# Toptachamann/Linear_Programming_Solver

Measured on AMD Instinct MI355X. Metric: simplex_pivots_per_sec, higher is better.
Workload: dtype f64

## Files before the change

### linear_programming_solver_amd/csrc/lpx_decisions.inc

```
constexpr int kMaxBlock = 32;

__global__ __launch_bounds__(256) void k_peek_multi(const double* __restrict__ A, int64_t ld,
                                                    const double* __restrict__ b, int m_local, int row0,
                                                    const double* __restrict__ prow_ring,
                                                    const double* __restrict__ col_ring, int64_t mp,
                                                    const LpxCtl* __restrict__ ring, int np,
                                                    double* __restrict__ col_out, double* __restrict__ col0_out,
                                                    RatioRow* __restrict__ partial,
                                                    const LpxCtl* __restrict__ ctl) {
  __shared__ RatioRow sh[4];
  __shared__ double sh_pe[kMaxBlock], sh_p[kMaxBlock], sh_bl[kMaxBlock];
  __shared__ int sh_e[kMaxBlock], sh_l[kMaxBlock];
  if (ctl->status != kRunning) return;
  const int en = ctl->e_next;
  if (en < 0) return;
  if ((int)threadIdx.x < np) {
    const LpxCtl& q = ring[threadIdx.x];
    sh_e[threadIdx.x] = q.e_cur;
    sh_l[threadIdx.x] = q.l - row0;
    sh_p[threadIdx.x] = q.p;
    sh_bl[threadIdx.x] = q.bl;
    sh_pe[threadIdx.x] = prow_ring[(int64_t)threadIdx.x * ld + en];
  }
  __syncthreads();
// ... 77 lines not shown
  }
}

struct ChainPart {
  double ratio, a, bi;
  int32_t row, pad;
  double unused[4];
};
#ifndef LPX_CHAIN_TAGGED
#define LPX_CHAIN_TAGGED 1
#endif
__device__ __forceinline__ unsigned lo32(double x) { return (unsigned)__double2loint(x); }
__device__ __forceinline__ unsigned hi32(double x) { return (unsigned)__double2hiint(x); }
__device__ __forceinline__ double from32(unsigned lo, unsigned hi) { return __hiloint2double((int)hi, (int)lo); }

struct MgMail {
  double ratio, a, bi;
  int32_t row;
  uint32_t tag;
};
static_assert(sizeof(MgMail) == 32, "mailbox record is one 32-byte granule");

__device__ __forceinline__ double ld_sys(const double* p) {
  return __hip_atomic_load(p, __ATOMIC_RELAXED, __HIP_MEMORY_SCOPE_SYSTEM);
}
__device__ __forceinline__ void st_sys(double* p, double x) {
  __hip_atomic_store(p, x, __ATOMIC_RELAXED, __HIP_MEMORY_SCOPE_SYSTEM);
}

__device__ __forceinline__ double ld_agent(const double* p) {
  return __hip_atomic_load(p, __ATOMIC_RELAXED, __HIP_MEMORY_SCOPE_AGENT);
}
__device__ __forceinline__ int ld_agent(const int32_t* p) {
  return __hip_atomic_load(p, __ATOMIC_RELAXED, __HIP_MEMORY_SCOPE_AGENT);
}
__device__ __forceinline__ void st_agent(double* p, double x) {
  __hip_atomic_store(p, x, __ATOMIC_RELAXED, __HIP_MEMORY_SCOPE_AGENT);
}
__device__ __forceinline__ void st_agent(int32_t* p, int32_t x) {
  __hip_atomic_store(p, x, __ATOMIC_RELAXED, __HIP_MEMORY_SCOPE_AGENT);
}

#ifndef LPX_BARRIER_SLEEP
#define LPX_BARRIER_SLEEP __builtin_amdgcn_s_sleep(1)
#endif
__device__ __forceinline__ bool grid_barrier(unsigned* bar, unsigned target, int* sh_fail, int fences, unsigned spin_max) {
  asm volatile("s_waitcnt vmcnt(0)" ::: "memory");
  __syncthreads();
  if (threadIdx.x == 0) {
    if (fences & 1) {
      __builtin_amdgcn_fence(__ATOMIC_RELEASE, "agent");
      asm volatile("s_waitcnt vmcnt(0)" ::: "memory");
    }
    __hip_atomic_fetch_add(bar, 1u, __ATOMIC_RELAXED, __HIP_MEMORY_SCOPE_AGENT);
    unsigned spins = 0;
    while (__hip_atomic_load(bar, __ATOMIC_RELAXED, __HIP_MEMORY_SCOPE_AGENT) < target) {
      LPX_BARRIER_SLEEP;
      if (++spins > spin_max) { *sh_fail = 1; break; }
    }
    if (fences & 2) {
      __builtin_amdgcn_fence(__ATOMIC_ACQUIRE, "agent");
      asm volatile("s_waitcnt vmcnt(0)" ::: "memory");
    }
  }
  __syncthreads();
  return *sh_fail == 0;
}

#define LPX_CHAIN_STEP_A(on, cs_r, pe_r, l_r)                                      \
  {                                                                                \
    const double t_ = submul(a, (cs_r), (pe_r));                     \
    const double nv_ = (ig == (l_r)) ? (pe_r) : t_;                                \
    a = (on) ? nv_ : a;                                                            \
  }
#define LPX_CHAIN_STEP_B(on, cs_r, prv_r, e_r, dv_r)                               \
  {                                                                                \
    const double t_ = submul(x, (cs_r), (prv_r));                    \
    const double nv_ = (j == (e_r)) ? (dv_r) : t_;                                 \
    x = (on) ? nv_ : x;                                                            \
  }
#define LPX_CHAIN_LIVE(r0, first, last) ((r0) < (last) && (r0) + 8 > (first))
#define LPX_CHAIN_CHUNK_A(off, r0, first, last, csv)                                                   \
  if (LPX_CHAIN_LIVE(r0, first, last)) {                                                           \
    double pe8[8];                                                                                     \
    int l8[8];                                                                                         \
    _Pragma("unroll") for (int q = 0; q < 8; ++q) { pe8[q] = sh_pe[(off) + (r0) + q]; l8[q] = sh_l[(off) + (r0) + q]; } \
    __builtin_amdgcn_sched_barrier(0);                                                                 \
    _Pragma("unroll") for (int q = 0; q < 8; ++q)                                                      \
        LPX_CHAIN_STEP_A(((r0) + q >= (first) && (r0) + q < (last)), csv[(r0) + q], pe8[q], l8[q])     \
  }
#define LPX_CHAIN_CHUNK_B(off, r0, first, last, prvv)                                                  \
  if (LPX_CHAIN_LIVE(r0, first, last)) {                                                           \
    double cs8[8], dv8[8];                                                                             \
    int e8[8];                                                                                         \
    _Pragma("unroll") for (int q = 0; q < 8; ++q) {                                                    \
      cs8[q] = sh_cs[(off) + (r0) + q]; dv8[q] = sh_dv[(off) + (r0) + q]; e8[q] = sh_e[(off) + (r0) + q]; \
    }                                                                                                  \
    __builtin_amdgcn_sched_barrier(0);                                                                 \
    _Pragma("unroll") for (int q = 0; q < 8; ++q)                                                      \
        LPX_CHAIN_STEP_B(((r0) + q >= (first) && (r0) + q < (last)), cs8[q], prvv[(r0) + q], e8[q], dv8[q]) \
  }

__device__ __forceinline__ void chain_publish(const LpxCtl* ctl, LpxCtl* host_snap) {
  if (!host_snap) return;
  *host_snap = *ctl;
  __threadfence_system();
}

__device__ __forceinline__ unsigned xcc_id() {
  unsigned x;
  asm volatile("s_getreg_b32 %0, hwreg(HW_REG_XCC_ID)" : "=s"(x));
  return x & 15u;
}

struct ChainArgs {
  const double* A;
  const double* b;
  int64_t ld, mp;
  int n, m;
  double* c;
  int32_t* perm;
  LpxCtl* ctl;
  double *prow, *col, *col0, *row0, *own_col, *own_prow, *own_dvc;
  LpxCtl* up;
  const double *prow_o, *col_o, *own_col_o, *own_prow_o, *own_dvc_o;
  const LpxCtl* up_o;
  int n_old;
  double* own_b;
  int32_t *own_rs_a, *own_rs_b;
  int b_from_tableau;
  int nb;
  ChainPart* partA;
  RatioRow* partB;
  unsigned long long* hand;
  unsigned hand_base;
  unsigned* bar;
  unsigned* bar_next;
  int dantzig, fences;
  LpxCtl* host_snap;
  long long* dbg;
  unsigned* census;
  int shard_row0;
  int m_global;
  int n_dev, dev;
  int mail_slot0;
  MgMail* mail_peer[kMaxDevices];
  double* prow_peer[kMaxDevices];
  unsigned long long* arrive_peer[kMaxDevices];
  int onehop;
  double* candrow_peer[kMaxDevices];
  unsigned long long* arrive2_peer[kMaxDevices];
  unsigned spin_max;
  int diag;
};

template <int KB>
__device__ __forceinline__ int chain_restart(const unsigned long long* sh_mask) {
  if constexpr (KB > 32) {
    const unsigned long long hi = sh_mask[1], lo = sh_mask[0];
    return hi ? 127 - __clzll((long long)hi) : (lo ? 63 - __clzll((long long)lo) : -1);
  } else {
    const unsigned long long lo = sh_mask[0];
    return lo ? 63 - __clzll((long long)lo) : -1;
  }
}

template <bool MG, int KB>
__global__ __launch_bounds__(256) void k_block_chain_t(const ChainArgs P) {
  static_assert(KB == 32 || KB == 64, "ring half of 32 or 64 slots");
  __shared__ RatioRow sh_rr[4];
  __shared__ unsigned long long sh_mask[2];
#if LPX_CHAIN_TAGGED
  __shared__ unsigned sh_gran[8], sh_part[kChainMaxWgs * 8];
#endif
  __shared__ double sh_pe[2 * KB], sh_cs[2 * KB], sh_dv[2 * KB], sh_p[2 * KB], sh_bl[2 * KB], sh_win[2];
  __shared__ int sh_e[2 * KB], sh_l[2 * KB];
  __shared__ int sh_fail, sh_restart;
  const int row0 = MG ? P.shard_row0 : 0;
  const double* __restrict__ A = P.A;
  const double* __restrict__ b = P.b;
  const int64_t ld = P.ld, mp = P.mp;
  const int n = P.n, m = P.m, nb = P.nb, n_old = P.n_old;
  LpxCtl* const ctl = P.ctl;
  const int G = gridDim.x, T = G * 256, tid = threadIdx.x, gid = blockIdx.x * 256 + tid;
  const bool lead = gid == 0;
  if (tid == 0) {
    sh_fail = 0;
    if (P.census) P.census[blockIdx.x] = xcc_id() + 1u;
  }
  if (lead) st_agent(reinterpret_cast<int32_t*>(P.bar_next), 0);
  int e = ctl->e_next;
  if (ctl->status != kRunning || e < 0 || nb < 1) {
    if (lead && nb >= 1) P.up[0].do_update = 0;
    if (lead) chain_publish(ctl, P.host_snap);
    return;
  }
  if (tid < n_old) {
    const LpxCtl& q = P.up_o[tid];
    sh_e[tid] = q.e_cur; sh_l[tid] = q.l; sh_p[tid] = q.p; sh_bl[tid] = q.bl;
  }
  int64_t pivots = ctl->pivots;
  const int64_t max_pivots = ctl->max_pivots;
  double v = ctl->v;
  int track = ctl->track, parity = ctl->parity;
  unsigned target = 0;

  for (int s = 0; s < nb; ++s) {
    if (P.dbg && lead) P.dbg[s * 5 + 0] = wall_clock64();
    const double pc = ld_agent(&P.c[e]);
    if (tid < 2 * KB) {
      const int r = tid & (KB - 1);
      const bool old = tid < KB;
      const bool valid = old ? r < n_old : r < s;
      bool same = false;
      if (valid) {
        const double* pe_src = (old ? P.prow_o : P.prow) + (int64_t)r * ld + e;
        sh_pe[tid] = MG ? ld_sys(pe_src) : ld_agent(pe_src);
        same = sh_e[tid] == e;
      }
      const unsigned long long mask = __ballot(same);
      if ((tid & 63) == 0) sh_mask[tid >> 6] = mask;
    }
    __syncthreads();
    const int ra = chain_restart<KB>(sh_mask);
    const int fo_a = ra < 0 ? 0 : (ra < KB ? ra + 1 : n_old);
    const int fn_a = ra >= KB ? ra - KB + 1 : 0;
    const bool use_b = P.b_from_tableau && s == 0;
    RatioRow best = rr_none();
    double best_a = 0.0, best_b = 0.0;
    for (int i = gid; i < m; i += T) {
      const double* src_a = ra < 0 ? &A[(int64_t)i * ld + e]
                                   : (ra < KB ? &P.own_dvc_o[(int64_t)ra * mp + i] : &P.own_dvc[(int64_t)(ra - KB) * mp + i]);
      const double* src_b = use_b ? &b[i] : &P.own_b[i];
      double a = *src_a;
      const double bi = *src_b;
      const int ig = row0 + i;
      double cs[KB], cso[KB];
#pragma unroll
      for (int r0 = 0; r0 < KB; r0 += 8)
        if (LPX_CHAIN_LIVE(r0, fo_a, n_old)) {
#pragma unroll
          for (int q = 0; q < 8; ++q) cso[r0 + q] = P.own_col_o[(int64_t)(r0 + q) * mp + i];
        }
#pragma unroll
      for (int r0 = 0; r0 < KB; r0 += 8)
        if (LPX_CHAIN_LIVE(r0, fn_a, s)) {
#pragma unroll
          for (int q = 0; q < 8; ++q) cs[r0 + q] = P.own_col[(int64_t)(r0 + q) * mp + i];
        }
#pragma unroll
      for (int r0 = 0; r0 < KB; r0 += 8) LPX_CHAIN_CHUNK_A(0, r0, fo_a, n_old, cso)
      st_agent(&P.col0[(int64_t)s * mp + i], a);
#pragma unroll
      for (int r0 = 0; r0 < KB; r0 += 8) LPX_CHAIN_CHUNK_A(KB, r0, fn_a, s, cs)
      st_agent(&P.col[(int64_t)s * mp + i], a);
      P.own_col[(int64_t)s * mp + i] = a;
      const double rt = ratio_of(a, bi);
      if (rt < best.ratio) {
        best = RatioRow{rt, ig, 0};
        best_a = a;
        best_b = bi;
      }
    }
    {
      const RatioRow w = rr_block_min(best, sh_rr);
      if (w.row != INT_MAX && best.row == w.row) { sh_win[0] = best_a; sh_win[1] = best_b; }
      __syncthreads();
#if !LPX_CHAIN_TAGGED
      if (tid == 0) {
        ChainPart* rec = &P.partA[(s & 1) * kChainMaxWgs + blockIdx.x];
        st_agent(&rec->ratio, w.ratio);
        st_agent(&rec->row, w.row);
        st_agent(&rec->a, (w.row != INT_MAX) ? sh_win[0] : 0.0);
        st_agent(&rec->bi, (w.row != INT_MAX) ? sh_win[1] : 0.0);
      }
    }
    const unsigned xtag = P.hand_base + (unsigned)s;
    if (P.dbg && lead) P.dbg[s * 5 + 1] = wall_clock64();
    target += (unsigned)G;
    if (!grid_barrier(P.bar, target, &sh_fail, P.fences, P.spin_max)) {
      if (lead) { ctl->status = 7 ; chain_publish(ctl, P.host_snap); }
      return;
    }
    if (P.dbg && lead) P.dbg[s * 5 + 2] = wall_clock64();

    RatioRow mine = rr_none();
    double mine_a = 0.0, mine_b = 0.0;
    if (tid < G) {
      const ChainPart* rec = &P.partA[(s & 1) * kChainMaxWgs + tid];
      mine.ratio = ld_agent(&rec->ratio);
      mine.row = ld_agent(&rec->row);
      mine_a = ld_agent(&rec->a);
      mine_b = ld_agent(&rec->bi);
    }
#else
      sh_gran[0] = lo32(w.ratio); sh_gran[1] = hi32(w.ratio);
      const double wa = (w.row != INT_MAX) ? sh_win[0] : 0.0, wb = (w.row != INT_MAX) ? sh_win[1] : 0.0;
      sh_gran[2] = lo32(wa); sh_gran[3] = hi32(wa); sh_gran[4] = lo32(wb); sh_gran[5] = hi32(wb);
      sh_gran[6] = (unsigned)w.row;
    }
    const unsigned xtag = P.hand_base + (unsigned)s;
#ifndef LPX_CHAIN_DBG2
    if (P.dbg && lead) P.dbg[s * 5 + 1] = wall_clock64();
#endif
    {
      unsigned long long* const gran = reinterpret_cast<unsigned long long*>(P.partA) + (size_t)(s & 1) * kChainMaxWgs * 8;
      asm volatile("s_waitcnt vmcnt(0)" ::: "memory");
// ... 328 lines not shown
      __syncthreads();
    }
    if (e_next < 0) {
      target += (unsigned)G;
      if (!grid_barrier(P.bar, target, &sh_fail, P.fences, P.spin_max)) {
        if (lead) { ctl->status = 7; chain_publish(ctl, P.host_snap); }
        return;
      }
      RatioRow m2 = rr_none();
      if (tid < G) { m2.ratio = ld_agent(&P.partB[tid].ratio); m2.row = ld_agent(&P.partB[tid].row); }
      const RatioRow w3 = rr_block_min(m2, sh_rr);
      e_next = (w3.row == INT_MAX) ? -1 : w3.row;
    }
    if (P.dbg && lead) P.dbg[s * 5 + 4] = wall_clock64();
    pivots += 1;
    parity ^= 1;
    if (lead) {
      ctl->v = v; ctl->p = p; ctl->bl = bl; ctl->pc = pc; ctl->ratio = w.ratio;
      ctl->e_cur = e; ctl->l = l; ctl->e_next = e_next; ctl->parity = parity; ctl->pivots = pivots;
      ctl->track = track; ctl->do_update = 1;
      if (e_next < 0) {
        ctl->status = 0 ;
        if (s + 1 < nb) P.up[s + 1].do_update = 0;
      }
    }
    if (e_next < 0 || s + 1 == nb) {
      if (lead) chain_publish(ctl, P.host_snap);
      return;
    }
    e = e_next;
  }
}

template <int CTRL>
__device__ __forceinline__ int dpp_i32(int v) { return __builtin_amdgcn_update_dpp(v, v, CTRL, 0xf, 0xf, false); }
template <int CTRL>
__device__ __forceinline__ double dpp_f64(double x) {
  return __hiloint2double(dpp_i32<CTRL>(__double2hiint(x)), dpp_i32<CTRL>(__double2loint(x)));
}
__device__ __forceinline__ double lane_f64(double x, int lane) {
  return __hiloint2double(__builtin_amdgcn_readlane(__double2hiint(x), lane), __builtin_amdgcn_readlane(__double2loint(x), lane));
}
__device__ __forceinline__ RatioRow rr_wave_min_all(RatioRow x) {
  double r = x.ratio;
  { const double o = dpp_f64<0xB1>(r); r = o < r ? o : r; }
  { const double o = dpp_f64<0x4E>(r); r = o < r ? o : r; }
  { const double o = dpp_f64<0x141>(r); r = o < r ? o : r; }
  { const double o = dpp_f64<0x140>(r); r = o < r ? o : r; }
  const double r0 = lane_f64(r, 0), r1 = lane_f64(r, 16), r2 = lane_f64(r, 32), r3 = lane_f64(r, 48);
  const double ra = r1 < r0 ? r1 : r0, rb = r3 < r2 ? r3 : r2;
  const double rmin = rb < ra ? rb : ra;
  int row = (x.ratio == rmin) ? x.row : INT_MAX;
  row = min(row, dpp_i32<0xB1>(row));
  row = min(row, dpp_i32<0x4E>(row));
  row = min(row, dpp_i32<0x141>(row));
  row = min(row, dpp_i32<0x140>(row));
  const int q = min(min(__builtin_amdgcn_readlane(row, 0), __builtin_amdgcn_readlane(row, 16)),
                    min(__builtin_amdgcn_readlane(row, 32), __builtin_amdgcn_readlane(row, 48)));
  return RatioRow{rmin, q, 0};
}
__device__ __forceinline__ void lds_barrier() { asm volatile("s_waitcnt lgkmcnt(0)\n\ts_barrier" ::: "memory"); }
__device__ __forceinline__ RatioRow rr_block_min2(RatioRow x, RatioRow* sh) {
  const int lane = threadIdx.x & 63, wave = threadIdx.x >> 6, nw = (blockDim.x + 63) >> 6;
  x = rr_wave_min_all(x);
  lds_barrier();
  if (lane == 0) sh[wave] = x;
  lds_barrier();
  RatioRow r = sh[0];
  for (int w = 1; w < nw; ++w) r = rr_min(r, sh[w]);
  return r;
}

#if LPX_FUSED
#define LPX_C2_T_OUT
#define LPX_C2_STEP(q) "v_fma_f64 %[x], -%[c" #q "], %[r" #q "], %[x]\n\t"
#else
#define LPX_C2_T_OUT , [t] "=&v"(t)
#define LPX_C2_STEP(q) "v_mul_f64 %[t], %[c" #q "], %[r" #q "]\n\tv_add_f64 %[x], %[x], -%[t]\n\t"
#endif
#define LPX_C2_INS                                                                                                           \
  [c0] "v"(c[0]), [c1] "v"(c[1]), [c2] "v"(c[2]), [c3] "v"(c[3]), [c4] "v"(c[4]), [c5] "v"(c[5]), [c6] "v"(c[6]), [c7] "v"(c[7]), \
  [r0] "v"(r[0]), [r1] "v"(r[1]), [r2] "v"(r[2]), [r3] "v"(r[3]), [r4] "v"(r[4]), [r5] "v"(r[5]), [r6] "v"(r[6]), [r7] "v"(r[7])
__device__ __forceinline__ void chain8(double& x, const double* c, const double* r) {
#if !LPX_FUSED
  double t;
#endif
  asm volatile(LPX_C2_STEP(0) LPX_C2_STEP(1) LPX_C2_STEP(2) LPX_C2_STEP(3) LPX_C2_STEP(4) LPX_C2_STEP(5) LPX_C2_STEP(6) LPX_C2_STEP(7)
               : [x] "+v"(x) LPX_C2_T_OUT : LPX_C2_INS);
}
__device__ __forceinline__ void chain8_from(double& x, const double* c, const double* r, int stc) {
#if !LPX_FUSED
  double t;
#endif
  unsigned long long sv, m0, m1, m2, m3, m4, m5, m6, m7;
  asm volatile("s_mov_b64 %[sv], exec\n\t"
               "v_cmp_ge_i32 %[m0], 0, %[stc]\n\tv_cmp_ge_i32 %[m1], 1, %[stc]\n\tv_cmp_ge_i32 %[m2], 2, %[stc]\n\t"
               "v_cmp_ge_i32 %[m3], 3, %[stc]\n\tv_cmp_ge_i32 %[m4], 4, %[stc]\n\tv_cmp_ge_i32 %[m5], 5, %[stc]\n\t"
               "v_cmp_ge_i32 %[m6], 6, %[stc]\n\tv_cmp_ge_i32 %[m7], 7, %[stc]\n\t"
               "s_mov_b64 exec, %[m0]\n\t" LPX_C2_STEP(0) "s_mov_b64 exec, %[m1]\n\t" LPX_C2_STEP(1)
               "s_mov_b64 exec, %[m2]\n\t" LPX_C2_STEP(2) "s_mov_b64 exec, %[m3]\n\t" LPX_C2_STEP(3)
               "s_mov_b64 exec, %[m4]\n\t" LPX_C2_STEP(4) "s_mov_b64 exec, %[m5]\n\t" LPX_C2_STEP(5)
               "s_mov_b64 exec, %[m6]\n\t" LPX_C2_STEP(6) "s_mov_b64 exec, %[m7]\n\t" LPX_C2_STEP(7)
               "s_mov_b64 exec, %[sv]"
               : [x] "+v"(x) LPX_C2_T_OUT, [sv] "=&s"(sv), [m0] "=&s"(m0), [m1] "=&s"(m1), [m2] "=&s"(m2), [m3] "=&s"(m3),
                 [m4] "=&s"(m4), [m5] "=&s"(m5), [m6] "=&s"(m6), [m7] "=&s"(m7)
               : LPX_C2_INS, [stc] "v"(stc));
}
#undef LPX_C2_INS
#undef LPX_C2_STEP
#undef LPX_C2_T_OUT
__device__ __forceinline__ int top_bit(unsigned long long lo, unsigned long long hi) {
  return hi ? 127 - __clzll((long long)hi) : (lo ? 63 - __clzll((long long)lo) : -1);
}
template <int H>
__device__ __forceinline__ int top_bit_of(const unsigned long long (&w)[H]) {
  static_assert(H == 1 || H == 2 || H == 4, "ballots of 64, 128 or 256 slots");
  if constexpr (H == 4) {
    const int hi = top_bit(w[2], w[3]);
    return hi >= 0 ? 128 + hi : top_bit(w[0], w[1]);
  } else if constexpr (H == 2) {
    return top_bit(w[0], w[1]);
  } else {
    return top_bit(w[0], 0);
  }
}

struct MinRec {
  double ratio, a, b;
  int row, pad;
};
template <int NW>
__device__ __forceinline__ RatioRow rr_block_min_rec(RatioRow x, double& a, double& b, MinRec (*sh)[NW], int slot) {
  const int wave = threadIdx.x >> 6, lane = threadIdx.x & 63;
  const RatioRow w = rr_wave_min_all(x);
  if (w.row == INT_MAX ? lane == 0 : x.row == w.row) sh[slot][wave] = MinRec{w.ratio, a, b, w.row, 0};
  lds_barrier();
  MinRec r = sh[slot][0];
#pragma unroll
  for (int k = 1; k < NW; ++k) {
    const MinRec o = sh[slot][k];
    if (o.ratio < r.ratio || (o.ratio == r.ratio && o.row < r.row)) r = o;
  }
  a = r.a;
  b = r.b;
  return RatioRow{r.ratio, r.row, 0};
}

constexpr int kChain2Threads = 256;
#ifdef LPX_CHAIN2_OWN_WT
#define LPX_OWN_STORE(p_, x_) st_agent((p_), (x_))
#else
#define LPX_OWN_STORE(p_, x_) (*(p_) = (x_))
#endif
template <int KB, int NT, bool MG>
__device__ __forceinline__ void block_chain2_body(const ChainArgs& P) {
  static_assert(KB == 32 || KB == 64 || KB == 128, "ring half of 32, 64 or 128 slots");
  static_assert(NT % 64 == 0 && NT >= 256 && NT >= 2 * KB + (KB == 128 ? 0 : 64), "lanes for the pending pivots and the loader lane");
  static_assert(KB <= 64 || !MG, "the shards decide at most kShardBlockMax pivots per block");
  constexpr int NC = 2 * KB / 8;
  constexpr int NH = (2 * KB + 63) / 64;
  constexpr int kWin = 8;
  __shared__ RatioRow sh_rr[NT / 64];
  __shared__ MinRec sh_rec[2][NT / 64];
  __shared__ unsigned sh_part[kChainMaxWgs * 8], sh_hand[8];
  __shared__ __attribute__((aligned(16))) double sh_pe[2 * KB], sh_cs[2 * KB], sh_dv[2 * KB], sh_p[2 * KB], sh_bl[2 * KB];
  __shared__ __attribute__((aligned(16))) int sh_e[2 * KB], sh_l[2 * KB];
  __shared__ int sh_fail;
#ifdef LPX_CHAIN2_FINE
#define LPX_C2_STAMP(k) if (P.dbg && lead) P.dbg[s * 16 + (k)] = wall_clock64();
#define LPX_C2_STRIDE 16
#else
#define LPX_C2_STAMP(k)
#define LPX_C2_STRIDE 8
#endif
  const int row0 = MG ? P.shard_row0 : 0;
  const double* __restrict__ A = P.A;
  const double* __restrict__ b = P.b;
  const int64_t ld = P.ld, mp = P.mp;
  const int n = P.n, m = P.m, nb = P.nb, n_old = P.n_old;
  LpxCtl* const ctl = P.ctl;
#ifdef LPX_CHAIN2_ONE_XCD
  if (blockIdx.x & 7u) return;
  const unsigned bid = blockIdx.x >> 3;
  const int G = gridDim.x >> 3;
#else
  const unsigned bid = blockIdx.x;
  const int G = gridDim.x;
#endif
  const int T = G * NT, tid = threadIdx.x, gid = bid * NT + tid;
  const bool lead = gid == 0;
  const bool book = bid == (unsigned)(G - 1) && tid == 0;
  if (tid == 0) {
    sh_fail = 0;
    if (P.census) P.census[bid] = xcc_id() + 1u;
  }
#ifdef LPX_CHAIN2_LAUNCH_STAMPS
  long long* const lst = P.dbg ? P.dbg + 8 * kBlockMax + 8 * ((P.hand_base / (unsigned)kBlockMax) & 1u) : nullptr;
  if (lst && lead) { lst[0] = wall_clock64(); lst[3] = P.hand_base / (unsigned)kBlockMax; }
#endif
  if (lead) st_agent(reinterpret_cast<int32_t*>(P.bar_next), 0);
  int e = ctl->e_next;
  if (ctl->status != kRunning || e < 0 || nb < 1) {
    if (book && nb >= 1) P.up[0].do_update = 0;
    if (book) chain_publish(ctl, P.host_snap);
    return;
  }
  if (tid < 2 * KB) {
    sh_pe[tid] = 0.0; sh_cs[tid] = 0.0; sh_dv[tid] = 0.0; sh_p[tid] = 1.0; sh_bl[tid] = 0.0;
    sh_e[tid] = -1; sh_l[tid] = -1;
  }
  lds_barrier();
  if (tid < n_old) {
    const LpxCtl& q = P.up_o[tid];
    sh_e[tid] = q.e_cur; sh_l[tid] = q.l; sh_p[tid] = q.p; sh_bl[tid] = q.bl;
  }
  int64_t pivots = ctl->pivots;
  const int64_t max_pivots = ctl->max_pivots;
  double v = ctl->v;
  int track = ctl->track, parity = ctl->parity;
  unsigned target = 0;
  const bool window = !P.dantzig && ld >= 256 && G > 1;
  const int jfirst = !window ? gid : (bid == 0 ? (tid < 256 ? tid : (int)ld) : 256 + (int)(bid - 1) * NT + tid);
  const int jstep = !window ? T : (bid == 0 ? (int)ld : T - NT);
  const char* const oc_o = reinterpret_cast<const char*>(P.own_col_o);
  const char* const oc_n = reinterpret_cast<const char*>(P.own_col);
  const char* const op_o = reinterpret_cast<const char*>(P.own_prow_o);
  const char* const op_n = reinterpret_cast<const char*>(P.own_prow);
  const uint32_t mp8_0 = (uint32_t)mp * 8u, ld8_0 = (uint32_t)ld * 8u;
  bool have_rec = false;
  unsigned long long* const hand = P.hand;
  for (int i = gid; i < m; i += T) {
#pragma unroll 8
    for (int u = 0; u < KB; ++u) LPX_OWN_STORE(&P.own_col[(int64_t)u * mp + i], 0.0);
  }
  for (int j = jfirst; j < (int)ld; j += jstep) {
#pragma unroll 8
    for (int u = 0; u < KB; ++u) LPX_OWN_STORE(&P.own_prow[(int64_t)u * ld + j], 0.0);
  }
  lds_barrier();
  for (int i = gid; i < m; i += T) {
    int r = -1;
    for (int u = 0; u < n_old; ++u) r = sh_l[u] == row0 + i ? u : r;
    P.own_rs_a[i] = r;
  }
  for (int j = jfirst; j < (int)ld; j += jstep) {
    int r = -1;
    for (int u = 0; u < n_old; ++u) r = sh_e[u] == j ? u : r;
    P.own_rs_b[j] = r;
  }

#ifdef LPX_CHAIN2_LAUNCH_STAMPS
  if (lst && lead) lst[1] = wall_clock64();
#endif
  for (int s = 0; s < nb; ++s) {
    if (P.dbg && lead) P.dbg[s * LPX_C2_STRIDE + 0] = wall_clock64();
#ifdef LPX_CHAIN2_LAUNCH_STAMPS
    if (lst && lead) lst[2] = wall_clock64();
#endif
    uint32_t mp8 = mp8_0, ld8 = ld8_0;
    asm volatile("" : "+s"(mp8), "+s"(ld8));
    const int r_mine = tid & (KB - 1);
    const bool old_mine = tid < KB;
    const bool valid_mine = tid < 2 * KB && (old_mine ? r_mine < n_old : r_mine < s);
    int ra;
    {
      unsigned long long hit[NH];
#pragma unroll
      for (int h = 0; h < NH; ++h) hit[h] = __ballot(sh_e[h * 64 + (tid & 63)] == e);
      ra = top_bit_of(hit);
    }
    const int fo_a = ra < 0 ? 0 : (ra < KB ? ra + 1 : n_old);
    const int fn_a = ra >= KB ? ra - KB + 1 : 0;
    const bool use_b = P.b_from_tableau && s == 0;
    const int co0_a = fo_a >> 3, co1_a = fo_a < n_old ? (n_old + 7) >> 3 : co0_a;
    const int cn0_a = fn_a >> 3, cn1_a = fn_a < s ? (s + 7) >> 3 : cn0_a;
    const int Lo_a = co1_a - co0_a, L_a = Lo_a + (cn1_a - cn0_a);
    auto chunk_a = [&](int k) { return (k < Lo_a ? co0_a + k : KB / 8 + cn0_a + (k - Lo_a)) & (NC - 1); };
    double pe_mine = 0.0, pc_mine = 0.0;
    const bool pe_from_rec = have_rec && tid == KB + s - 1;
    if (valid_mine && !pe_from_rec) {
      const double* const pe_src = (old_mine ? P.prow_o : P.prow) + (int64_t)r_mine * ld + e;
      pe_mine = MG ? ld_sys(pe_src) : ld_agent(pe_src);
    }
    if (tid == NT - 1 && !have_rec) pc_mine = ld_agent(&P.c[e]);
    RatioRow best = rr_none();
    double best_a = 0.0, best_b = 0.0;
    double a = 0.0, bi = 0.0, a_first = 0.0, b_first = 0.0;
    int rs = -1;
    double cv[kWin * 8];
    auto load_window_a = [&](int i, int w0) {
#pragma unroll
      for (int k = 0; k < kWin; ++k) {
        if (w0 + k < L_a) {
          const int c = chunk_a(w0 + k);
          const char* const base = (c < KB / 8 ? oc_o : oc_n) + (uint32_t)((c * 8) & (KB - 1)) * mp8;
#pragma unroll
          for (int q = 0; q < 8; ++q) cv[k * 8 + q] = *reinterpret_cast<const double*>(base + ((uint32_t)q * mp8 + (uint32_t)i * 8u));
        }
      }
    };
    auto load_row = [&](int i) {
      const uint32_t i8 = (uint32_t)i * 8u;
#ifdef LPX_DIAG_BUILD
      a = ra < 0 ? ((P.diag & 1) ? A[(int64_t)(e & 7) * ld + i] : A[(int64_t)i * ld + e])
#else
      a = ra < 0 ? A[(int64_t)i * ld + e]
#endif
                 : *reinterpret_cast<const double*>((ra < KB ? oc_o : oc_n) + ((uint32_t)(ra & (KB - 1)) * mp8 + i8));
      bi = use_b ? b[i] : P.own_b[i];
      rs = P.own_rs_a[i];
      load_window_a(i, 0);
    };
    int i = gid;
    if (i < m) load_row(i);
    int reach_a[2];
    {
      const int row_w = row0 + (int)(bid * NT) + (tid & ~63);
      unsigned long long h0[NH], h1[NH];
#pragma unroll
      for (int h = 0; h < NH; ++h) {
        const int lu = sh_l[h * 64 + (tid & 63)];
        h0[h] = __ballot((unsigned)(lu - row_w) < 64u);
        h1[h] = __ballot((unsigned)(lu - row_w - T) < 64u);
      }
      reach_a[0] = max(ra, top_bit_of(h0)) + 1;
      reach_a[1] = max(ra, top_bit_of(h1)) + 1;
    }
    asm volatile("s_waitcnt vmcnt(0)" ::: "memory");
    if (P.dbg && lead) P.dbg[s * LPX_C2_STRIDE + 1] = wall_clock64();
    if (valid_mine) sh_pe[tid] = pe_from_rec ? from32(sh_hand[3], sh_hand[4]) : pe_mine;
    if (tid == NT - 1 && !have_rec) { sh_hand[1] = lo32(pc_mine); sh_hand[2] = hi32(pc_mine); }
    lds_barrier();
    LPX_C2_STAMP(8)
    int pass_a = 0;
    while (i < m) {
      const int ig = row0 + i;
      const int reach = pass_a == 0 ? reach_a[0] : pass_a == 1 ? reach_a[1] : 2 * KB;
      ++pass_a;
      const int st = max(ra, rs) + 1;
      if (rs >= ra && rs >= 0) a = sh_pe[rs];
      else if (ra >= 0) a = -__ddiv_rn(a, sh_p[ra]);
      double pe8[2][8];
      double a_mid = a;
      auto ladder_a = [&](const int w0) {
        auto params = [&](int k) {
          if (k < kWin) {
            const double* const src = &sh_pe[chunk_a(w0 + k) * 8];
#pragma unroll
            for (int q = 0; q < 8; ++q) pe8[k & 1][q] = src[q];
          }
        };
        params(0);
#pragma unroll
        for (int k = 0; k < kWin; ++k) {
          if (w0 + k >= L_a) break;
          params(k + 1);
          __builtin_amdgcn_sched_barrier(0);
          if (w0 + k == Lo_a) a_mid = a;
          const int c8 = chunk_a(w0 + k) * 8;
          if (__builtin_expect(c8 >= reach, 1)) chain8(a, &cv[k * 8], pe8[k & 1]);
          else chain8_from(a, &cv[k * 8], pe8[k & 1], st - c8);
          __builtin_amdgcn_sched_barrier(0);
        }
      };
      ladder_a(0);
      if constexpr (NC > kWin) {
        if (L_a > kWin) {
          load_window_a(i, kWin);
          ladder_a(kWin);
        }
      }
      if constexpr (NC > 2 * kWin) {
        if (L_a > 2 * kWin) {
          load_window_a(i, 2 * kWin);
          ladder_a(2 * kWin);
        }
        if (L_a > 3 * kWin) {
          load_window_a(i, 3 * kWin);
          ladder_a(3 * kWin);
        }
      }
      if (Lo_a >= L_a) a_mid = a;
      P.col0[(int64_t)s * mp + i] = a_mid;
      LPX_C2_STAMP(9)
      st_agent(&P.col[(int64_t)s * mp + i], a);
      LPX_OWN_STORE(&P.own_col[(int64_t)s * mp + i], a);
      if (i == gid) { a_first = a; b_first = bi; }
      const double rt = ratio_of(a, bi);
      if (rt < best.ratio) {
        best = RatioRow{rt, ig, 0};
        best_a = a;
        best_b = bi;
      }
      i += T;
      __builtin_amdgcn_sched_barrier(0);
      if (i < m) load_row(i);
    }
    LPX_C2_STAMP(10)
    const double pc = from32(sh_hand[1], sh_hand[2]);
    const unsigned xtag = P.hand_base + (unsigned)s;
    {
      double wa = best_a, wb = best_b;
      const RatioRow w = rr_block_min_rec<NT / 64>(best, wa, wb, sh_rec, s & 1);
      LPX_C2_STAMP(11)
      if (w.row == INT_MAX) { wa = 0.0; wb = 0.0; }
      if (P.dbg && lead) P.dbg[s * LPX_C2_STRIDE + 2] = wall_clock64();
      unsigned long long* const gran = reinterpret_cast<unsigned long long*>(P.partA) + (size_t)(s & 1) * kChainMaxWgs * 8;
      if (tid < 7) {
        const unsigned d = tid == 0 ? lo32(w.ratio) : tid == 1 ? hi32(w.ratio) : tid == 2 ? lo32(wa) : tid == 3 ? hi32(wa)
                         : tid == 4 ? lo32(wb) : tid == 5 ? hi32(wb) : (unsigned)w.row;
        __hip_atomic_store(&gran[bid * 8 + tid], ((unsigned long long)xtag << 32) | d, __ATOMIC_RELAXED,
                           __HIP_MEMORY_SCOPE_AGENT);
      }
      for (int idx = tid; idx < G * 8; idx += NT) {
        if ((idx & 7) == 7) continue;
        unsigned long long g;
        unsigned spins = 0;
        while ((unsigned)((g = __hip_atomic_load(&gran[idx], __ATOMIC_RELAXED, __HIP_MEMORY_SCOPE_AGENT)) >> 32) != xtag) {
          LPX_BARRIER_SLEEP;
          if (++spins > P.spin_max) { sh_fail = 1; break; }
        }
        sh_part[idx] = (unsigned)g;
      }
      if (P.fences & 2) __builtin_amdgcn_fence(__ATOMIC_ACQUIRE, "agent");
      lds_barrier();
      if (sh_fail) {
        if (book) { ctl->status = 7 ; ctl->reserved = sh_fail + 1000 * s; chain_publish(ctl, P.host_snap); }
        return;
      }
    }
    if (P.dbg && lead) P.dbg[s * LPX_C2_STRIDE + 3] = wall_clock64();

    RatioRow mine = rr_none();
    double mine_a = 0.0, mine_b = 0.0;
    for (int t = tid & 63; t < G; t += 64) {
      const unsigned* q = &sh_part[t * 8];
      const RatioRow o{from32(q[0], q[1]), (int)q[6], 0};
      if (o.ratio < mine.ratio || (o.ratio == mine.ratio && o.row < mine.row)) {
        mine = o;
        mine_a = from32(q[2], q[3]);
        mine_b = from32(q[4], q[5]);
      }
    }
    RatioRow w = rr_wave_min_all(mine);
    double win_p = 0.0, win_b = 0.0;
    if (w.row != INT_MAX) {
      const int wl = __ffsll((long long)__ballot(mine.row == w.row)) - 1;
      win_p = lane_f64(mine_a, wl);
      win_b = lane_f64(mine_b, wl);
    }
    if constexpr (MG) {
      const int mslot = (P.mail_slot0 + s) & 1;
      if (lead) {
        for (int d = 0; d < P.n_dev; ++d) {
          MgMail* rec = &P.mail_peer[d][mslot * kMaxDevices + P.dev];
          st_sys(&rec->ratio, w.ratio);
          st_sys(&rec->a, win_p);
          st_sys(&rec->bi, win_b);
          __hip_atomic_store(&rec->row, w.row, __ATOMIC_RELAXED, __HIP_MEMORY_SCOPE_SYSTEM);
        }
        asm volatile("s_waitcnt vmcnt(0)" ::: "memory");
        if (P.fences & 1) {
          __builtin_amdgcn_fence(__ATOMIC_RELEASE, "");
          asm volatile("s_waitcnt vmcnt(0)" ::: "memory");
        }
        for (int d = 0; d < P.n_dev; ++d)
          __hip_atomic_store(&P.mail_peer[d][mslot * kMaxDevices + P.dev].tag, xtag, __ATOMIC_RELAXED, __HIP_MEMORY_SCOPE_SYSTEM);
      }
      RatioRow theirs = rr_none();
      double theirs_a = 0.0, theirs_b = 0.0;
      if ((tid & 63) < P.n_dev) {
        const MgMail* rec = &P.mail_peer[P.dev][mslot * kMaxDevices + (tid & 63)];
        unsigned spins = 0;
        while (__hip_atomic_load(&rec->tag, __ATOMIC_RELAXED, __HIP_MEMORY_SCOPE_SYSTEM) != xtag) {
          LPX_BARRIER_SLEEP;
          if (++spins > P.spin_max) { sh_fail = 2 + 16 * (tid & 63); break; }
        }
        if (P.fences & 2) __builtin_amdgcn_fence(__ATOMIC_ACQUIRE, "");
        theirs.ratio = ld_sys(&rec->ratio);
        theirs.row = __hip_atomic_load(&rec->row, __ATOMIC_RELAXED, __HIP_MEMORY_SCOPE_SYSTEM);
        theirs_a = ld_sys(&rec->a);
        theirs_b = ld_sys(&rec->bi);
      }
      w = rr_wave_min_all(theirs);
      win_p = 0.0; win_b = 0.0;
      if (w.row != INT_MAX) {
        const int wl = __ffsll((long long)__ballot(theirs.row == w.row)) - 1;
        win_p = lane_f64(theirs_a, wl);
        win_b = lane_f64(theirs_b, wl);
      }
      lds_barrier();
      if (sh_fail) { if (book) { ctl->status = 7; ctl->reserved = sh_fail + 1000 * s; chain_publish(ctl, P.host_snap); } return; }
    }
    if (w.row == INT_MAX || !(w.ratio < kInf)) {
      if (book) {
        ctl->status = 1; ctl->do_update = 0; ctl->l = -1; ctl->ratio = w.ratio; P.up[s].do_update = 0;
        chain_publish(ctl, P.host_snap);
      }
      return;
    }
    if (max_pivots >= 0 && pivots >= max_pivots) {
      if (book) {
        ctl->status = 9 ; ctl->do_update = 0; P.up[s].do_update = 0;
        chain_publish(ctl, P.host_snap);
      }
      return;
    }
    LPX_C2_STAMP(12)
    const int l = w.row;
    const double p = win_p, raw_b = win_b;
    if (p == 0.0) {
      if (book) { ctl->status = 8; ctl->do_update = 0; P.up[s].do_update = 0; chain_publish(ctl, P.host_snap); }
      return;
    }
    int rb;
    {
      unsigned long long hit[NH];
#pragma unroll
      for (int h = 0; h < NH; ++h) hit[h] = __ballot(sh_l[h * 64 + (tid & 63)] == l);
      rb = top_bit_of(hit);
    }
    const bool owner = !MG || (l >= row0 && l < row0 + m);
    const int ll = l - row0;
    const int fo_b = rb < 0 ? 0 : (rb < KB ? rb + 1 : n_old);
    const int fn_b = rb >= KB ? rb - KB + 1 : 0;
    const int co0_b = fo_b >> 3, co1_b = fo_b < n_old ? (n_old + 7) >> 3 : co0_b;
    const int cn0_b = fn_b >> 3, cn1_b = fn_b < s ? (s + 7) >> 3 : cn0_b;
    const int Lo_b = owner ? co1_b - co0_b : 0, L_b = owner ? Lo_b + (cn1_b - cn0_b) : 0;
    auto chunk_b = [&](int k) { return (k < Lo_b ? co0_b + k : KB / 8 + cn0_b + (k - Lo_b)) & (NC - 1); };
    double cs_mine = 0.0;
    if (valid_mine && owner) cs_mine = ld_agent((old_mine ? P.col_o : P.col) + (int64_t)r_mine * mp + ll);
    int32_t perm_e = 0, perm_l = 0;
    if (book) { perm_e = P.perm[e]; perm_l = P.perm[n + l]; }
    const double bl = __ddiv_rn(raw_b, p);
    const double inv_p = __ddiv_rn(1.0, p);
    RatioRow cand = rr_none();
    double rec_c = 0.0, rec_pr = 0.0;
    const double* rowl = A + (int64_t)(owner ? ll : 0) * ld;
    if constexpr (MG) {
      if (!owner) {
        if (tid < G) {
          const unsigned long long* aw = &P.arrive_peer[P.dev][tid];
          unsigned spins = 0;
          while (__hip_atomic_load(aw, __ATOMIC_RELAXED, __HIP_MEMORY_SCOPE_SYSTEM) != (unsigned long long)xtag) {
            LPX_BARRIER_SLEEP;
            if (++spins > P.spin_max) { sh_fail = 3 + 16 * tid; break; }
          }
          if (P.fences & 2) __builtin_amdgcn_fence(__ATOMIC_ACQUIRE, "");
        }
        lds_barrier();
        if (sh_fail) { if (book) { ctl->status = 7; ctl->reserved = sh_fail + 1000 * s; chain_publish(ctl, P.host_snap); } return; }
      }
    }
    double x = 0.0, cj = 0.0;
    int rsb = -1;
    auto load_window_b = [&](int j, int w0) {
#pragma unroll
      for (int k = 0; k < kWin; ++k) {
        if (w0 + k < L_b) {
          const int c = chunk_b(w0 + k);
          const char* const base = (c < KB / 8 ? op_o : op_n) + (uint32_t)((c * 8) & (KB - 1)) * ld8;
#pragma unroll
          for (int q = 0; q < 8; ++q) cv[k * 8 + q] = *reinterpret_cast<const double*>(base + ((uint32_t)q * ld8 + (uint32_t)j * 8u));
        }
      }
    };
    auto load_col = [&](int j) {
      cj = ld_agent(&P.c[j]);
      x = 0.0;
      rsb = P.own_rs_b[j];
      if (!owner) {
        x = (j < n && j != e) ? ld_sys(&P.prow[(int64_t)s * ld + j]) : 0.0;
      } else if (j < n) {
        const uint32_t j8 = (uint32_t)j * 8u;
        x = rb < 0 ? rowl[j]
                   : *reinterpret_cast<const double*>((rb < KB ? op_o : op_n) + ((uint32_t)(rb & (KB - 1)) * ld8 + j8));
        load_window_b(j, 0);
      }
    };
    int j = jfirst;
    if (j < (int)ld) load_col(j);
    int reach_b[2];
    {
      const int col_w = __builtin_amdgcn_readfirstlane(jfirst);
      unsigned long long h0[NH], h1[NH];
#pragma unroll
      for (int h = 0; h < NH; ++h) {
        const int eu = sh_e[h * 64 + (tid & 63)];
        h0[h] = __ballot((unsigned)(eu - col_w) < 64u);
        h1[h] = __ballot((unsigned)(eu - col_w - jstep) < 64u);
      }
      reach_b[0] = max(rb, top_bit_of(h0)) + 1;
      reach_b[1] = max(rb, top_bit_of(h1)) + 1;
    }
    asm volatile("s_waitcnt vmcnt(0)" ::: "memory");
    if (P.dbg && lead) P.dbg[s * LPX_C2_STRIDE + 4] = wall_clock64();
    if (valid_mine) {
      sh_cs[tid] = cs_mine;
      sh_dv[tid] = -__ddiv_rn(cs_mine, sh_p[tid]);
    }
    lds_barrier();
    LPX_C2_STAMP(13)
    int pass_b = 0;
    while (j < (int)ld) {
      const int reach = pass_b == 0 ? reach_b[0] : pass_b == 1 ? reach_b[1] : 2 * KB;
      ++pass_b;
      if (j < n && owner) {
        const int st = max(rb, rsb) + 1;
        if (rsb > rb) x = sh_dv[rsb];
        double cs8[2][8];
        double x_mid = x;
        auto ladder_b = [&](const int w0) {
          auto params = [&](int k) {
            if (k < kWin) {
              const double* const src = &sh_cs[chunk_b(w0 + k) * 8];
#pragma unroll
              for (int q = 0; q < 8; ++q) cs8[k & 1][q] = src[q];
            }
          };
          params(0);
#pragma unroll
          for (int k = 0; k < kWin; ++k) {
            if (w0 + k >= L_b) break;
            params(k + 1);
            __builtin_amdgcn_sched_barrier(0);
            if (w0 + k == Lo_b) x_mid = x;
            const int c8 = chunk_b(w0 + k) * 8;
            if (__builtin_expect(c8 >= reach, 1)) chain8(x, cs8[k & 1], &cv[k * 8]);
            else chain8_from(x, cs8[k & 1], &cv[k * 8], st - c8);
            __builtin_amdgcn_sched_barrier(0);
          }
        };
        ladder_b(0);
        if constexpr (NC > kWin) {
          if (L_b > kWin) {
            load_window_b(j, kWin);
            ladder_b(kWin);
          }
        }
        if constexpr (NC > 2 * kWin) {
          if (L_b > 2 * kWin) {
            load_window_b(j, 2 * kWin);
            ladder_b(2 * kWin);
          }
          if (L_b > 3 * kWin) {
            load_window_b(j, 3 * kWin);
            ladder_b(3 * kWin);
          }
        }
        if (Lo_b >= L_b) x_mid = x;
        P.row0[(int64_t)s * ld + j] = x_mid;
      }
      LPX_C2_STAMP(14)
      double cn, pr;
      if (j == e) {
        pr = inv_p;
        cn = -__ddiv_rn(pc, p);
      } else {
        pr = owner ? __ddiv_rn(x, p) : x;
        cn = submul(cj, pc, pr);
      }
      if constexpr (MG) {
        if (owner) {
          for (int d = 0; d < P.n_dev; ++d)
            if (d != P.dev) st_sys(&P.prow_peer[d][(int64_t)s * ld + j], pr);
        }
      }
      st_agent(&P.prow[(int64_t)s * ld + j], pr);
      LPX_OWN_STORE(&P.own_prow[(int64_t)s * ld + j], pr);
      if (j == e) P.own_rs_b[j] = KB + s;
      st_agent(&P.c[j], cn);
      if (j < n && cn > kEps) {
        const RatioRow k2{P.dantzig ? -cn : 0.0, j, 0};
        cand = rr_min(cand, k2);
      }
      rec_c = cn;
      rec_pr = pr;
      j += jstep;
      __builtin_amdgcn_sched_barrier(0);
      if (j < (int)ld) load_col(j);
    }
    LPX_C2_STAMP(15)
    if (window && bid == 0) {
      MinRec* const ho = sh_rec[s & 1];
      const unsigned long long cm = __ballot(cand.row != INT_MAX);
      if ((tid & 63) == (cm ? __ffsll((long long)cm) - 1 : 0)) ho[tid >> 6] = MinRec{rec_c, rec_pr, 0.0, cm ? cand.row : -1, 0};
      lds_barrier();
      if (tid < 5) {
        int slot = -1;
        double hc = 0.0, hp = 0.0;
#pragma unroll
        for (int k = NT / 64 - 1; k >= 0; --k) {
          const MinRec o = ho[k];
          if (o.row >= 0) { slot = o.row; hc = o.ratio; hp = o.a; }
        }
        const unsigned d = tid == 0 ? (unsigned)((slot < 0 ? -2 : slot) + 2) : slot < 0 ? 0u : tid == 1 ? lo32(hc) : tid == 2 ? hi32(hc) : tid == 3 ? lo32(hp) : hi32(hp);
        __hip_atomic_store(&hand[tid], ((unsigned long long)xtag << 32) | d, __ATOMIC_RELAXED, __HIP_MEMORY_SCOPE_AGENT);
      }
    }
    if constexpr (MG) {
      if (owner && P.n_dev > 1) {
        asm volatile("s_waitcnt vmcnt(0)" ::: "memory");
        lds_barrier();
        if (tid == 0) {
          if (P.fences & 1) {
            __builtin_amdgcn_fence(__ATOMIC_RELEASE, "");
            asm volatile("s_waitcnt vmcnt(0)" ::: "memory");
          }
          for (int d = 0; d < P.n_dev; ++d)
            if (d != P.dev)
              __hip_atomic_store(&P.arrive_peer[d][bid], (unsigned long long)xtag, __ATOMIC_RELAXED, __HIP_MEMORY_SCOPE_SYSTEM);
        }
      }
    }
    if (P.dbg && lead) P.dbg[s * LPX_C2_STRIDE + 5] = wall_clock64();
    if (gid < m) P.own_b[gid] = (row0 + gid == l) ? bl : submul(b_first, a_first, bl);
    if (gid < m && row0 + gid == l) P.own_rs_a[gid] = KB + s;
    for (int i2 = gid + T; i2 < m; i2 += T) {
      const double colv = P.own_col[(int64_t)s * mp + i2];
      const double bcur = use_b ? b[i2] : P.own_b[i2];
      P.own_b[i2] = (row0 + i2 == l) ? bl : submul(bcur, colv, bl);
      if (row0 + i2 == l) P.own_rs_a[i2] = KB + s;
    }
    if (tid == 0) { sh_e[KB + s] = e; sh_l[KB + s] = l; sh_p[KB + s] = p; sh_bl[KB + s] = bl; }
    if (book) {
      v = addmul(v, bl, pc);
      P.perm[e] = perm_l;
      P.perm[n + l] = perm_e;
      if (track >= 0) {
        if (e == track) track = l + n;
        else if (l + n == track) track = e;
      }
      LpxCtl& up = P.up[s];
      up.p = p; up.bl = bl; up.e_cur = e; up.l = l; up.e_next = -1; up.parity = 0; up.do_update = 1;
    }
    if (P.dbg && lead) P.dbg[s * LPX_C2_STRIDE + 6] = wall_clock64();
    int e_next = -2;
    have_rec = false;
    if (window) {
      if (tid < 5) {
        unsigned long long rec = 0;
        unsigned spins = 0;
        for (;;) {
          rec = __hip_atomic_load(&hand[tid], __ATOMIC_RELAXED, __HIP_MEMORY_SCOPE_AGENT);
          if ((unsigned)(rec >> 32) == xtag) break;
          LPX_BARRIER_SLEEP;
          if (++spins > P.spin_max) { sh_fail = 4; break; }
        }
        sh_hand[tid] = (unsigned)rec;
      }
      lds_barrier();
      if (sh_fail) { if (book) { ctl->status = 7; ctl->reserved = sh_fail + 1000 * s; chain_publish(ctl, P.host_snap); } return; }
      e_next = (int)sh_hand[0] - 2;
      have_rec = e_next >= 0;
    }
    if (e_next < 0) {
      const RatioRow w2 = rr_block_min2(cand, sh_rr);
      if (tid == 0) {
        st_agent(&P.partB[bid].ratio, w2.ratio);
        st_agent(&P.partB[bid].row, w2.row);
      }
      target += (unsigned)G;
      if (!grid_barrier(P.bar, target, &sh_fail, P.fences, P.spin_max)) {
        if (book) { ctl->status = 7; chain_publish(ctl, P.host_snap); }
        return;
      }
      RatioRow m2 = rr_none();
      if (tid < G) { m2.ratio = ld_agent(&P.partB[tid].ratio); m2.row = ld_agent(&P.partB[tid].row); }
      const RatioRow w3 = rr_block_min2(m2, sh_rr);
      e_next = (w3.row == INT_MAX) ? -1 : w3.row;
    }
    if (P.dbg && lead) P.dbg[s * LPX_C2_STRIDE + 7] = wall_clock64();
    pivots += 1;
    parity ^= 1;
    if (book) {
      ctl->v = v; ctl->p = p; ctl->bl = bl; ctl->pc = pc; ctl->ratio = w.ratio;
      ctl->e_cur = e; ctl->l = l; ctl->e_next = e_next; ctl->parity = parity; ctl->pivots = pivots;
      ctl->track = track; ctl->do_update = 1;
      if (e_next < 0) {
        ctl->status = 0 ;
        if (s + 1 < nb) P.up[s + 1].do_update = 0;
      }
    }
    if (e_next < 0 || s + 1 == nb) {
      if (book) chain_publish(ctl, P.host_snap);
      return;
    }
    e = e_next;
    lds_barrier();
  }
}
template <int KB, int NT, bool MG>
__global__ __launch_bounds__(NT) void k_block_chain2_t(const ChainArgs P) {
  static_assert(KB == 32 || KB == 64, "ring half of 32 or 64 slots");
  block_chain2_body<KB, NT, MG>(P);
}
template <int NT>
__global__ __launch_bounds__(NT) void k_block_decide128(const ChainArgs P) {
  block_chain2_body<128, NT, false>(P);
}
#undef LPX_C2_STAMP
#undef LPX_C2_STRIDE
#undef LPX_CHAIN_STEP_A
#undef LPX_CHAIN_STEP_B
#undef LPX_CHAIN_CHUNK_A
#undef LPX_CHAIN_CHUNK_B
#undef LPX_CHAIN_LIVE
```

### linear_programming_solver_amd/csrc/lpx_dispatch.cpp

```cpp
#include "lpx_kernels.h"

#include <algorithm>

namespace lpxk {

#define LPX_PICK(B, f) ((B).fused ? fused::f : plain::f)

void launch_entering(const Buffers& B, int n, hipStream_t s, const LoopStart& start) { LPX_PICK(B, launch_entering)(B, n, s, start); }
void launch_entering_dantzig(const Buffers& B, int n, bool seed, hipStream_t s, const LoopStart& start) {
  LPX_PICK(B, launch_entering_dantzig)(B, n, seed, s, start);
}
void launch_ratio_gather(const Buffers& B, int m_local, int row0, const Geometry& g, int forced_e, hipStream_t s) {
  LPX_PICK(B, launch_ratio_gather)(B, m_local, row0, g, forced_e, s);
}
void launch_reduce_partials(const Buffers& B, const Geometry& g, hipStream_t s) {
  LPX_PICK(B, launch_reduce_partials)(B, g, s);
}
void launch_select_pivot(const Buffers& B, int n, int m_global, const Geometry& g, int forced_e, int forced_l,
                         hipStream_t s) {
  LPX_PICK(B, launch_select_pivot)(B, n, m_global, g, forced_e, forced_l, s);
}
void launch_update(const Buffers& B, int m_local, int n, int row0, const Geometry& g, bool nontemporal,
                   const double* prow, const LpxCtl* up, double* A_out, double* b_out, hipStream_t s) {
  LPX_PICK(B, launch_update)(B, m_local, n, row0, g, nontemporal, prow, up, A_out, b_out, s);
}
void launch_propose(const Buffers& B, int n, int row0, int m_local, const Geometry& g, double* d_candidate,
                    hipStream_t s) {
  LPX_PICK(B, launch_propose)(B, n, row0, m_local, g, d_candidate, s);
}
void launch_commit(const Buffers& B, int n, int m_global, const double* d_gathered, int nranks, double* prow,
                   LpxCtl* up, int up_parity, hipStream_t s) {
  LPX_PICK(B, launch_commit)(B, n, m_global, d_gathered, nranks, prow, up, up_parity, s);
}
void launch_peek(const Buffers& B, int n, int m_local, int row0, const double* prow_t, const double* col_t,
                 double* col_next, const LpxCtl* pend, double* d_candidate, hipStream_t s) {
  LPX_PICK(B, launch_peek)(B, n, m_local, row0, prow_t, col_t, col_next, pend, d_candidate, s);
}
void launch_block_peek(const Buffers& B, const BlockRing& R, int n, int m_local, int row0, int np, double* d_candidate,
                       hipStream_t s) {
  LPX_PICK(B, launch_block_peek)(B, R, n, m_local, row0, np, d_candidate, s);
}
void launch_block_decide(const Buffers& B, const BlockRing& R, int n, int m_global, const double* d_gathered, int nranks,
                         int slot, hipStream_t s) {
  LPX_PICK(B, launch_block_decide)(B, R, n, m_global, d_gathered, nranks, slot, s);
}
int launch_block_chain(const Buffers& B, const BlockRing& R, int n, int m, int nb, int half, int old_half, int n_old,
                       int b_from_tableau, int seq, int dantzig, int wgs, int fences, bool trace, LpxCtl* host_snap,
                       hipStream_t s, const MgPeers* mg, hipEvent_t stop) {
  return LPX_PICK(B, launch_block_chain)(B, R, n, m, nb, half, old_half, n_old, b_from_tableau, seq, dantzig, wgs, fences, trace,
                                  host_snap, s, mg, stop);
}
void preload_block_kernels(const Buffers& B, const BlockRing& R, hipStream_t s) {
  plain::preload_block_kernels(B, R, s);
  fused::preload_block_kernels(B, R, s);
}
unsigned* sweep_fail_word(const BlockRing& R, int64_t ld) { return plain::sweep_fail_word(R, ld); }
int64_t sweep_ticket_slots(int64_t ld) { return plain::sweep_ticket_slots(ld); }
int chain_blocks_per_cu() { return std::min(plain::chain_blocks_per_cu(), fused::chain_blocks_per_cu()); }
const char* sweep_kernel_name(int code) { return plain::sweep_kernel_name(code); }
int launch_block_sweep(const Buffers& B, const BlockRing& R, int n, int m_local, int row0, int K, int rows_per_wg,
                       bool nt, hipStream_t s, const double* A_src, const double* b_src, hipEvent_t after_sweep, int cus,
                       int form, int* kernel_used, const FixSide* side, hipEvent_t stop, hipEvent_t before_sweep) {
  return LPX_PICK(B, launch_block_sweep)(B, R, n, m_local, row0, K, rows_per_wg, nt, s, A_src, b_src, after_sweep, cus,
                                         form, kernel_used, side, stop, before_sweep);
}
void launch_fill_column(double* A, int64_t ld, int m, int col, double value, hipStream_t s) {
  plain::launch_fill_column(A, ld, m, col, value, s);
}
void launch_drop_column(double* A, int64_t ld, int m, int n_old, int col, hipStream_t s) {
  plain::launch_drop_column(A, ld, m, n_old, col, s);
}
void launch_restore_objective(const Buffers& B, int n, const RestoreEntry* d_entries, int n_entries, hipStream_t s) {
  LPX_PICK(B, launch_restore_objective)(B, n, d_entries, n_entries, s);
}
void launch_checksum(const Buffers& B, int m_local, int n, int row0, unsigned long long* d_out3, hipStream_t s) {
  plain::launch_checksum(B, m_local, n, row0, d_out3, s);
}
hipError_t launch_batch_simplex(const BatchArgs& a, hipStream_t s) {
  return a.fused ? fused::launch_batch_simplex(a, s) : plain::launch_batch_simplex(a, s);
}
int batch_blocks_per_cu(int threads, int lds_bytes) {
  return std::min(plain::batch_blocks_per_cu(threads, lds_bytes), fused::batch_blocks_per_cu(threads, lds_bytes));
}
hipError_t launch_batch_solve(const BatchSolveArgs& a, hipStream_t s) {
  return a.fused ? fused::launch_batch_solve(a, s) : plain::launch_batch_solve(a, s);
}
int batch_solve_blocks_per_cu(int threads, int lds_bytes) {
  return std::min(plain::batch_solve_blocks_per_cu(threads, lds_bytes), fused::batch_solve_blocks_per_cu(threads, lds_bytes));
}
hipError_t launch_batch_scenarios(const BatchScenarioArgs& a, hipStream_t s) {
  return a.fused ? fused::launch_batch_scenarios(a, s) : plain::launch_batch_scenarios(a, s);
}
int batch_scenarios_blocks_per_cu(int threads, int lds_bytes) {
  return std::min(plain::batch_scenarios_blocks_per_cu(threads, lds_bytes), fused::batch_scenarios_blocks_per_cu(threads, lds_bytes));
}
hipError_t launch_scenarios_crash(const ScenarioCrashArgs& a, hipStream_t s) {
  return a.fused ? fused::launch_scenarios_crash(a, s) : plain::launch_scenarios_crash(a, s);
}
hipError_t launch_batch_resolve(const BatchResolveArgs& a, hipStream_t s) {
  return a.fused ? fused::launch_batch_resolve(a, s) : plain::launch_batch_resolve(a, s);
}
int batch_resolve_blocks_per_cu(int threads, int lds_bytes) {
  return std::min(plain::batch_resolve_blocks_per_cu(threads, lds_bytes), fused::batch_resolve_blocks_per_cu(threads, lds_bytes));
}
void launch_transpose(const double* dA, int64_t lda, double* dAt, int64_t ldat, int m, int n, hipStream_t s) {
  plain::launch_transpose(dA, lda, dAt, ldat, m, n, s);
}

}
```

### linear_programming_solver_amd/csrc/lpx_engine.cpp

```cpp
#include <hip/hip_runtime.h>

#include <algorithm>
#include <chrono>
#include <cmath>
#include <cstdio>
#include <cstdlib>
#include <cstring>
#include <string>
#include <vector>

#include "../../include/lpx.h"
#include "lpx_kernels.h"
#include "lpx_internal.h"

using lpxk::Buffers;
using lpxk::Geometry;
using lpxk::LpxCtl;
using lpxk::RatioRow;

thread_local std::string g_last_error;

int fail(int status, const std::string& msg) {
  g_last_error = msg;
  return status;
// ... 457 lines not shown
extern "C" int lpx_pivot(lpx_state* s, int32_t entering, int32_t leaving) {
  if (int rc = require_single(s, "lpx_pivot")) return rc;
  if (!(entering >= 0 && entering < s->n) || !(leaving >= 0 && leaving < s->m))
    return fail(LPX_BAD_ARGUMENT, "lpx_pivot: index out of range");
  HIP_TRY(hipSetDevice(s->device));
  if (int rc = set_running(s, -1, -1)) return rc;
  lpxk::launch_ratio_gather(s->B, s->m, s->row0, s->g, entering, s->stream);
  lpxk::launch_select_pivot(s->B, s->n, s->m_global, s->g, entering, leaving, s->stream);
  if (int rc = launch_update_profiled(s)) return rc;
  HIP_TRY(hipGetLastError());
  if (int rc = sync_ctl_to_host(s)) return rc;
  if (s->h_ctl->status == LPX_DIVIDE_BY_ZERO) return fail(LPX_DIVIDE_BY_ZERO, "lpx_pivot: pivot element is zero");
  return 0;
}

hipError_t peer_visible_malloc(const lpx_state* s, void** ptr, size_t bytes) {
  if (s->peer_written) return hipExtMallocWithFlags(ptr, bytes, hipDeviceMallocFinegrained);
  return hipMalloc(ptr, bytes);
}

int32_t state_n(const lpx_state* s) { return s->n; }

static int build_block_ring(lpx_state* s);
int ensure_block_ring(lpx_state* s) {
  if (s->R.prow) return 0;
  const int rc = build_block_ring(s);
  if (rc) {
    const std::string why = g_last_error;
    free_block_ring(s);
    if (s->peer_written) return fail(rc, (why + " (ring of a multi-GPU shard: peer-written buffers need fine-grained device memory)").c_str());
    g_last_error = why;
  }
  return rc;
}
static int build_block_ring(lpx_state* s) {
  const int64_t mp = std::max<int64_t>(2, round_up(s->m, 2)) + 2;
  s->R.mp = mp;
  const size_t K = 2 * lpxk::kBlockMax;
  HIP_TRY(peer_visible_malloc(s, (void**)&s->R.prow, K * (size_t)s->B.ld * sizeof(double)));
  HIP_TRY(peer_visible_malloc(s, &s->R.mg_mail, 2 * lpxk::kMaxDevices * 32));
  HIP_TRY(peer_visible_malloc(s, (void**)&s->R.mg_arrive, lpxk::kChainMaxWgs * sizeof(unsigned long long)));
  HIP_TRY(hipMemsetAsync(s->R.mg_mail, 0, 2 * lpxk::kMaxDevices * 32, s->stream));
  HIP_TRY(hipMemsetAsync(s->R.mg_arrive, 0, lpxk::kChainMaxWgs * sizeof(unsigned long long), s->stream));
  if (s->m != s->m_global || s->peer_written || s->multi_shard) {
    const size_t rows_bytes = 2 * (size_t)lpxk::kMaxDevices * (size_t)s->B.ld * sizeof(double);
    const size_t words_bytes = 2 * (size_t)lpxk::kMaxDevices * lpxk::kChainMaxWgs * sizeof(unsigned long long);
    HIP_TRY(peer_visible_malloc(s, (void**)&s->R.mg_candrow, rows_bytes));
    HIP_TRY(peer_visible_malloc(s, (void**)&s->R.mg_arrive2, words_bytes));
    HIP_TRY(hipMemsetAsync(s->R.mg_candrow, 0, rows_bytes, s->stream));
    HIP_TRY(hipMemsetAsync(s->R.mg_arrive2, 0, words_bytes, s->stream));
  }
  HIP_TRY(hipMalloc((void**)&s->R.col, K * (size_t)mp * sizeof(double)));
  HIP_TRY(hipMalloc((void**)&s->R.col0, K * (size_t)mp * sizeof(double)));
  HIP_TRY(hipMalloc((void**)&s->R.row0, K * (size_t)s->B.ld * sizeof(double)));
  HIP_TRY(hipMemsetAsync(s->R.col0, 0, K * (size_t)mp * sizeof(double), s->stream));
  HIP_TRY(hipMemsetAsync(s->R.row0, 0, K * (size_t)s->B.ld * sizeof(double), s->stream));
  HIP_TRY(hipMalloc((void**)&s->R.up, K * sizeof(LpxCtl)));
  HIP_TRY(hipMalloc(&s->R.chain_part_a, 2 * lpxk::kChainMaxWgs * 64));
  HIP_TRY(hipMemsetAsync(s->R.chain_part_a, 0, 2 * lpxk::kChainMaxWgs * 64, s->stream));
  HIP_TRY(hipMalloc(&s->R.chain_part_b, lpxk::kChainMaxWgs * 16));
  HIP_TRY(hipMalloc((void**)&s->R.chain_bar, 512));
  HIP_TRY(hipMemsetAsync(s->R.chain_bar, 0, 512, s->stream));
  HIP_TRY(hipMalloc((void**)&s->R.chain_own_col, K * (size_t)mp * sizeof(double)));
  HIP_TRY(hipMalloc((void**)&s->R.chain_own_prow, K * (size_t)s->B.ld * sizeof(double)));
  HIP_TRY(hipMalloc((void**)&s->R.chain_own_dvc, K * (size_t)mp * sizeof(double)));
  HIP_TRY(hipMalloc((void**)&s->R.chain_own_b, (size_t)mp * sizeof(double)));
  HIP_TRY(hipMalloc((void**)&s->R.chain_own_rs, (size_t)(mp + s->B.ld) * sizeof(int32_t)));
  HIP_TRY(hipMemsetAsync(s->R.chain_own_rs, 0xff, (size_t)(mp + s->B.ld) * sizeof(int32_t), s->stream));
  HIP_TRY(hipMemsetAsync(s->R.chain_own_col, 0, K * (size_t)mp * sizeof(double), s->stream));
  HIP_TRY(hipMemsetAsync(s->R.chain_own_prow, 0, K * (size_t)s->B.ld * sizeof(double), s->stream));
  HIP_TRY(hipMalloc((void**)&s->R.chain_dbg, 16 * lpxk::kBlockMax * sizeof(long long)));
  HIP_TRY(hipMemsetAsync(s->R.chain_dbg, 0, 16 * lpxk::kBlockMax * sizeof(long long), s->stream));
  HIP_TRY(hipMalloc((void**)&s->R.census, (lpxk::kChainMaxWgs + 2 + 1200) * sizeof(unsigned)));
  HIP_TRY(hipMemsetAsync(s->R.census, 0, (lpxk::kChainMaxWgs + 2 + 1200) * sizeof(unsigned), s->stream));
  HIP_TRY(hipMalloc((void**)&s->R.zeros, 256));
  HIP_TRY(hipMemsetAsync(const_cast<double*>(s->R.zeros), 0, 256, s->stream));
  HIP_TRY(hipMalloc((void**)&s->R.tickets, 2 * (size_t)lpxk::sweep_ticket_slots(s->B.ld) * 128));
  HIP_TRY(hipMemsetAsync(s->R.tickets, 0, 2 * (size_t)lpxk::sweep_ticket_slots(s->B.ld) * 128, s->stream));
  HIP_TRY(hipMalloc((void**)&s->R.sweep_fail, 128));
  HIP_TRY(hipMemsetAsync(s->R.sweep_fail, 0, 128, s->stream));
  HIP_TRY(hipMalloc((void**)&s->R.clk, 256));
  HIP_TRY(hipMemsetAsync(s->R.clk, 0, 256, s->stream));
  HIP_TRY(hipMalloc((void**)&s->R.col_packed, 2 * (size_t)(mp / 4 + 1) * 4 * lpxk::kColPackedRowBytes));
  HIP_TRY(hipMemsetAsync(s->R.col_packed, 0, 2 * (size_t)(mp / 4 + 1) * 4 * lpxk::kColPackedRowBytes, s->stream));
  HIP_TRY(hipMalloc((void**)&s->d_cand, (size_t)(LPX_CAND_HEADER + s->B.ld) * sizeof(double)));
  HIP_TRY(hipMemsetAsync(s->R.prow, 0, K * (size_t)s->B.ld * sizeof(double), s->stream));
  HIP_TRY(hipMemsetAsync(s->R.col, 0, K * (size_t)mp * sizeof(double), s->stream));
  HIP_TRY(hipMemsetAsync(s->R.up, 0, K * sizeof(LpxCtl), s->stream));
  HIP_TRY(hipMemsetAsync(s->d_cand, 0, (size_t)(LPX_CAND_HEADER + s->B.ld) * sizeof(double), s->stream));
  lpxk::preload_block_kernels(s->B, s->R, s->stream);
  return 0;
}

int ensure_spare_tableau(lpx_state* s) {
  if (s->A2) return 0;
  const int64_t mp = std::max<int64_t>(2, round_up(s->m, 2)) + 2;
  const int64_t off = s->opt[LPX_OPT_A2_OFFSET];
  HIP_TRY(hipMalloc((void**)&s->A_base[1], (size_t)(mp * s->B.ld + off) * sizeof(double)));
  s->A2 = s->A_base[1] + off;
  HIP_TRY(hipMalloc((void**)&s->b_base[1], (size_t)mp * sizeof(double)));
  s->b2 = s->b_base[1];
  HIP_TRY(hipMemset(s->A2, 0, (size_t)(mp * s->B.ld) * sizeof(double)));
  HIP_TRY(hipMemset(s->b2, 0, (size_t)mp * sizeof(double)));
  HIP_TRY(hipDeviceSynchronize());
  return 0;
}

constexpr double kBlock128MinSweepUs = 1400.0;
constexpr int64_t kBlock128MinBudget = 256;
int choose_block(const lpx_state* s, int64_t max_pivots) {
  int K = (int)s->opt[LPX_OPT_BLOCK];
  if (K == 0) {
    const double sweep_us = 16.0 * (double)s->m * (double)s->B.ld / 6.0e6;
    if (sweep_us < 6.3) K = s->R.prow ? 16 : 1;
    else if (sweep_us < 10.0) K = 16;
    else K = 32;
    if (sweep_us >= 2500.0 && s->m % 4 == 0 && s->B.ld >= 512) K = 64;
    if (s->B.fused && sweep_us >= 300.0 && s->m % 16 == 0 && s->B.ld >= 512 && s->m_global == s->m) K = 64;
    if (K == 64 && s->B.fused && sweep_us >= kBlock128MinSweepUs && s->B.ld % 512 == 0 && s->m_global == s->m && !s->multi_shard &&
        s->opt[LPX_OPT_CHAIN] != 0 && s->opt[LPX_OPT_OVERLAP] != 0 && (max_pivots < 0 || max_pivots >= kBlock128MinBudget))
      K = 128;
  }
#ifdef LPX_WITH_VARIANTS
  if (s->B.chain_form != 1) K = std::min(K, 64);
#endif
  if (!s->opt[LPX_OPT_CHAIN] || s->m_global != s->m) K = std::min(K, (int)lpxk::kShardBlockMax);
  return std::max(1, std::min(K, (int)lpxk::kBlockMax));
}

int block_len(int K, int64_t max_pivots, int64_t decided) {
  if (max_pivots < 0) return K;
  const int64_t room = max_pivots + 1 - decided;
  return (int)std::max<int64_t>(0, std::min<int64_t>(K, room));
}

int clamp_chain_wgs(lpx_state* s, int want, int cus) {
  const int per_cu = lpxk::chain_blocks_per_cu();
  const int cap = std::max(1, per_cu * std::max(1, cus));
  s->info.chain_blocks_per_cu = per_cu;
  s->info.chain_resident_max = cap;
  s->info.chain_wgs_requested = want;
  const int G = std::max(1, std::min(std::min(want, cap), (int)lpxk::kChainMaxWgs));
  s->info.chain_wgs = G;
  return G;
}

int device_cus(const lpx_state* s) {
  int ncu = 0;
  if (hipDeviceGetAttribute(&ncu, hipDeviceAttributeMultiprocessorCount, s->device) != hipSuccess) ncu = 0;
  return ncu;
}

int launch_sweep_profiled(lpx_state* s, int K, hipStream_t stream, const Buffers& B, const lpxk::BlockRing& R,
                                 const double* A_src, const double* b_src, const lpxk::FixSide* side, hipEvent_t stop) {
  const bool sample = s->prof > 0 && (s->prof_seq++ % s->prof) == 0;
  if (sample) {
    if (s->ev_used + 2 > s->ev.size()) {
      for (int k = 0; k < 512; k++) {
        hipEvent_t e;
        HIP_TRY(hipEventCreate(&e));
        s->ev.push_back(e);
      }
    }
  }
  const int cus = (stream == s->ov_sweep && s->ov_masked) ? s->ov_sweep_cus : device_cus(s);
  int kernel_used = 0;
  s->info.sweep_cus = cus;
  s->info.sweep_rows = lpxk::launch_block_sweep(B, R, s->n, s->m, s->row0, K, (int)s->opt[LPX_OPT_SWEEP_ROWS],
                                                s->nontemporal, stream, A_src, b_src,
                                                sample ? s->ev[s->ev_used + 1] : nullptr, cus,
                                                (int)s->opt[LPX_OPT_SWEEP_FORM], &kernel_used, side, stop,
                                                sample ? s->ev[s->ev_used] : nullptr);
  s->info.sweep_kernel = kernel_used;
  if (sample) s->ev_used += 2;
  HIP_TRY(hipGetLastError());
  return 0;
}
static int launch_sweep_profiled(lpx_state* s, int K) {
  return launch_sweep_profiled(s, K, s->stream, s->B, s->R, nullptr, nullptr, nullptr, nullptr);
}

lpxk::BlockRing ring_half(const lpx_state* s, int h) {
  lpxk::BlockRing R = s->R;
  const int64_t o = (int64_t)h * lpxk::kBlockMax;
  R.prow += o * s->B.ld;
  R.row0 += o * s->B.ld;
  R.col += o * R.mp;
  R.col0 += o * R.mp;
  if (R.fix_col) R.fix_col += o * R.mp;
  if (R.fix_row) R.fix_row += o * s->B.ld;
  if (R.col_packed) R.col_packed += (int64_t)h * (R.mp / 4 + 1) * (4 * lpxk::kColPackedRowBytes / sizeof(double));
  if (R.tickets) R.tickets += (int64_t)h * lpxk::sweep_ticket_slots(s->B.ld) * 32;
  R.up += o;
  return R;
}

#ifndef LPX_CHAIN_CUS_PER_XCD
#define LPX_CHAIN_CUS_PER_XCD 4
#endif
static int chain_cus_per_xcd(const lpx_state* s, int per_xcd) {
  int k = LPX_CHAIN_CUS_PER_XCD;
  const int64_t work = std::max<int64_t>(s->m, s->B.ld);
  const double bytes = 8.0 * (double)s->m * (double)s->B.ld;
  if (!s->multi_shard && work > 8192 && bytes <= 1.5 * 1073741824.0) k = 8;
  if (!s->multi_shard && work > 8192 && s->B.fused) k = 8;
  if (s->opt[LPX_OPT_CHAIN_CUS] > 0) k = std::max(4, (int)s->opt[LPX_OPT_CHAIN_CUS] / 4 * 4);
  return std::max(1, std::min(k, (per_xcd - 1) / 4 * 4));
}
int ensure_overlap_streams(lpx_state* s) {
  if (s->ov_chain) return 0;
  hipDeviceProp_t prop;
  HIP_TRY(hipGetDeviceProperties(&prop, s->device));
  const int ncu = prop.multiProcessorCount;
  const int per_xcd = ncu / 8;
  std::vector<uint32_t> m_sweep((ncu + 31) / 32, 0u), m_chain((ncu + 31) / 32, 0u);
  const int kChainCusPerXcd = chain_cus_per_xcd(s, per_xcd);
  int sweep_per_xcd = per_xcd - kChainCusPerXcd;
  if (s->opt[LPX_OPT_SWEEP_CUS] > 0) sweep_per_xcd = std::max(1, std::min(sweep_per_xcd, (int)s->opt[LPX_OPT_SWEEP_CUS] / 8));
  for (int cu = 0; cu < ncu; cu++) {
    if (cu / 8 >= per_xcd - kChainCusPerXcd) m_chain[cu / 32] |= 1u << (cu % 32);
    else if (cu / 8 < sweep_per_xcd) m_sweep[cu / 32] |= 1u << (cu % 32);
  }
  bool masked = false;
  if (s->opt[LPX_OPT_OVERLAP_MASK] != 0 && ncu >= 64) {
    masked = hipExtStreamCreateWithCUMask(&s->ov_chain, (uint32_t)m_chain.size(), m_chain.data()) == hipSuccess &&
             hipExtStreamCreateWithCUMask(&s->ov_sweep, (uint32_t)m_sweep.size(), m_sweep.data()) == hipSuccess;
    if (!masked) {
      (void)hipGetLastError();
      if (s->ov_chain) { (void)hipStreamDestroy(s->ov_chain); s->ov_chain = nullptr; }
      if (s->ov_sweep) { (void)hipStreamDestroy(s->ov_sweep); s->ov_sweep = nullptr; }
    }
  }
  if (!masked) {
    int lo = 0, hi = 0;
    HIP_TRY(hipDeviceGetStreamPriorityRange(&lo, &hi));
    HIP_TRY(hipStreamCreateWithPriority(&s->ov_chain, hipStreamNonBlocking, hi));
    HIP_TRY(hipStreamCreateWithFlags(&s->ov_sweep, hipStreamNonBlocking));
  }
  s->ov_masked = masked;
  s->ov_chain_cus = masked ? 8 * kChainCusPerXcd : ncu;
  s->ov_sweep_cus = masked ? 8 * sweep_per_xcd : ncu;
  for (int k = 0; k < 2; k++) {
    HIP_TRY(hipEventCreateWithFlags(&s->ev_ov_chain[k], hipEventDisableTiming));
    HIP_TRY(hipEventCreateWithFlags(&s->ev_ov_sweep[k], hipEventDisableTiming));
  }
  for (int k = 0; k < 3; k++) HIP_TRY(hipEventCreateWithFlags(&s->ev_ov_join[k], hipEventDisableTiming));
  return 0;
}

int ensure_fix_side(lpx_state* s, int mode) {
  if (mode < 1 || mode > 3) return fail(LPX_BAD_ARGUMENT, "ensure_fix_side: mode");
  const size_t K = 2 * lpxk::kBlockMax;
  if (!s->R.fix_col) {
    HIP_TRY(hipMalloc((void**)&s->R.fix_col, K * (size_t)s->R.mp * sizeof(double)));
    HIP_TRY(hipMemsetAsync(s->R.fix_col, 0, K * (size_t)s->R.mp * sizeof(double), s->stream));
  }
  if (!s->R.fix_row) {
    HIP_TRY(hipMalloc((void**)&s->R.fix_row, K * (size_t)s->B.ld * sizeof(double)));
    HIP_TRY(hipMemsetAsync(s->R.fix_row, 0, K * (size_t)s->B.ld * sizeof(double), s->stream));
  }
  for (int k = 0; k < 2; k++) {
    if (!s->ev_ov_fix[k]) HIP_TRY(hipEventCreateWithFlags(&s->ev_ov_fix[k], hipEventDisableTiming));
    if (!s->ev_ov_pack[k]) HIP_TRY(hipEventCreateWithFlags(&s->ev_ov_pack[k], hipEventDisableTiming));
  }
  if (s->ov_fix[mode]) return 0;
  bool made = false;
  if (s->ov_masked && mode != 3) {
    hipDeviceProp_t prop;
    HIP_TRY(hipGetDeviceProperties(&prop, s->device));
    const int ncu = prop.multiProcessorCount, per_xcd = ncu / 8;
    const int chain_per_xcd = s->ov_chain_cus / 8, sweep_per_xcd = s->ov_sweep_cus / 8;
    std::vector<uint32_t> mask((ncu + 31) / 32, 0u);
    for (int cu = 0; cu < ncu; cu++) {
      const bool chain_cu = cu / 8 >= per_xcd - chain_per_xcd, sweep_cu = !chain_cu && cu / 8 < sweep_per_xcd;
      if (mode == 1 ? sweep_cu : chain_cu) mask[cu / 32] |= 1u << (cu % 32);
    }
    made = hipExtStreamCreateWithCUMask(&s->ov_fix[mode], (uint32_t)mask.size(), mask.data()) == hipSuccess;
    if (!made) { (void)hipGetLastError(); s->ov_fix[mode] = nullptr; }
  }
  if (!made) HIP_TRY(hipStreamCreateWithFlags(&s->ov_fix[mode], hipStreamNonBlocking));
  return 0;
}

static int blocked_loop_overlapped(lpx_state* s, int K, int64_t max_pivots, const lpxk::LoopStart& start) {
  if (int rc = ensure_block_ring(s)) return rc;
  if (int rc = ensure_spare_tableau(s)) return rc;
  if (int rc = ensure_overlap_streams(s)) return rc;
  launch_seed_entering(s, start);
  HIP_TRY(hipEventRecord(s->ev_ov_join[0], s->stream));
  HIP_TRY(hipStreamWaitEvent(s->ov_chain, s->ev_ov_join[0], 0));
  HIP_TRY(hipStreamWaitEvent(s->ov_sweep, s->ev_ov_join[0], 0));
  LpxCtl* h2 = s->h_snap;
  LpxCtl* d_snap = nullptr;
  HIP_TRY(hipHostGetDevicePointer((void**)&d_snap, s->h_snap, 0));
  const int64_t work = std::max<int64_t>(s->m, s->B.ld);
  const int chain_cap = s->ov_masked ? std::max(32, s->ov_chain_cus) : 32;
  int auto_wgs = (int)std::min<int64_t>(chain_cap, std::max<int64_t>(1, (work + 255) / 256));
  if (s->pricing == 0 && auto_wgs >= 8) auto_wgs += 1;
  const int chain_wgs = clamp_chain_wgs(s, s->opt[LPX_OPT_CHAIN_WGS] > 0 ? (int)s->opt[LPX_OPT_CHAIN_WGS] : auto_wgs,
                                        s->ov_chain_cus);
  const int fences = (int)s->opt[LPX_OPT_CHAIN_FENCES];
  const bool trace = s->opt[LPX_OPT_CHAIN_TRACE] != 0;
  s->info.chain_stream_masked = s->ov_masked ? 1 : 0;
  s->info.overlapped = 1;
  double* Abuf[2] = {s->B.A, s->A2};
  double* bbuf[2] = {s->B.b, s->b2};
  int64_t decided = 0;
  int nb_prev = 0, nblk = 0;
  const bool serial = s->opt[LPX_OPT_OVERLAP_SERIAL] != 0;
  int fix_mode = serial ? 0 : (int)s->opt[LPX_OPT_FIXUP_SIDE];
  if (fix_mode == 4) fix_mode = 8.0 * (double)s->m * (double)s->B.ld >= 2.0 * 1073741824.0 ? 2 : 0;
  if (fix_mode > 0 && ensure_fix_side(s, fix_mode) != 0) {
    (void)hipGetLastError();
    fix_mode = 0;
  }
  auto issue_block = [&](int k) -> int {
    const int nb = block_len(K, max_pivots, decided);
    if (nb <= 0) return 1;
    const int h = k & 1;
    Buffers Brd = s->B;
    if (serial) {
      if (k >= 1) HIP_TRY(hipStreamWaitEvent(s->ov_chain, s->ev_ov_sweep[h ^ 1], 0));
      Brd.A = Abuf[h];
      Brd.b = bbuf[h];
      s->info.chain_wgs = lpxk::launch_block_chain(Brd, s->R, s->n, s->m, nb, h, h ^ 1, 0, 1, s->chain_seq++, s->pricing == 1,
                                                   chain_wgs, fences, trace, d_snap + h, s->ov_chain, nullptr, s->ev_ov_chain[h]);
    } else {
      if (k >= 2) HIP_TRY(hipStreamWaitEvent(s->ov_chain, s->ev_ov_sweep[h], 0));
      Brd.A = Abuf[k == 0 ? 0 : (k - 1) & 1];
      Brd.b = bbuf[k == 0 ? 0 : (k - 1) & 1];
      s->info.chain_wgs = lpxk::launch_block_chain(Brd, s->R, s->n, s->m, nb, h, h ^ 1, k > 0 ? nb_prev : 0, k == 0,
                                                   s->chain_seq++, s->pricing == 1, chain_wgs, fences, trace, d_snap + h,
                                                   s->ov_chain, nullptr, s->ev_ov_chain[h]);
    }
    s->chain_nb_last = nb;
    if (max_pivots >= 0 && decided == max_pivots) {
      decided += nb;
      return 0;
    }
    HIP_TRY(hipStreamWaitEvent(s->ov_sweep, s->ev_ov_chain[h], 0));
    Buffers Bdst = s->B;
    Bdst.A = Abuf[h ^ 1];
    Bdst.b = bbuf[h ^ 1];
    const lpxk::FixSide side{fix_mode > 0 ? s->ov_fix[fix_mode] : nullptr, s->ev_ov_chain[h], s->ev_ov_fix[h], s->ev_ov_pack[h]};
    if (int rc = launch_sweep_profiled(s, nb, s->ov_sweep, Bdst, ring_half(s, h), Abuf[h], bbuf[h], fix_mode > 0 ? &side : nullptr,
                                       s->ev_ov_sweep[h])) return rc;
    decided += nb;
    nb_prev = nb;
    nblk = k + 1;
    return 0;
  };
  int rc = issue_block(0);
  if (rc == 1) rc = 0;
  for (int k = 1; rc == 0; k++) {
    const int r = issue_block(k);
    if (r != 0 && r != 1) { rc = r; break; }
    hipError_t e = hipEventSynchronize(s->ev_ov_chain[(k - 1) & 1]);
    if (e != hipSuccess) { rc = fail(LPX_DEVICE_ERROR, hipGetErrorString(e)); break; }
    if (h2[(k - 1) & 1].status != lpxk::kRunning || r == 1) break;
  }
  (void)hipEventRecord(s->ev_ov_join[1], s->ov_chain);
  (void)hipEventRecord(s->ev_ov_join[2], s->ov_sweep);
  (void)hipStreamWaitEvent(s->stream, s->ev_ov_join[1], 0);
  (void)hipStreamWaitEvent(s->stream, s->ev_ov_join[2], 0);
  if (nblk & 1) {
    std::swap(s->B.A, s->A2);
    std::swap(s->B.b, s->b2);
  }
  if (rc == 0) rc = enqueue_ctl_fetch(s);
  hipError_t e2 = hipStreamSynchronize(s->stream);
  if (rc == 0 && e2 != hipSuccess) rc = fail(LPX_DEVICE_ERROR, hipGetErrorString(e2));
  return rc;
}

static int blocked_loop(lpx_state* s, int K, int64_t max_pivots, const lpxk::LoopStart& start) {
  const bool one_block = max_pivots >= 0 && max_pivots + 1 <= K;
  if (s->opt[LPX_OPT_CHAIN] != 0 && s->opt[LPX_OPT_OVERLAP] != 0 && s->row0 == 0 && s->m == s->m_global && !one_block) {
    if (s->A2 || ensure_spare_tableau(s) == 0) return blocked_loop_overlapped(s, K, max_pivots, start);
    (void)hipGetLastError();
    if (s->A_base[1]) { (void)hipFree(s->A_base[1]); s->A_base[1] = nullptr; }
    if (s->b_base[1]) { (void)hipFree(s->b_base[1]); s->b_base[1] = nullptr; }
    s->A2 = nullptr;
    s->b2 = nullptr;
  }
  if (int rc = ensure_block_ring(s)) return rc;
  launch_seed_entering(s, start);
  hipEvent_t* evs = s->ev_batch;
  LpxCtl* h2 = s->h_snap;
  int64_t decided = 0;
  const bool fused = s->opt[LPX_OPT_CHAIN] != 0 && s->row0 == 0 && s->m == s->m_global;
  const int64_t work = std::max<int64_t>(s->m, s->B.ld);
  const int auto_wgs = (int)std::min<int64_t>(64, std::max<int64_t>(1, (work + 255) / 256));
  const int chain_wgs = fused ? clamp_chain_wgs(s, s->opt[LPX_OPT_CHAIN_WGS] > 0 ? (int)s->opt[LPX_OPT_CHAIN_WGS] : auto_wgs,
                                                device_cus(s))
                              : 0;
  const int fences = (int)s->opt[LPX_OPT_CHAIN_FENCES];
  const bool trace = s->opt[LPX_OPT_CHAIN_TRACE] != 0;
  s->info.chain_stream_masked = 0;
  s->info.overlapped = 0;
  LpxCtl* d_snap = nullptr;
  if (fused) HIP_TRY(hipHostGetDevicePointer((void**)&d_snap, s->h_snap, 0));
  auto issue_block = [&](int slot) -> int {
    const int nb = block_len(K, max_pivots, decided);
    if (fused && nb > 0) {
      s->info.chain_wgs = lpxk::launch_block_chain(s->B, s->R, s->n, s->m, nb, 0, 0, 0, 1, s->chain_seq++, s->pricing == 1,
                                                   chain_wgs, fences, trace, d_snap + slot, s->stream);
      s->chain_nb_last = nb;
    } else {
      for (int k = 0; k < nb; k++) {
        lpxk::launch_block_peek(s->B, s->R, s->n, s->m, s->row0, k, s->d_cand, s->stream);
        lpxk::launch_block_decide(s->B, s->R, s->n, s->m_global, s->d_cand, 1, k, s->stream);
        if (s->pricing == 1) lpxk::launch_entering_dantzig(s->B, s->n, false, s->stream);
      }
    }
    const bool probe_only = max_pivots >= 0 && decided == max_pivots;
    decided += nb;
    if (nb > 0 && !probe_only) {
      if (int rc = launch_sweep_profiled(s, nb)) return rc;
    }
    if (!fused)
      HIP_TRY(hipMemcpyAsync(&h2[slot], s->B.ctl, sizeof(LpxCtl), hipMemcpyDeviceToHost, s->stream));
    HIP_TRY(hipEventRecord(evs[slot], s->stream));
    return 0;
  };
  int rc = issue_block(0);
  int cur = 0;
  while (rc == 0) {
    rc = issue_block(cur ^ 1);
    if (rc) break;
    hipError_t e = hipEventSynchronize(evs[cur]);
    if (e != hipSuccess) { rc = fail(LPX_DEVICE_ERROR, hipGetErrorString(e)); break; }
    if (h2[cur].status != lpxk::kRunning) break;
    cur ^= 1;
  }
  if (rc == 0) rc = enqueue_ctl_fetch(s);
  hipError_t e2 = hipStreamSynchronize(s->stream);
  if (rc == 0 && e2 != hipSuccess) rc = fail(LPX_DEVICE_ERROR, hipGetErrorString(e2));
  return rc;
}

extern "C" int lpx_state_get_block(const lpx_state* s) { return s ? choose_block(s, -1) : -1; }

extern "C" int lpx_shard_block_peek(lpx_state* s, double* d_candidate, int32_t slot) {
  if (!s || !d_candidate || slot < 0 || slot >= lpxk::kShardBlockMax)
    return fail(LPX_BAD_ARGUMENT, "lpx_shard_block_peek: bad argument");
  HIP_TRY(hipSetDevice(s->device));
  if (int rc = ensure_block_ring(s)) return rc;
  lpxk::launch_block_peek(s->B, s->R, s->n, s->m, s->row0, slot, d_candidate, s->stream);
  HIP_TRY(hipGetLastError());
  return 0;
}

extern "C" int lpx_shard_block_decide(lpx_state* s, const double* d_gathered, int32_t nranks, int32_t slot) {
  if (!s || !d_gathered || nranks < 1 || slot < 0 || slot >= lpxk::kShardBlockMax)
    return fail(LPX_BAD_ARGUMENT, "lpx_shard_block_decide: bad argument");
  HIP_TRY(hipSetDevice(s->device));
  if (int rc = ensure_block_ring(s)) return rc;
  lpxk::launch_block_decide(s->B, s->R, s->n, s->m_global, d_gathered, nranks, slot, s->stream);
  if (s->pricing == 1) lpxk::launch_entering_dantzig(s->B, s->n, false, s->stream);
  HIP_TRY(hipGetLastError());
  return 0;
}

extern "C" int lpx_shard_block_sweep(lpx_state* s, int32_t nslots) {
  if (!s || nslots < 0 || nslots > lpxk::kShardBlockMax) return fail(LPX_BAD_ARGUMENT, "lpx_shard_block_sweep: bad argument");
  HIP_TRY(hipSetDevice(s->device));
  if (nslots == 0) return 0;
  if (int rc = ensure_block_ring(s)) return rc;
  return launch_sweep_profiled(s, nslots);
}

extern "C" int lpx_state_set_block(lpx_state* s, int32_t pivots_per_sweep) {
  if (!s || pivots_per_sweep < 0 || pivots_per_sweep > lpxk::kBlockMax)
    return fail(LPX_BAD_ARGUMENT, "lpx_state_set_block: 0 (auto), 1 (off) .. 128");
  s->opt[LPX_OPT_BLOCK] = pivots_per_sweep;
  s->loop_block = 0;
  return 0;
}

extern "C" int lpx_state_set_option(lpx_state* s, int32_t key, int64_t value) {
  if (!s || key < 0 || key >= LPX_OPT_COUNT) return fail(LPX_BAD_ARGUMENT, "lpx_state_set_option: unknown option");
  const OptionSpec& sp = kOptionSpec[key];
  if (value < sp.lo || value > sp.hi) return fail(LPX_BAD_ARGUMENT, std::string("lpx_state_set_option: value out of range for ") + sp.env);
  if (key == LPX_OPT_UPDATE_U && value == 3) return fail(LPX_BAD_ARGUMENT, "lpx_state_set_option: UPDATE_U is 1, 2 or 4");
  if (key == LPX_OPT_A2_OFFSET && s->A2) return fail(LPX_BAD_ARGUMENT, "lpx_state_set_option: the second tableau exists already");
  if ((key == LPX_OPT_CHAIN_CUS || key == LPX_OPT_SWEEP_CUS) && s->ov_chain && value != s->opt[key])
    return fail(LPX_BAD_ARGUMENT, "lpx_state_set_option: the CU-masked stream pair of this handle exists already (set CHAIN_CUS / SWEEP_CUS before the first blocked loop)");
  s->opt[key] = value;
  s->loop_block = 0;
  if (key == LPX_OPT_CHAIN_FORM) s->B.chain_form = (int)value;
  if (key == LPX_OPT_FUSED) resolve_arithmetic(s);
  if (key == LPX_OPT_UPDATE_U || key == LPX_OPT_UPDATE_ROWS || key == LPX_OPT_NT) apply_layout_options(s);
  return 0;
}

extern "C" int lpx_state_get_option(const lpx_state* s, int32_t key, int64_t* value) {
  if (!s || !value || key < 0 || key >= LPX_OPT_COUNT) return fail(LPX_BAD_ARGUMENT, "lpx_state_get_option: bad argument");
  *value = s->opt[key];
  return 0;
}

extern "C" int lpx_state_get_info(lpx_state* s, lpx_state_info* out) {
  if (!s || !out) return fail(LPX_BAD_ARGUMENT, "lpx_state_get_info: NULL argument");
  HIP_TRY(hipSetDevice(s->device));
  s->info.block = s->loop_block > 0 ? s->loop_block : choose_block(s, -1);
  s->info.arith_fused = s->B.fused ? 1 : 0;
  s->info.chain_xcd_mask = 0;
  s->info.sweep_xcd_mask = 0;
  if (s->R.census) {
    HIP_TRY(hipStreamSynchronize(s->stream));
    std::vector<unsigned> h(lpxk::kChainMaxWgs + 2);
    HIP_TRY(hipMemcpy(h.data(), s->R.census, h.size() * sizeof(unsigned), hipMemcpyDeviceToHost));
    for (int w = 0; w < s->info.chain_wgs && w < (int)lpxk::kChainMaxWgs; w++)
      if (h[w]) s->info.chain_xcd_mask |= 1 << ((h[w] - 1) & 15);
    s->info.sweep_xcd_mask = (int32_t)h[lpxk::kChainMaxWgs];
  }
  s->info.sweep_clock_mhz = 0;
  if (s->R.clk) {
    long long c32[32] = {};
    HIP_TRY(hipStreamSynchronize(s->stream));
    HIP_TRY(hipMemcpy(c32, s->R.clk, sizeof c32, hipMemcpyDeviceToHost));
    std::vector<double> mhz;
    for (int x = 0; x < 8; x++) {
      const long long* c4 = c32 + 4 * x;
      if (c4[3] > c4[1] && c4[2] > c4[0] && c4[3] - c4[1] > 1000) {
        const double f = 100.0 * (double)(c4[2] - c4[0]) / (double)(c4[3] - c4[1]);
        if (f > 300.0 && f < 3500.0) mhz.push_back(f);
      }
    }
    if (!mhz.empty()) {
      std::sort(mhz.begin(), mhz.end());
      s->info.sweep_clock_mhz = (int32_t)(mhz[mhz.size() / 2] + 0.5);
    }
  }
  *out = s->info;
  return 0;
}

extern "C" const char* lpx_sweep_kernel_name(int32_t code) { return lpxk::sweep_kernel_name(code); }

extern "C" int lpx_debug_read_census(lpx_state* s, uint32_t* out, int32_t count) {
  if (!s || !out || !s->R.census || count < 0 || count > (int)lpxk::kChainMaxWgs + 2 + 1200) return LPX_BAD_ARGUMENT;
  if (hipSetDevice(s->device) != hipSuccess || hipDeviceSynchronize() != hipSuccess) return LPX_DEVICE_ERROR;
  return hipMemcpy(out, s->R.census, (size_t)count * sizeof(uint32_t), hipMemcpyDeviceToHost) == hipSuccess ? 0 : LPX_DEVICE_ERROR;
}

extern "C" int lpx_debug_read_chain_dbg(lpx_state* s, int64_t* out, int32_t count) {
  if (!s || !out || !s->R.chain_dbg || count < 0 || count > 16 * (int)lpxk::kBlockMax) return LPX_BAD_ARGUMENT;
  if (hipSetDevice(s->device) != hipSuccess || hipDeviceSynchronize() != hipSuccess) return LPX_DEVICE_ERROR;
  return hipMemcpy(out, s->R.chain_dbg, (size_t)count * sizeof(int64_t), hipMemcpyDeviceToHost) == hipSuccess ? 0 : LPX_DEVICE_ERROR;
}

#ifdef LPX_CHAIN2_FINE
static int chain_trace_stride(const lpx_state* s) { return (s->B.chain_form == 1 && !(s->multi_shard && s->opt[LPX_OPT_MULTI_ONEHOP] != 0)) ? 16 : 5; }
#else
static int chain_trace_stride(const lpx_state* s) { return (s->B.chain_form == 1 && !(s->multi_shard && s->opt[LPX_OPT_MULTI_ONEHOP] != 0)) ? 8 : 5; }
#endif

extern "C" int lpx_state_read_chain_trace(lpx_state* s, int64_t* ticks, int32_t cap, int32_t* ndecisions) {
  if (!s || !ticks || cap < 0 || !ndecisions) return fail(LPX_BAD_ARGUMENT, "lpx_state_read_chain_trace: bad argument");
  *ndecisions = 0;
  if (!s->R.chain_dbg || s->opt[LPX_OPT_CHAIN_TRACE] == 0) return 0;
  HIP_TRY(hipSetDevice(s->device));
  HIP_TRY(hipStreamSynchronize(s->stream));
  long long h[16 * lpxk::kBlockMax];
  HIP_TRY(hipMemcpy(h, s->R.chain_dbg, sizeof h, hipMemcpyDeviceToHost));
  const int nd = std::min<int>(std::min<int>(cap, s->chain_nb_last), lpxk::kBlockMax);
  static const int pick8[5] = {0, 2, 3, 6, 7};
  const int st = chain_trace_stride(s);
  for (int d = 0; d < nd; d++)
    for (int k = 0; k < 5; k++) ticks[5 * d + k] = h[st * d + (st >= 8 ? pick8[k] : k)];
// ... 327 lines not shown
```

### linear_programming_solver_amd/csrc/lpx_internal.h

```cpp
#pragma once
#include <hip/hip_runtime.h>

#include <string>
#include <vector>

#include "../../include/lpx.h"
#include "lpx_kernels.h"

using lpxk::Buffers;
using lpxk::Geometry;
using lpxk::LpxCtl;
using lpxk::RatioRow;

int fail(int status, const std::string& msg);

#define HIP_TRY(expr)                                                                         \
  do {                                                                                        \
    hipError_t _e = (expr);                                                                   \
    if (_e != hipSuccess)                                                                     \
      return fail(LPX_DEVICE_ERROR, std::string(#expr) + ": " + hipGetErrorString(_e));       \
  } while (0)

struct DeviceRestore {
  int d = -1;
  DeviceRestore() { if (hipGetDevice(&d) != hipSuccess) { d = -1; (void)hipGetLastError(); } }
  ~DeviceRestore() { if (d >= 0) (void)hipSetDevice(d); }
};

struct lpx_state {
  int device = 0;
  hipStream_t own_stream = nullptr;
  hipStream_t stream = nullptr;
  int32_t m = 0;
  int32_t n = 0;
  int32_t row0 = 0, m_global = 0;
  int32_t n_cap = 0;
  Buffers B{};
  Geometry g{};
  bool nontemporal = false;
  int pricing = 0;
  int64_t opt[LPX_OPT_COUNT] = {};
  lpx_state_info info{};
  int loop_block = 0;
  int chain_nb_last = 0;
  bool peer_written = false;
  bool multi_shard = false;
  lpxk::BlockRing R{};
  int chain_seq = 0;
  hipStream_t ov_chain = nullptr, ov_sweep = nullptr;
  bool ov_masked = false;
  int ov_chain_cus = 0;
  int ov_sweep_cus = 0;
  hipEvent_t ev_ov_chain[2] = {nullptr, nullptr}, ev_ov_sweep[2] = {nullptr, nullptr}, ev_ov_join[3] = {nullptr, nullptr, nullptr};
  hipStream_t ov_fix[4] = {nullptr, nullptr, nullptr, nullptr};
  hipEvent_t ev_ov_fix[2] = {nullptr, nullptr};
  hipEvent_t ev_ov_pack[2] = {nullptr, nullptr};
  double* d_cand = nullptr;
  LpxCtl* h_ctl = nullptr;
  LpxCtl* h_snap = nullptr;
  hipEvent_t ev_batch[2] = {nullptr, nullptr};
  LpxCtl* ring = nullptr;
  double* prow2 = nullptr;
  hipStream_t comm_stream = nullptr;
  hipEvent_t ev_peek = nullptr, ev_decide = nullptr, ev_upd = nullptr;
  int pipeline = 1;
  double* A2 = nullptr;
  double* A_base[2] = {nullptr, nullptr};
  double* b_base[2] = {nullptr, nullptr};
  double* b2 = nullptr;
  bool upd_recorded = false;
  bool settled = true;
  unsigned long long* d_sum = nullptr;
  int prof = 0;
  int64_t prof_seq = 0;
  std::vector<hipEvent_t> ev;
  size_t ev_used = 0;
  int64_t prof_launches = 0;
  double prof_ms = 0.0;
};


int sync_ctl_to_host(lpx_state* s);
int push_ctl(lpx_state* s);
void free_state(lpx_state* s);
int alloc_state(int32_t m_local, int32_t n, int32_t n_cap, int32_t row0, int32_t m_global, int device, lpx_state** out);
int upload_common(lpx_state* s, const double* A, int64_t lda, const double* b, const double* c, double v,
                  const int32_t* perm, hipMemcpyKind kind);
void init_ctl(lpx_state* s, double v);
int set_running(lpx_state* s, int64_t max_pivots, int32_t track);
void resolve_arithmetic(lpx_state* s);
int ensure_block_ring(lpx_state* s);
int ensure_spare_tableau(lpx_state* s);
int ensure_overlap_streams(lpx_state* s);
hipError_t peer_visible_malloc(const lpx_state* s, void** ptr, size_t bytes);
int32_t state_n(const lpx_state* s);
int choose_block(const lpx_state* s, int64_t max_pivots = -1);
int block_len(int K, int64_t max_pivots, int64_t decided);
int clamp_chain_wgs(lpx_state* s, int want, int cus);
int device_cus(const lpx_state* s);
int launch_sweep_profiled(lpx_state* s, int K, hipStream_t stream, const Buffers& B, const lpxk::BlockRing& R,
                          const double* A_src, const double* b_src, const lpxk::FixSide* side = nullptr,
                          hipEvent_t stop = nullptr);
int ensure_fix_side(lpx_state* s, int mode);
lpxk::BlockRing ring_half(const lpx_state* s, int h);
void launch_seed_entering(lpx_state* s, const lpxk::LoopStart& start = lpxk::LoopStart{});
int launch_update_profiled(lpx_state* s, const double* prow = nullptr, const LpxCtl* up = nullptr,
                           const Buffers* Bin = nullptr, double* A_out = nullptr, double* b_out = nullptr);

int multi_create(int32_t m, int32_t n, int32_t n_cap, const double* A, int64_t lda, const double* b, const double* c,
                 double v, const int32_t* perm, const int32_t* devices, int32_t n_dev, lpx_multi** out);
namespace lpx_internal {
int multi_shards(lpx_multi* M);
lpx_state* multi_shard(lpx_multi* M, int r);
int multi_device(lpx_multi* M, int r);
int32_t multi_row_start(lpx_multi* M, int r);
int multi_owner(lpx_multi* M, int32_t row);
void multi_set_n(lpx_multi* M, int32_t n);
}
```

### linear_programming_solver_amd/csrc/lpx_kernels.hip

```cpp
#include "lpx_kernels.h"

#include <hip/hip_ext.h>

#include <atomic>

#include <limits.h>
#include <stdint.h>
#include <stdlib.h>

#include <algorithm>
#include <type_traits>

#ifndef LPX_FUSED
#define LPX_FUSED 0
#endif

namespace lpxk {
#if LPX_FUSED
namespace fused {
#else
namespace plain {
#endif

typedef double d2 __attribute__((ext_vector_type(2)));
// ... 637 lines not shown
  const int64_t total = (int64_t)m_local * n;
  for (int64_t idx = (int64_t)blockIdx.x * blockDim.x + threadIdx.x; idx < total;
       idx += (int64_t)gridDim.x * blockDim.x) {
    const int64_t i = idx / n, j = idx - i * n;
    const unsigned long long bits = (unsigned long long)__double_as_longlong(A[i * ld + j]);
    sa += mix64(bits, (unsigned long long)((row0 + i) * (int64_t)n + j));
  }
  if (blockIdx.x == 0) {
    for (int i = threadIdx.x; i < m_local; i += blockDim.x)
      sb += mix64((unsigned long long)__double_as_longlong(b[i]), (unsigned long long)(row0 + i));
    for (int j = threadIdx.x; j < n; j += blockDim.x)
      sc += mix64((unsigned long long)__double_as_longlong(c[j]), (unsigned long long)j);
  }
#pragma unroll
  for (int off = 32; off >= 1; off >>= 1) {
    sa += __shfl_down(sa, off, 64);
    sb += __shfl_down(sb, off, 64);
    sc += __shfl_down(sc, off, 64);
  }
  if ((threadIdx.x & 63) == 0) {
    atomicAdd(&out[0], sa);
    if (blockIdx.x == 0) { atomicAdd(&out[1], sb); atomicAdd(&out[2], sc); }
  }
}

__global__ __launch_bounds__(256) void k_transpose(const double* __restrict__ A, int64_t lda,
                                                   double* __restrict__ At, int64_t ldat, int m, int n) {
  __shared__ double tile[64][65];
  const int bx = blockIdx.x * 64, by = blockIdx.y * 64;
  const int tx = threadIdx.x & 63, ty = threadIdx.x >> 6;
  for (int r = ty; r < 64; r += 4) {
    const int i = by + r, j = bx + tx;
    if (i < m && j < n) tile[r][tx] = A[(int64_t)i * lda + j];
  }
  __syncthreads();
  for (int r = ty; r < 64; r += 4) {
    const int j = bx + r, i = by + tx;
    if (j < n && i < m) At[(int64_t)j * ldat + i] = tile[tx][r];
  }
}

#define LPX_LAUNCH_STOP(kernel_, grid_, block_, stream_, stop_, ...)                                        \
  do {                                                                                                      \
    hipEvent_t lpx_stop_ = (stop_);                                                                          \
    if (lpx_stop_) hipExtLaunchKernelGGL(kernel_, grid_, block_, 0, stream_, nullptr, lpx_stop_, 0, __VA_ARGS__); \
    else hipLaunchKernelGGL(kernel_, grid_, block_, 0, stream_, __VA_ARGS__);                               \
  } while (0)
#define LPX_LAUNCH_TIMED(kernel_, grid_, block_, stream_, t0_, t1_, ...)                                    \
  do {                                                                                                      \
    hipEvent_t lpx_t0_ = (t0_), lpx_t1_ = (t1_);                                                             \
    if (lpx_t0_ && lpx_t1_) hipExtLaunchKernelGGL(kernel_, grid_, block_, 0, stream_, lpx_t0_, lpx_t1_, 0, __VA_ARGS__); \
    else hipLaunchKernelGGL(kernel_, grid_, block_, 0, stream_, __VA_ARGS__);                               \
  } while (0)
void launch_entering(const Buffers& B, int n, hipStream_t s, const LoopStart& start) {
  hipLaunchKernelGGL(k_entering, dim3(1), dim3(1024), 0, s, B.c, n, B.ctl, start);
}

void launch_entering_dantzig(const Buffers& B, int n, bool seed, hipStream_t s, const LoopStart& start) {
  hipLaunchKernelGGL(k_entering_dantzig, dim3(1), dim3(256), 0, s, B.c, n, B.ctl, seed ? 1 : 0, start);
}

void launch_ratio_gather(const Buffers& B, int m_local, int row0, const Geometry& g, int forced_e, hipStream_t s) {
  if (g.ntiles <= 0) return;
  const int nblk = (m_local + 255) / 256;
  hipLaunchKernelGGL(k_ratio_gather, dim3(nblk), dim3(256), 0, s, B.A, B.ld, B.b, m_local, row0, B.col[0],
                     B.col[1], B.partial, B.ctl, g.ntiles, forced_e);
}

void launch_reduce_partials(const Buffers& B, const Geometry& g, hipStream_t s) {
  hipLaunchKernelGGL(k_reduce_partials, dim3(1), dim3(256), 0, s, B.partial, g.ntiles, B.ctl);
}

static int finish_blocks(int64_t ld) {
  if (ld <= 4096) return 1;
  return (int)std::min<int64_t>(16, (ld + 1023) / 1024);
}

void launch_select_pivot(const Buffers& B, int n, int m_global, const Geometry& g, int forced_e, int forced_l,
                         hipStream_t s) {
  hipLaunchKernelGGL(k_select_pivot, dim3(finish_blocks(B.ld)), dim3(1024), 0, s, B.A, B.ld, n, m_global, B.b, B.c, B.prow,
                     B.partial, g.ntiles, B.perm, B.ctl, forced_e, forced_l);
}

template <int U, bool NT, bool OOP>
static void launch_update_t(const Buffers& B, int m_local, int row0, const Geometry& g, const double* prow,
                            const LpxCtl* up, double* A_out, double* b_out, hipStream_t s) {
  hipLaunchKernelGGL((k_update<U, NT, OOP>), dim3(g.nstrips * g.ntiles), dim3(256), 0, s, OOP ? A_out : B.A, B.A, B.ld,
                     m_local, row0, OOP ? b_out : B.b, B.b, prow, B.col[0], B.col[1], B.partial, up, g.rows_per_tile,
                     g.nstrips);
}

template <int U>
static void launch_update_u(const Buffers& B, int m_local, int row0, const Geometry& g, bool nt, const double* prow,
                            const LpxCtl* up, double* A_out, double* b_out, hipStream_t s) {
  const bool oop = A_out != nullptr;
  if (oop) {
    if (nt) launch_update_t<U, true, true>(B, m_local, row0, g, prow, up, A_out, b_out, s);
    else launch_update_t<U, false, true>(B, m_local, row0, g, prow, up, A_out, b_out, s);
  } else {
    if (nt) launch_update_t<U, true, false>(B, m_local, row0, g, prow, up, A_out, b_out, s);
    else launch_update_t<U, false, false>(B, m_local, row0, g, prow, up, A_out, b_out, s);
  }
}

void launch_update(const Buffers& B, int m_local, int n, int row0, const Geometry& g, bool nt, const double* prow,
                   const LpxCtl* up, double* A_out, double* b_out, hipStream_t s) {
  (void)n;
  if (g.ntiles <= 0 || g.nstrips <= 0) return;
  switch (g.U) {
    case 1: launch_update_u<1>(B, m_local, row0, g, nt, prow, up, A_out, b_out, s); break;
    case 2: launch_update_u<2>(B, m_local, row0, g, nt, prow, up, A_out, b_out, s); break;
    default: launch_update_u<4>(B, m_local, row0, g, nt, prow, up, A_out, b_out, s); break;
  }
}

void launch_propose(const Buffers& B, int n, int row0, int m_local, const Geometry& g, double* d_candidate,
                    hipStream_t s) {
  hipLaunchKernelGGL(k_propose, dim3(finish_blocks(B.ld)), dim3(1024), 0, s, B.A, B.ld, n, row0, m_local, B.b, B.partial,
                     g.ntiles, B.ctl, d_candidate);
}

static int small_blocks(int64_t ld) { return (int)std::max<int64_t>(1, std::min<int64_t>(64, (ld + 255) / 256)); }

void launch_commit(const Buffers& B, int n, int m_global, const double* d_gathered, int nranks, double* prow,
                   LpxCtl* up, int up_parity, hipStream_t s) {
  hipLaunchKernelGGL(k_commit, dim3(small_blocks(B.ld)), dim3(256), 0, s, d_gathered, nranks, n, B.ld, m_global, B.c,
                     prow, B.perm, B.ctl, up, up_parity);
}

void launch_peek(const Buffers& B, int n, int m_local, int row0, const double* prow_t, const double* col_t,
                 double* col_next, const LpxCtl* pend, double* d_candidate, hipStream_t s) {
  const int nblk = std::max(1, (m_local + 255) / 256);
  hipLaunchKernelGGL(k_peek, dim3(nblk), dim3(256), 0, s, B.A, B.ld, B.b, m_local, row0, prow_t, col_t, col_next,
                     B.partial, B.ctl, pend);
  hipLaunchKernelGGL(k_peek_pack, dim3(small_blocks(B.ld)), dim3(256), 0, s, B.A, B.ld, n, row0, B.b, prow_t, col_t,
                     B.partial, nblk, B.ctl, pend, d_candidate);
}

void launch_block_peek(const Buffers& B, const BlockRing& R, int n, int m_local, int row0, int np, double* d_candidate,
                       hipStream_t s) {
  const int nblk = std::max(1, (m_local + 255) / 256);
  hipLaunchKernelGGL(k_peek_multi, dim3(nblk), dim3(256), 0, s, B.A, B.ld, B.b, m_local, row0, R.prow, R.col, R.mp, R.up,
                     np, R.col + (int64_t)np * R.mp, R.col0 + (int64_t)np * R.mp, B.partial, B.ctl);
  hipLaunchKernelGGL(k_pack_multi, dim3(small_blocks(B.ld)), dim3(256), 0, s, B.A, B.ld, n, row0, B.b, R.prow, R.col,
                     R.mp, R.up, np, B.partial, nblk, B.ctl, d_candidate, R.row0 + (int64_t)np * B.ld);
}

void launch_block_decide(const Buffers& B, const BlockRing& R, int n, int m_global, const double* d_gathered, int nranks,
                         int slot, hipStream_t s) {
  hipLaunchKernelGGL(k_commit, dim3(small_blocks(B.ld)), dim3(256), 0, s, d_gathered, nranks, n, B.ld, m_global, B.c,
                     R.prow + (int64_t)slot * B.ld, B.perm, B.ctl, R.up + slot, 0);
}

int launch_block_chain(const Buffers& B, const BlockRing& R, int n, int m, int nb, int half, int old_half, int n_old,
                        int b_from_tableau, int seq, int dantzig, int wgs, int fences, bool trace, LpxCtl* host_snap,
                        hipStream_t s, const MgPeers* mg, hipEvent_t stop) {
  const int64_t work = std::max<int64_t>(m, B.ld);
  int G = wgs > 0 ? wgs : (int)std::min<int64_t>(64, std::max<int64_t>(1, (work + 511) / 512));
  G = std::max(1, std::min(G, kChainMaxWgs));
#ifdef LPX_WITH_VARIANTS
  const bool form2 = B.chain_form == 1 && (mg == nullptr || !mg->onehop);
#else
  const bool form2 = mg == nullptr || (B.chain_form == 1 && !mg->onehop);
#endif
  if (form2 && mg == nullptr) {
    const int64_t rows_wgs = (m + kChain2Threads - 1) / kChain2Threads;
    const int64_t cols_wgs = (std::max<int64_t>(B.ld - 256, 0) + kChain2Threads - 1) / kChain2Threads + 1;
    G = (int)std::max<int64_t>(1, std::min<int64_t>(G, std::max(rows_wgs, cols_wgs)));
  }
  const int64_t K = kBlockMax;
  const bool wide = nb > 32 || n_old > 32;
  const bool wide128 = nb > 64 || n_old > 64;
  ChainArgs P{};
  P.A = B.A; P.b = B.b; P.ld = B.ld; P.mp = R.mp; P.n = n; P.m = m;
  P.c = B.c; P.perm = B.perm; P.ctl = B.ctl;
  const int64_t ho = half * K, oo = old_half * K;
  P.prow = R.prow + ho * B.ld; P.col = R.col + ho * R.mp; P.col0 = R.col0 + ho * R.mp; P.row0 = R.row0 + ho * B.ld;
  P.own_col = R.chain_own_col + ho * R.mp; P.own_prow = R.chain_own_prow + ho * B.ld;
  P.own_dvc = R.chain_own_dvc + ho * R.mp; P.up = R.up + ho;
  P.prow_o = R.prow + oo * B.ld; P.col_o = R.col + oo * R.mp;
  P.own_col_o = R.chain_own_col + oo * R.mp; P.own_prow_o = R.chain_own_prow + oo * B.ld;
  P.own_dvc_o = R.chain_own_dvc + oo * R.mp; P.up_o = R.up + oo;
  P.n_old = n_old; P.own_b = R.chain_own_b; P.b_from_tableau = b_from_tableau; P.nb = nb;
  P.own_rs_a = R.chain_own_rs; P.own_rs_b = R.chain_own_rs + R.mp;
  P.partA = reinterpret_cast<ChainPart*>(R.chain_part_a); P.partB = reinterpret_cast<RatioRow*>(R.chain_part_b);
  P.bar = R.chain_bar + 32 * (seq & 1); P.bar_next = R.chain_bar + 32 * ((seq + 1) & 1);
  P.hand = reinterpret_cast<unsigned long long*>(R.chain_bar + 64);
  P.hand_base = (unsigned)(seq + 1) * (unsigned)kBlockMax;
  P.dantzig = dantzig; P.fences = fences; P.host_snap = host_snap; P.dbg = trace ? R.chain_dbg : nullptr;
  P.spin_max = (mg && mg->spin_max) ? mg->spin_max : (1u << 22);
#ifdef LPX_DIAG_BUILD
  static const int chain_diag = getenv("LPX_CHAIN_DIAG") ? atoi(getenv("LPX_CHAIN_DIAG")) : 0;
  P.diag = chain_diag;
#endif
  P.census = R.census;
  if (mg) {
    P.shard_row0 = mg->row0; P.m_global = mg->m_global; P.n_dev = mg->n_dev; P.dev = mg->dev;
    P.mail_slot0 = mg->mail_slot0;
    P.onehop = mg->onehop;
    for (int d = 0; d < mg->n_dev && d < kMaxDevices; ++d) {
      P.mail_peer[d] = reinterpret_cast<MgMail*>(mg->mail[d]);
      P.prow_peer[d] = mg->prow[d] + ho * B.ld;
      P.arrive_peer[d] = mg->arrive[d];
      P.candrow_peer[d] = mg->candrow[d];
      P.arrive2_peer[d] = mg->arrive2[d];
    }
    if (form2) {
      if (wide) LPX_LAUNCH_STOP((k_block_chain2_t<64, kChain2Threads, true>), dim3(G), dim3(kChain2Threads), s, stop, P);
      else LPX_LAUNCH_STOP((k_block_chain2_t<32, kChain2Threads, true>), dim3(G), dim3(kChain2Threads), s, stop, P);
    } else LPX_LAUNCH_STOP((k_block_chain_t<true, 32>), dim3(G), dim3(256), s, stop, P);
  } else if (form2) {
    P.m_global = m; P.n_dev = 1;
#ifdef LPX_CHAIN2_ONE_XCD
    G = std::min(G, 32);
    if (wide128) hipLaunchKernelGGL((k_block_decide128<kChain2Threads>), dim3(8 * G), dim3(kChain2Threads), 0, s, P);
    else if (wide) hipLaunchKernelGGL((k_block_chain2_t<64, kChain2Threads, false>), dim3(8 * G), dim3(kChain2Threads), 0, s, P);
    else hipLaunchKernelGGL((k_block_chain2_t<32, kChain2Threads, false>), dim3(8 * G), dim3(kChain2Threads), 0, s, P);
    if (stop) (void)hipEventRecord(stop, s);
#else
    if (wide128) LPX_LAUNCH_STOP((k_block_decide128<kChain2Threads>), dim3(G), dim3(kChain2Threads), s, stop, P);
    else if (wide) LPX_LAUNCH_STOP((k_block_chain2_t<64, kChain2Threads, false>), dim3(G), dim3(kChain2Threads), s, stop, P);
    else LPX_LAUNCH_STOP((k_block_chain2_t<32, kChain2Threads, false>), dim3(G), dim3(kChain2Threads), s, stop, P);
#endif
  } else {
#ifdef LPX_WITH_VARIANTS
    P.m_global = m; P.n_dev = 1;
    if (wide) LPX_LAUNCH_STOP((k_block_chain_t<false, 64>), dim3(G), dim3(256), s, stop, P);
    else LPX_LAUNCH_STOP((k_block_chain_t<false, 32>), dim3(G), dim3(256), s, stop, P);
#else
    if (stop) (void)hipEventRecord(stop, s);
#endif
  }
  return G;
}

int64_t sweep_ticket_slots(int64_t ld) { return kSweep128Ranges * std::max<int64_t>(ld / 64, 4) + 4; }
unsigned* sweep_fail_word(const BlockRing& R, int64_t ld) {
#ifdef LPX_WITH_VARIANTS
  (void)ld;
  return R.sweep_fail;
#else
  (void)R; (void)ld;
  return nullptr;
#endif
}

void preload_block_kernels(const Buffers& B, const BlockRing& R, hipStream_t s) {
  static std::atomic<unsigned> done{0};
  int dev = 0;
  if (hipGetDevice(&dev) != hipSuccess || dev < 0 || dev >= 32) return;
  if (done.fetch_or(1u << dev) & (1u << dev)) return;
  double* const A = B.A;
  const int64_t ld = B.ld;
  unsigned* const no_census = nullptr;
#define LPX_EACH_NT_OOP(X) X(true, true) X(true, false) X(false, true) X(false, false)
#define LPX_PRE_TILES(K_, NT_, OOP_) \
  hipLaunchKernelGGL((k_update_tiles<K_, NT_, OOP_>), dim3(1), dim3(256), 0, s, A, A, ld, 0, R.prow, R.col, R.mp, R.up, 0, 16, 1, no_census);
#define LPX_PRE_T2(NT_, OOP_) LPX_PRE_TILES(2, NT_, OOP_)
#define LPX_PRE_T4(NT_, OOP_) LPX_PRE_TILES(4, NT_, OOP_)
#define LPX_PRE_T8(NT_, OOP_) LPX_PRE_TILES(8, NT_, OOP_)
#define LPX_PRE_T16(NT_, OOP_) LPX_PRE_TILES(16, NT_, OOP_)
#define LPX_PRE_T32(NT_, OOP_) LPX_PRE_TILES(32, NT_, OOP_)
#define LPX_PRE_MULTI(NT_, OOP_) \
  hipLaunchKernelGGL((k_update_multi<32, NT_, OOP_>), dim3(1), dim3(256), 0, s, A, A, ld, 0, R.prow, R.col, R.mp, R.up, 0, 64, 1, no_census, 0, 0);
#define LPX_PRE_STEADY(NT_, OOP_) \
  hipLaunchKernelGGL((k_sweep32_steady<NT_, OOP_>), dim3(1), dim3(256), 0, s, A, A, ld, 0, R.prow, R.col, R.mp, R.up, 0, 48, 1);
#define LPX_PRE_PIPE(NT_, OOP_) \
  hipLaunchKernelGGL((k_sweep64_pipe<NT_, OOP_>), dim3(1), dim3(512), 0, s, A, A, ld, 0, R.prow, R.col, R.mp, R.up, 0, 48, 1);
#define LPX_PRE_DMA(NT_, OOP_) \
  hipLaunchKernelGGL((k_sweep32_dma<NT_, OOP_>), dim3(1), dim3(256), 0, s, A, A, ld, 0, R.prow, R.col, R.mp, R.up, 0, 2, 1, 1, R.zeros, 0);
  LPX_EACH_NT_OOP(LPX_PRE_T2) LPX_EACH_NT_OOP(LPX_PRE_T4) LPX_EACH_NT_OOP(LPX_PRE_T8) LPX_EACH_NT_OOP(LPX_PRE_T16)
  LPX_EACH_NT_OOP(LPX_PRE_T32) LPX_EACH_NT_OOP(LPX_PRE_MULTI)
#ifdef LPX_WITH_VARIANTS
  LPX_EACH_NT_OOP(LPX_PRE_STEADY) LPX_EACH_NT_OOP(LPX_PRE_PIPE) LPX_EACH_NT_OOP(LPX_PRE_DMA)
#endif
#define LPX_PRE_PULL(NT_, OOP_) \
  hipLaunchKernelGGL((k_sweep32_pull<NT_, OOP_>), dim3(1), dim3(256), 0, s, A, A, ld, 0, R.prow, R.col, R.mp, R.up, 0, 1, R.col_packed, R.tickets, (long long*)nullptr);
  if (R.tickets && R.col_packed) {
    LPX_EACH_NT_OOP(LPX_PRE_PULL)
    hipLaunchKernelGGL(k_pack_multipliers<32>, dim3(1), dim3(256), 0, s, R.col, R.mp, R.up, 0, 0, R.col_packed, R.tickets, 0, (long long*)nullptr);
    hipLaunchKernelGGL(k_pack_multipliers<64>, dim3(1), dim3(256), 0, s, R.col, R.mp, R.up, 0, 0, R.col_packed, R.tickets, 0, (long long*)nullptr);
#ifdef LPX_WITH_VARIANTS
#define LPX_PRE_PULL64(NT_, OOP_) \
    hipLaunchKernelGGL((k_sweep64_pull<NT_, OOP_>), dim3(1), dim3(256), 0, s, A, A, ld, 0, R.prow, R.up, 0, 1, R.col_packed, R.tickets, (sweep_fail_word)(R, ld));
    LPX_EACH_NT_OOP(LPX_PRE_PULL64)
#undef LPX_PRE_PULL64
#endif
#define LPX_PRE_ONE64(NT_, OOP_) \
    hipLaunchKernelGGL((k_sweep64_one<NT_, OOP_>), dim3(1), dim3(256), 0, s, A, A, ld, 0, R.prow, R.up, 0, 1, R.col_packed, R.tickets, (long long*)nullptr);
    LPX_EACH_NT_OOP(LPX_PRE_ONE64)
#undef LPX_PRE_ONE64
#if LPX_FUSED
    hipLaunchKernelGGL(k_pack_multipliers_mfma, dim3(1), dim3(256), 0, s, R.col, R.mp, R.up, 0, 0, R.col_packed, R.tickets, 0, (long long*)nullptr, 0);
#ifdef LPX_WITH_VARIANTS
#define LPX_PRE_MFMA64(NT_, OOP_) \
    hipLaunchKernelGGL((k_sweep64_mfma<NT_, OOP_>), dim3(1), dim3(256), 0, s, A, A, ld, 0, R.prow, R.up, 0, 1, R.col_packed, R.tickets);
    LPX_EACH_NT_OOP(LPX_PRE_MFMA64)
#undef LPX_PRE_MFMA64
#endif
#define LPX_PRE_MFMA642(NT_, OOP_) \
    hipLaunchKernelGGL((k_sweep64_mfma2<NT_, OOP_>), dim3(1), dim3(256), 0, s, A, A, ld, 0, R.prow, R.up, 0, 1, R.col_packed, R.tickets, 33, (long long*)nullptr);
    LPX_EACH_NT_OOP(LPX_PRE_MFMA642)
#undef LPX_PRE_MFMA642
    hipLaunchKernelGGL(k_pack_multipliers_mfma128, dim3(1), dim3(256), 0, s, R.col, R.mp, R.up, 0, 0, R.col_packed, R.tickets, 0, (long long*)nullptr);
#define LPX_PRE_MFMA128(NT_, OOP_) \
    hipLaunchKernelGGL((k_sweep128_mfma<NT_, OOP_>), dim3(1), dim3(256), 0, s, A, A, ld, 0, R.prow, R.up, 0, 0, R.col_packed, R.tickets, 1);
    LPX_EACH_NT_OOP(LPX_PRE_MFMA128)
#undef LPX_PRE_MFMA128
#endif
  }
#undef LPX_PRE_PULL
#undef LPX_PRE_DMA
#undef LPX_PRE_PIPE
#undef LPX_PRE_STEADY
#undef LPX_PRE_MULTI
#undef LPX_PRE_T32
#undef LPX_PRE_T16
#undef LPX_PRE_T8
#undef LPX_PRE_T4
#undef LPX_PRE_T2
#undef LPX_PRE_TILES
#undef LPX_EACH_NT_OOP
  hipLaunchKernelGGL(k_block_fixup, dim3(1, 1, 3), dim3(256), 0, s, A, ld, 0, 0, 0, B.b, R.prow, R.col, R.col0, R.row0,
                     R.mp, R.up, 0, B.b, (long long*)nullptr, (double*)nullptr, (double*)nullptr);
  hipLaunchKernelGGL(k_block_fixup_scatter, dim3(1, 1, 2), dim3(256), 0, s, A, ld, 0, 0, (const double*)nullptr, (const double*)nullptr,
                     R.mp, R.up, 0, (long long*)nullptr);
  ChainArgs P{};
  P.ctl = B.ctl; P.up = R.up; P.nb = 0;
  P.bar = R.chain_bar; P.bar_next = R.chain_bar + 32;
  P.spin_max = 1u << 22;
#ifdef LPX_WITH_VARIANTS
  hipLaunchKernelGGL((k_block_chain_t<false, 32>), dim3(1), dim3(256), 0, s, P);
  hipLaunchKernelGGL((k_block_chain_t<false, 64>), dim3(1), dim3(256), 0, s, P);
#endif
  hipLaunchKernelGGL((k_block_chain_t<true, 32>), dim3(1), dim3(256), 0, s, P);
  hipLaunchKernelGGL((k_block_chain2_t<32, kChain2Threads, false>), dim3(1), dim3(kChain2Threads), 0, s, P);
  hipLaunchKernelGGL((k_block_chain2_t<64, kChain2Threads, false>), dim3(1), dim3(kChain2Threads), 0, s, P);
  hipLaunchKernelGGL((k_block_chain2_t<32, kChain2Threads, true>), dim3(1), dim3(kChain2Threads), 0, s, P);
  hipLaunchKernelGGL((k_block_decide128<kChain2Threads>), dim3(1), dim3(kChain2Threads), 0, s, P);
  (void)hipGetLastError();
}

int chain_blocks_per_cu() {
  int nb = 0;
  int nw = 0;
  int n2 = 0, n3 = 0;
  if (hipOccupancyMaxActiveBlocksPerMultiprocessor(&nb, (k_block_chain_t<true, 32>), 256, 0) != hipSuccess ||
      hipOccupancyMaxActiveBlocksPerMultiprocessor(&nw, (k_block_chain2_t<32, kChain2Threads, false>), kChain2Threads, 0) != hipSuccess ||
      hipOccupancyMaxActiveBlocksPerMultiprocessor(&n2, (k_block_chain2_t<64, kChain2Threads, true>), kChain2Threads, 0) != hipSuccess ||
      hipOccupancyMaxActiveBlocksPerMultiprocessor(&n3, (k_block_decide128<kChain2Threads>), kChain2Threads, 0) != hipSuccess) {
    (void)hipGetLastError();
    nb = nw = n2 = n3 = 1;
  }
  return std::max(1, std::min(std::min(nb, nw), std::min(n2, n3)));
}

template <int K>
static void launch_sweep_tiles(const Buffers& B, const BlockRing& R, int m_local, int kmax, int rows_per_tile, bool nt,
                               const double* A_src, hipStream_t s) {
  const int nstrips = (int)((B.ld + 511) / 512);
  const int ntiles = (m_local + rows_per_tile - 1) / rows_per_tile;
  const dim3 grid(nstrips * ntiles), block(256);
#define LPX_LAUNCH_SWEEP(NT_, OOP_)                                                                              \
  hipLaunchKernelGGL((k_update_tiles<K, NT_, OOP_>), grid, block, 0, s, B.A, A_src, B.ld, m_local, R.prow, R.col, \
                     R.mp, R.up, kmax, rows_per_tile, nstrips, R.census ? R.census + kChainMaxWgs : nullptr)
  if (A_src) { if (nt) LPX_LAUNCH_SWEEP(true, true); else LPX_LAUNCH_SWEEP(false, true); }
  else { if (nt) LPX_LAUNCH_SWEEP(true, false); else LPX_LAUNCH_SWEEP(false, false); }
#undef LPX_LAUNCH_SWEEP
}

template <int K>
static void launch_sweep_k(const Buffers& B, const BlockRing& R, int m_local, int kmax, int rows_per_wg, bool nt,
                           const double* A_src, hipStream_t s, int complement = 0, int slot0 = 0) {
  const int nstrips = (int)((B.ld + 511) / 512);
  const int ngroups = (m_local + rows_per_wg - 1) / rows_per_wg;
  const dim3 grid(nstrips * ngroups), block(256);
#define LPX_LAUNCH_SWEEP(NT_, OOP_)                                                                              \
  hipLaunchKernelGGL((k_update_multi<K, NT_, OOP_>), grid, block, 0, s, B.A, A_src, B.ld, m_local, R.prow, R.col, \
                     R.mp, R.up, kmax, rows_per_wg, nstrips, R.census ? R.census + kChainMaxWgs : nullptr, complement, \
                     slot0)
  if (A_src) { if (nt) LPX_LAUNCH_SWEEP(true, true); else LPX_LAUNCH_SWEEP(false, true); }
  else { if (nt) LPX_LAUNCH_SWEEP(true, false); else LPX_LAUNCH_SWEEP(false, false); }
#undef LPX_LAUNCH_SWEEP
}

static hipStream_t pack_stream(const FixSide* side, hipStream_t s) { return (side && side->stream && side->packed) ? side->stream : s; }
static hipEvent_t pack_stop(const FixSide* side) { return (side && side->stream && side->packed) ? side->packed : nullptr; }
static void pack_done(const FixSide* side, hipStream_t s) {
  if (pack_stop(side)) (void)hipStreamWaitEvent(s, side->packed, 0);
}

static void launch_sweep_pull(const Buffers& B, const BlockRing& R, int m_local, int kmax, bool nt, const double* A_src,
                              hipStream_t s, int slots = 512, const FixSide* side = nullptr, hipEvent_t t0 = nullptr,
                              hipEvent_t t1 = nullptr) {
  const int nstrips_full = (int)(B.ld / 512);
  const int nbt = m_local / 4;
  const int G = std::max(1, std::min(nbt, slots / std::max(1, nstrips_full)));
  LPX_LAUNCH_STOP(k_pack_multipliers<32>, dim3((nbt + 7) / 8), dim3(256), pack_stream(side, s), pack_stop(side), R.col, R.mp, R.up, kmax, nbt, R.col_packed,
                     R.tickets, nstrips_full * 4, (long long*)nullptr);
  pack_done(side, s);
  const dim3 grid(nstrips_full * G), block(256);
#define LPX_LAUNCH_PULL(NT_, OOP_)                                                                                \
  LPX_LAUNCH_TIMED((k_sweep32_pull<NT_, OOP_>), grid, block, s, t0, t1, B.A, A_src, B.ld, m_local, R.prow, R.col, R.mp, \
                   R.up, kmax, nstrips_full, R.col_packed, R.tickets, R.clk)
  if (A_src) { if (nt) LPX_LAUNCH_PULL(true, true); else LPX_LAUNCH_PULL(false, true); }
  else { if (nt) LPX_LAUNCH_PULL(true, false); else LPX_LAUNCH_PULL(false, false); }
#undef LPX_LAUNCH_PULL
}

static void launch_sweep64_one(const Buffers& B, const BlockRing& R, int m_local, int kmax, bool nt, const double* A_src,
                               hipStream_t s, int slots = 512, const FixSide* side = nullptr, hipEvent_t t0 = nullptr,
                               hipEvent_t t1 = nullptr) {
  const int nstrips_full = (int)(B.ld / 512);
  const int ngroups = nstrips_full * 2;
  const int nbt = m_local / 4;
  const int G = std::max(1, std::min(nbt, slots / std::max(1, ngroups)));
  LPX_LAUNCH_STOP(k_pack_multipliers<64>, dim3((nbt + 3) / 4), dim3(256), pack_stream(side, s), pack_stop(side), R.col, R.mp, R.up, kmax, nbt, R.col_packed,
                     R.tickets, nstrips_full * 8, (long long*)nullptr);
  pack_done(side, s);
  const dim3 grid(ngroups * G), block(256);
#define LPX_LAUNCH_ONE64(NT_, OOP_)                                                                               \
  LPX_LAUNCH_TIMED((k_sweep64_one<NT_, OOP_>), grid, block, s, t0, t1, B.A, A_src, B.ld, m_local, R.prow, R.up, kmax, \
                   nstrips_full, R.col_packed, R.tickets, R.clk)
  if (A_src) { if (nt) LPX_LAUNCH_ONE64(true, true); else LPX_LAUNCH_ONE64(false, true); }
  else { if (nt) LPX_LAUNCH_ONE64(true, false); else LPX_LAUNCH_ONE64(false, false); }
#undef LPX_LAUNCH_ONE64
}

#if LPX_FUSED
static void launch_sweep64_mfma(const Buffers& B, const BlockRing& R, int m_local, int kmax, bool nt, const double* A_src,
                                hipStream_t s, int slots = 256, bool two_waves = false, int kmin = 33, const FixSide* side = nullptr,
                                hipEvent_t t0 = nullptr, hipEvent_t t1 = nullptr) {
  const int nstrips_full = (int)(B.ld / 512);
  const int ngroups = nstrips_full * 2;
  const int ntiles = m_local / 16;
  const int G = std::max(1, std::min(ntiles, slots / std::max(1, ngroups)));
  LPX_LAUNCH_STOP(k_pack_multipliers_mfma, dim3(ntiles), dim3(256), pack_stream(side, s), pack_stop(side), R.col, R.mp, R.up, kmax, ntiles, R.col_packed,
                     R.tickets, nstrips_full * 8, two_waves ? (long long*)nullptr : R.clk, two_waves ? 1 : 0);
  pack_done(side, s);
  if (two_waves) {
    const int ng2 = nstrips_full * 4;
    const int G2 = std::max(1, std::min(ntiles, 2 * slots / std::max(1, ng2)));
    const dim3 grid2(ng2 * G2), block2(256);
#define LPX_LAUNCH_MFMA642(NT_, OOP_)                                                                               \
    LPX_LAUNCH_TIMED((k_sweep64_mfma2<NT_, OOP_>), grid2, block2, s, t0, t1, B.A, A_src, B.ld, m_local, R.prow, R.up, kmax, \
                     nstrips_full, R.col_packed, R.tickets, kmin, R.clk)
    if (A_src) { if (nt) LPX_LAUNCH_MFMA642(true, true); else LPX_LAUNCH_MFMA642(false, true); }
    else { if (nt) LPX_LAUNCH_MFMA642(true, false); else LPX_LAUNCH_MFMA642(false, false); }
#undef LPX_LAUNCH_MFMA642
    return;
  }
#ifdef LPX_WITH_VARIANTS
  const dim3 grid(ngroups * G), block(256);
#define LPX_LAUNCH_MFMA64(NT_, OOP_)                                                                               \
  hipLaunchKernelGGL((k_sweep64_mfma<NT_, OOP_>), grid, block, 0, s, B.A, A_src, B.ld, m_local, R.prow, R.up, kmax, \
                     nstrips_full, R.col_packed, R.tickets)
  if (A_src) { if (nt) LPX_LAUNCH_MFMA64(true, true); else LPX_LAUNCH_MFMA64(false, true); }
  else { if (nt) LPX_LAUNCH_MFMA64(true, false); else LPX_LAUNCH_MFMA64(false, false); }
#undef LPX_LAUNCH_MFMA64
#else
  (void)G;
#endif
}
#endif

#if LPX_FUSED
static void launch_sweep128_mfma(const Buffers& B, const BlockRing& R, int m_local, int kmax, bool nt, const double* A_src,
                                 hipStream_t s, int cus, const FixSide* side, hipEvent_t t0, hipEvent_t t1) {
  const int nsub = (int)(B.ld / 64);
  const int ntiles = m_local / 16;
  const int nranges = std::max(1, std::min(kSweep128Ranges, ntiles));
  LPX_LAUNCH_STOP(k_pack_multipliers_mfma128, dim3(ntiles), dim3(256), pack_stream(side, s), pack_stop(side), R.col, R.mp, R.up, kmax,
                  ntiles, R.col_packed, R.tickets, 1 + nsub * nranges, R.clk);
  pack_done(side, s);
  const dim3 grid(std::max(1, std::min(2 * cus, nsub * nranges))), block(256);
#define LPX_LAUNCH_MFMA128(NT_, OOP_)                                                                                    \
  LPX_LAUNCH_TIMED((k_sweep128_mfma<NT_, OOP_>), grid, block, s, t0, t1, B.A, A_src, B.ld, m_local, R.prow, R.up, kmax, nsub, \
                   R.col_packed, R.tickets, nranges)
  if (A_src) { if (nt) LPX_LAUNCH_MFMA128(true, true); else LPX_LAUNCH_MFMA128(false, true); }
  else { if (nt) LPX_LAUNCH_MFMA128(true, false); else LPX_LAUNCH_MFMA128(false, false); }
#undef LPX_LAUNCH_MFMA128
}
#endif

static int choose_sweep_rows(int m_local, int64_t ld, int K, int cus) {
  const int64_t nstrips = (ld + 511) / 512;
  const int64_t slots = std::max(1, 2 * cus);
  const int prologue_rows = std::max(8, (K * 3) / 2);
  int best_rows = kSweepChunk;
  int64_t best_cost = INT64_MAX;
  const int max_rows = (int)std::min<int64_t>(4096, (((int64_t)1 << 32) - 1) / (ld * 8) / kSweepChunk * kSweepChunk);
  for (int rows = kSweepChunk; rows <= std::max(kSweepChunk, max_rows); rows += kSweepChunk) {
    const int64_t groups = (m_local + rows - 1) / rows;
    const int64_t rounds = (nstrips * groups + slots - 1) / slots;
    const int64_t want_rounds = (int64_t)m_local * nstrips >= 3 * slots * kSweepChunk ? 3 : 1;
    const int64_t cost = std::max(rounds, want_rounds) * (rows + prologue_rows);
    if (cost < best_cost || (cost == best_cost && rows > best_rows)) { best_cost = cost; best_rows = rows; }
    if (groups == 1) break;
  }
  return best_rows;
}

const char* sweep_kernel_name(int code) {
  switch (code) {
    case kSweepTiles: return "k_update_tiles";
    case kSweepMulti: return "k_update_multi";
    case kSweepSteady: return "k_sweep32_steady";
    case kSweepPipe64: return "k_sweep64_pipe";
    case kSweepDma: return "k_sweep32_dma";
    case kSweepPull: return "k_sweep32_pull";
    case kSweepPull64: return "k_sweep64_pull";
    case kSweepOne64: return "k_sweep64_one";
    case kSweepMfma64: return "k_sweep64_mfma";
    case kSweepMfma642: return "k_sweep64_mfma2";
    case kSweepMfma128: return "k_sweep128_mfma";
    default: return "";
  }
}

#ifdef LPX_WITH_VARIANTS
#define LPX_VARIANT_PART 6
#include "variants/lpx_variants.inc"
#undef LPX_VARIANT_PART
#endif

int launch_block_sweep(const Buffers& B, const BlockRing& R, int n, int m_local, int row0, int K, int rows_per_wg,
                       bool nt, hipStream_t s, const double* A_src, const double* b_src, hipEvent_t after_sweep,
                       int cus, int form, int* kernel_used, const FixSide* side, hipEvent_t stop, hipEvent_t before_sweep) {
  int used = kSweepNone;
  if (kernel_used) *kernel_used = used;
  if (K < 1) {
    if (before_sweep) (void)hipEventRecord(before_sweep, s);
    if (after_sweep) (void)hipEventRecord(after_sweep, s);
    if (stop) (void)hipEventRecord(stop, s);
    return 0;
  }
  bool timed_own = false, bracket_open = false;
  auto bracket = [&]() { if (before_sweep && !bracket_open) { (void)hipEventRecord(before_sweep, s); bracket_open = true; } };
  if (cus <= 0) {
    int dev = 0;
    (void)hipGetDevice(&dev);
    if (hipDeviceGetAttribute(&cus, hipDeviceAttributeMultiprocessorCount, dev) != hipSuccess || cus <= 0) cus = 256;
  }
  const bool side_fix = side && side->stream && R.fix_col && R.fix_row;
  if (side_fix) (void)hipStreamWaitEvent(side->stream, side->ready, 0);
  else side = nullptr;
  if (K <= 16) {
    bracket();
    int rows_per_tile = rows_per_wg <= 0 ? 16 : rows_per_wg;
    rows_per_tile = std::max(8, std::min(rows_per_tile, kSweepMaxRows)) & ~7;
    while (rows_per_tile > 8 && (int64_t)rows_per_tile * B.ld * 8 >= (int64_t)1 << 32) rows_per_tile -= 8;
    if (K <= 2) launch_sweep_tiles<2>(B, R, m_local, K, rows_per_tile, nt, A_src, s);
    else if (K <= 4) launch_sweep_tiles<4>(B, R, m_local, K, rows_per_tile, nt, A_src, s);
    else if (K <= 8) launch_sweep_tiles<8>(B, R, m_local, K, rows_per_tile, nt, A_src, s);
    else launch_sweep_tiles<16>(B, R, m_local, K, rows_per_tile, nt, A_src, s);
    rows_per_wg = rows_per_tile;
    used = kSweepTiles;
  } else if (K > 64) {
    bool mfma128 = false;
#if LPX_FUSED
    mfma128 = form != 3 && m_local % 16 == 0 && m_local >= 16 && B.ld % 512 == 0 && 16 * B.ld * 8 + 1024 < ((int64_t)1 << 32) &&
              R.tickets && R.col_packed;
#endif
    if (mfma128) {
#if LPX_FUSED
      timed_own = before_sweep && after_sweep;
      if (!timed_own) bracket();
      launch_sweep128_mfma(B, R, m_local, K, nt, A_src, s, cus, side, timed_own ? before_sweep : nullptr, timed_own ? after_sweep : nullptr);
#endif
      rows_per_wg = 16;
      used = kSweepMfma128;
    } else {
      bracket();
      int rows = choose_sweep_rows(m_local, B.ld, 32, cus);
      while (rows > kSweepChunk && (int64_t)rows * B.ld * 8 >= (int64_t)1 << 32) rows -= kSweepChunk;
      for (int slot0 = 0; slot0 < K; slot0 += 32) launch_sweep_k<32>(B, R, m_local, K, rows, nt, slot0 == 0 ? A_src : nullptr, s, 0, slot0);
      rows_per_wg = rows;
      used = kSweepMulti;
    }
  } else if (K > 32) {
    const int nstrips_full = (int)(B.ld / 512);
    const bool geom = m_local % 4 == 0 && nstrips_full >= 1 && 3 * B.ld * 8 + 1024 < ((int64_t)1 << 32);
#ifdef LPX_WITH_VARIANTS
    const bool pull = geom && form != 1 && R.tickets && R.col_packed;
    const bool pipe = geom && !pull && K == 64;
    const bool one = pull && form != 2;
    [[maybe_unused]] const bool mfma_form = form == 0 || form == 4;
    const bool mfma2 = form == 0;
#else
    const bool pull = geom && R.tickets && R.col_packed;
    const bool pipe = false;
    const bool one = pull;
    [[maybe_unused]] const bool mfma_form = form != 3;
    const bool mfma2 = true;
#endif
    bool mfma = false;
#if LPX_FUSED
    mfma = one && mfma_form && m_local % 16 == 0 && 16 * B.ld * 8 + 1024 < ((int64_t)1 << 32);
#endif
    int rows64 = 0;
    const bool whole = mfma && mfma2 && B.ld % 512 == 0;
    timed_own = whole && before_sweep && after_sweep;
    if (!timed_own) bracket();
    if (mfma) {
#if LPX_FUSED
      launch_sweep64_mfma(B, R, m_local, K, nt, A_src, s, cus, mfma2, whole ? 1 : 33, side, timed_own ? before_sweep : nullptr,
                          timed_own ? after_sweep : nullptr);
#endif
      rows64 = 16;
    } else if (one) {
      launch_sweep64_one(B, R, m_local, K, nt, A_src, s, 2 * cus, side);
      rows64 = 4;
    }
#ifdef LPX_WITH_VARIANTS
    else if (pull) {
      launch_sweep64_pull(B, R, m_local, K, nt, A_src, s, 2 * cus);
      rows64 = 4;
    } else if (pipe) {
      rows64 = rows_per_wg > 0 ? std::max(4, rows_per_wg / 4 * 4) : choose_pipe_rows(m_local, nstrips_full, cus);
      while (rows64 > 4 && (int64_t)rows64 * B.ld * 8 >= (int64_t)1 << 32) rows64 -= 4;
      launch_sweep64_pipe(B, R, m_local, K, rows64, nt, A_src, s);
    }
#endif
    const int complement = pull ? 34 : (pipe ? 65 : 0);
    int rows = choose_sweep_rows(m_local, B.ld, 32, cus);
    while (rows > kSweepChunk && (int64_t)rows * B.ld * 8 >= (int64_t)1 << 32) rows -= kSweepChunk;
    if (!whole) {
      launch_sweep_k<32>(B, R, m_local, K, rows, nt, A_src, s, complement, 0);
      launch_sweep_k<32>(B, R, m_local, K, rows, nt, nullptr, s, complement, 32);
    }
    rows_per_wg = (pull || pipe) ? rows64 : rows;
    used = mfma ? (mfma2 ? kSweepMfma642 : kSweepMfma64) : one ? kSweepOne64 : (pull ? kSweepPull64 : (pipe ? kSweepPipe64 : kSweepMulti));
  } else if (K < kMaxBlock && !(m_local % 4 == 0 && B.ld >= 512)) {
    bracket();
    const int64_t nstrips = (B.ld + 511) / 512;
    int rows_per_tile = 16;
    for (int rows : {64, 32})
      if ((int64_t)((m_local + rows - 1) / rows) * nstrips >= 4096) { rows_per_tile = rows; break; }
    while (rows_per_tile > 8 && (int64_t)rows_per_tile * B.ld * 8 >= (int64_t)1 << 32) rows_per_tile -= 8;
    launch_sweep_tiles<32>(B, R, m_local, K, rows_per_tile, nt, A_src, s);
    rows_per_wg = rows_per_tile;
    used = kSweepTiles;
  } else {
    if (rows_per_wg <= 0) rows_per_wg = choose_sweep_rows(m_local, B.ld, K, cus);
    rows_per_wg = std::max(kSweepChunk, (rows_per_wg + kSweepChunk - 1) / kSweepChunk * kSweepChunk);
    while (rows_per_wg > kSweepChunk && (int64_t)rows_per_wg * B.ld * 8 >= (int64_t)1 << 32) rows_per_wg -= kSweepChunk;
    const bool wide32 = 3 * B.ld * 8 + 1024 >= ((int64_t)1 << 32);
    const bool pullable = m_local % 4 == 0 && B.ld >= 512 && !wide32 && R.zeros && R.tickets && R.col_packed;
    bool done = false;
#ifdef LPX_WITH_VARIANTS
    const bool variant32 = m_local % 4 == 0 && B.ld >= 512 && (form == 1 || form == 2 || !pullable);
#else
    const bool variant32 = false;
#endif
    timed_own = !variant32 && pullable && B.ld % 512 == 0 && before_sweep && after_sweep;
    if (!timed_own) bracket();
#ifdef LPX_WITH_VARIANTS
    if (variant32) {
      int rows48 = choose_pipe_rows(m_local, (int)(B.ld / 512), 2 * cus, 48);
      while (rows48 > 4 && (int64_t)rows48 * B.ld * 8 >= (int64_t)1 << 32) rows48 -= 4;
      if (form == 2 && pullable) {
        launch_sweep_dma(B, R, m_local, K, rows48, nt, A_src, s, 2 * cus);
        used = kSweepDma;
      } else {
        launch_sweep_steady(B, R, m_local, K, rows48, nt, A_src, s);
        used = kSweepSteady;
      }
      if (B.ld % 512 != 0) launch_sweep_k<32>(B, R, m_local, K, rows_per_wg, nt, A_src, s, 1);
      rows_per_wg = rows48;
      done = true;
    }
#endif
    if (!done && pullable) {
      launch_sweep_pull(B, R, m_local, K, nt, A_src, s, 2 * cus, side, timed_own ? before_sweep : nullptr, timed_own ? after_sweep : nullptr);
      used = kSweepPull;
      if (B.ld % 512 != 0) launch_sweep_k<32>(B, R, m_local, K, rows_per_wg, nt, A_src, s, 1);
      rows_per_wg = 4;
    } else if (!done) {
      launch_sweep_k<32>(B, R, m_local, K, rows_per_wg, nt, A_src, s);
      used = kSweepMulti;
    }
  }
  if (kernel_used) *kernel_used = used;
  if (after_sweep && !timed_own) { bracket(); (void)hipEventRecord(after_sweep, s); }
  const bool probed = used == kSweepPull || used == kSweepPull64 || used == kSweepOne64 || used == kSweepMfma64 || used == kSweepMfma642;
  const int gx = (int)((std::max<int64_t>(m_local, B.ld) + 255) / 256);
  if (side_fix) {
    LPX_LAUNCH_STOP(k_block_fixup, dim3(gx, (K + kFixChunk - 1) / kFixChunk, 3), dim3(256), side->stream, side->done, B.A, B.ld, n, m_local, row0,
                    B.b, R.prow, R.col, R.col0, R.row0, R.mp, R.up, K, b_src ? b_src : B.b, (long long*)nullptr, R.fix_col, R.fix_row);
    (void)hipStreamWaitEvent(s, side->done, 0);
  }
  const bool memset_behind = !probed && R.clk && used != kSweepMfma128;
  hipEvent_t last_stop = memset_behind ? nullptr : stop;
  if (side_fix) {
    LPX_LAUNCH_STOP(k_block_fixup_scatter, dim3(gx, (K + kFixChunk - 1) / kFixChunk, 2), dim3(256), s, last_stop, B.A, B.ld, m_local, row0,
                    (const double*)R.fix_col, (const double*)R.fix_row, R.mp, R.up, K, probed ? R.clk : (long long*)nullptr);
  } else {
    LPX_LAUNCH_STOP(k_block_fixup, dim3(gx, (K + kFixChunk - 1) / kFixChunk, 3), dim3(256), s, last_stop, B.A, B.ld, n, m_local, row0, B.b, R.prow, R.col,
                    R.col0, R.row0, R.mp, R.up, K, b_src ? b_src : B.b, probed ? R.clk : (long long*)nullptr, (double*)nullptr, (double*)nullptr);
  }
  if (memset_behind) {
    (void)hipMemsetAsync(R.clk, 0, 256, s);
    if (stop) (void)hipEventRecord(stop, s);
  }
  return rows_per_wg;
}

void launch_fill_column(double* A, int64_t ld, int m, int col, double value, hipStream_t s) {
  if (m <= 0) return;
  hipLaunchKernelGGL(k_fill_column, dim3((m + 255) / 256), dim3(256), 0, s, A, ld, m, col, value);
}

void launch_drop_column(double* A, int64_t ld, int m, int n_old, int col, hipStream_t s) {
  if (m <= 0) return;
  hipLaunchKernelGGL(k_drop_column, dim3(m), dim3(256), 0, s, A, ld, m, n_old, col);
}

void launch_restore_objective(const Buffers& B, int n, const RestoreEntry* d_entries, int n_entries, hipStream_t s) {
  const int blocks = n > 0 ? (n + 255) / 256 : 1;
  hipLaunchKernelGGL(k_restore_objective, dim3(blocks), dim3(256), 0, s, B.A, B.ld, B.b, B.c, n, d_entries,
                     n_entries, B.ctl);
}

void launch_checksum(const Buffers& B, int m_local, int n, int row0, unsigned long long* d_out3, hipStream_t s) {
  hipLaunchKernelGGL(k_checksum, dim3(1024), dim3(256), 0, s, B.A, B.ld, m_local, n, row0, B.b, B.c, d_out3);
}

void launch_transpose(const double* dA, int64_t lda, double* dAt, int64_t ldat, int m, int n, hipStream_t s) {
  if (m <= 0 || n <= 0) return;
  hipLaunchKernelGGL(k_transpose, dim3((n + 63) / 64, (m + 63) / 64), dim3(256), 0, s, dA, lda, dAt, ldat, m, n);
}

#include "lpx_batch.inc"

}
}
```

### linear_programming_solver_amd/csrc/lpx_launchers.inc

```
void launch_entering(const Buffers& B, int n, hipStream_t s, const LoopStart& start = LoopStart{});
void launch_entering_dantzig(const Buffers& B, int n, bool seed, hipStream_t s, const LoopStart& start = LoopStart{});
void launch_ratio_gather(const Buffers& B, int m_local, int row0, const Geometry& g, int forced_e, hipStream_t s);
void launch_reduce_partials(const Buffers& B, const Geometry& g, hipStream_t s);
void launch_select_pivot(const Buffers& B, int n, int m_global, const Geometry& g, int forced_e, int forced_l,
                         hipStream_t s);
void launch_update(const Buffers& B, int m_local, int n, int row0, const Geometry& g, bool nontemporal,
                   const double* prow, const LpxCtl* up, double* A_out, double* b_out, hipStream_t s);
void launch_propose(const Buffers& B, int n, int row0, int m_local, const Geometry& g, double* d_candidate,
                    hipStream_t s);
void launch_commit(const Buffers& B, int n, int m_global, const double* d_gathered, int nranks, double* prow,
                   LpxCtl* up, int up_parity, hipStream_t s);
void launch_peek(const Buffers& B, int n, int m_local, int row0, const double* prow_t, const double* col_t,
                 double* col_next, const LpxCtl* pend, double* d_candidate, hipStream_t s);
void launch_block_peek(const Buffers& B, const BlockRing& R, int n, int m_local, int row0, int np, double* d_candidate,
                       hipStream_t s);
void launch_block_decide(const Buffers& B, const BlockRing& R, int n, int m_global, const double* d_gathered, int nranks,
                         int slot, hipStream_t s);
int launch_block_chain(const Buffers& B, const BlockRing& R, int n, int m, int nb, int half, int old_half, int n_old,
                        int b_from_tableau, int seq, int dantzig, int wgs, int fences, bool trace, LpxCtl* host_snap,
                        hipStream_t s, const MgPeers* mg = nullptr, hipEvent_t stop = nullptr);
void preload_block_kernels(const Buffers& B, const BlockRing& R, hipStream_t s);
unsigned* sweep_fail_word(const BlockRing& R, int64_t ld);
int64_t sweep_ticket_slots(int64_t ld);
int chain_blocks_per_cu();
const char* sweep_kernel_name(int code);
int launch_block_sweep(const Buffers& B, const BlockRing& R, int n, int m_local, int row0, int K, int rows_per_wg,
                       bool nt, hipStream_t s, const double* A_src = nullptr, const double* b_src = nullptr,
                       hipEvent_t after_sweep = nullptr, int cus = 0, int form = 0, int* kernel_used = nullptr,
                       const FixSide* side = nullptr, hipEvent_t stop = nullptr, hipEvent_t before_sweep = nullptr);
void launch_fill_column(double* A, int64_t ld, int m, int col, double value, hipStream_t s);
void launch_drop_column(double* A, int64_t ld, int m, int n_old, int col, hipStream_t s);
void launch_restore_objective(const Buffers& B, int n, const RestoreEntry* d_entries, int n_entries, hipStream_t s);
void launch_checksum(const Buffers& B, int m_local, int n, int row0, unsigned long long* d_out3, hipStream_t s);
hipError_t launch_batch_simplex(const BatchArgs& a, hipStream_t s);
int batch_blocks_per_cu(int threads, int lds_bytes);
hipError_t launch_batch_solve(const BatchSolveArgs& a, hipStream_t s);
int batch_solve_blocks_per_cu(int threads, int lds_bytes);
hipError_t launch_batch_scenarios(const BatchScenarioArgs& a, hipStream_t s);
int batch_scenarios_blocks_per_cu(int threads, int lds_bytes);
hipError_t launch_scenarios_crash(const ScenarioCrashArgs& a, hipStream_t s);
hipError_t launch_batch_resolve(const BatchResolveArgs& a, hipStream_t s);
int batch_resolve_blocks_per_cu(int threads, int lds_bytes);
void launch_transpose(const double* dA, int64_t lda, double* dAt, int64_t ldat, int m, int n, hipStream_t s);
```

### linear_programming_solver_amd/csrc/lpx_sweeps.inc

```
constexpr int kSweepMaxRows = 128;
#ifndef LPX_SWEEP_NBUF
#define LPX_SWEEP_NBUF 2
#endif

__device__ __forceinline__ int ring_count(const LpxCtl* __restrict__ ring, int kcap, int kmax, int* sh_np) {
  if (threadIdx.x < 64) {
    const int lane = threadIdx.x;
    const bool ok = lane < kcap && lane < kmax && ring[lane].do_update != 0;
    const unsigned long long mask = __ballot(ok);
    if (lane == 0) *sh_np = (~mask == 0ull) ? 64 : (__ffsll((long long)~mask) - 1);
  }
  __syncthreads();
  return *sh_np;
}
__device__ __forceinline__ int ring_count128(const LpxCtl* __restrict__ ring, int kmax, int* sh_np) {
  if (threadIdx.x < 64) {
    const int lane = threadIdx.x;
    const unsigned long long m0 = __ballot(lane < kmax && ring[lane].do_update != 0);
    const unsigned long long m1 = __ballot(lane + 64 < kmax && ring[lane + 64].do_update != 0);
    const int n0 = (~m0 == 0ull) ? 64 : (__ffsll((long long)~m0) - 1);
    const int n1 = (~m1 == 0ull) ? 64 : (__ffsll((long long)~m1) - 1);
    if (lane == 0) *sh_np = n0 < 64 ? n0 : 64 + n1;
  }
  __syncthreads();
// ... 637 lines not shown
template <bool NT, bool OOP>
__global__ __launch_bounds__(256, 2) void k_sweep64_one(double* __restrict__ A, const double* __restrict__ Asrc,
                                                        int64_t ld, int m_local,
                                                        const double* __restrict__ prow_ring,
                                                        const LpxCtl* __restrict__ ring, int kmax, int nstrips_full,
                                                        const double* __restrict__ col_packed,
                                                        unsigned* __restrict__ tickets, long long* __restrict__ clk) {
  constexpr int K = 64, RB = kDmaRB, NS = kPullNS, NM = kPullNM;
  sweep_front_stamp(clk);
  constexpr int kOps = 2 + 2 + 1 + RB;
  constexpr int kAhead = RB + (NS - 1) * kOps;
  static_assert(kAhead <= 60 && RB == 4, "vmcnt is six bits wide; a batch is two two-row DMAs");
  __shared__ __attribute__((aligned(16))) char sm[4 * kOneWaveBytes];
  const int np = ring_count(ring, K, kmax, reinterpret_cast<int*>(sm));
  __syncthreads();
  if (np <= 32) return;
  const int lane = threadIdx.x & 63;
  const int wave = __builtin_amdgcn_readfirstlane((int)(threadIdx.x >> 6));
  const int ngroups = nstrips_full * 2;
  const int grp = (ngroups % 8 == 0)
                      ? (int)(((blockIdx.x >> 3) + (blockIdx.x & 7) * (unsigned)(ngroups / 8)) % (unsigned)ngroups)
                      : (int)(blockIdx.x % (unsigned)ngroups);
  const int sub = grp * 4 + wave;
  const int nbt = m_local / RB;
  unsigned* const ctr = tickets + sub * 32;
  const int64_t row_bytes = ld * 8;
  const int64_t batch_bytes = RB * row_bytes;
  char* const dst_base = reinterpret_cast<char*>(A + sub * 64);
  const char* const src_base = OOP ? reinterpret_cast<const char*>(Asrc + sub * 64) : dst_base;
  const uint32_t rb32 = (uint32_t)row_bytes;
  const uint32_t off_r = (uint32_t)(lane >> 5) * rb32 + (uint32_t)(lane & 31) * 16u;
  const uint32_t off_m = (uint32_t)lane * 16u;
  const uint32_t off_x = (uint32_t)lane * 8u;
  char* const stage = sm + wave * kOneWaveBytes;
  char* const mult = stage + NS * kOneSlotBytes;
  const uint32_t lds_stage = lds_addr_of(stage), lds_mult = lds_addr_of(mult);
  auto issue = [&](int t, int it) {
    const char* const base = src_base + (int64_t)t * batch_bytes;
    const char* const mbase = reinterpret_cast<const char*>(col_packed) + (int64_t)t * 2048;
    dma_batch2m2<NT>(base, off_r, off_r + 2 * rb32,
                     (uint32_t)__builtin_amdgcn_readfirstlane((int)(lds_stage + (uint32_t)((it % NS) * kOneSlotBytes))),
                     mbase, off_m, (uint32_t)__builtin_amdgcn_readfirstlane((int)(lds_mult + (uint32_t)((it % NM) * 2048))));
  };

  unsigned tk[NS];
  int bq[NS + 1];
#pragma unroll
  for (int u = 0; u < NS; ++u) ticket_pull(tk[u], ctr);
  dma_wait<0>();
#pragma unroll
  for (int u = 0; u < NS; ++u) {
    bq[u] = ticket_take(tk[u]);
    if (bq[u] < nbt) issue(bq[u], u);
  }
#pragma unroll
  for (int u = 0; u < NS; ++u) ticket_pull(tk[u], ctr);
  double pr[K];
#pragma unroll
  for (int s = 0; s < K; ++s) {
    pr[s] = prow_ring[(int64_t)s * ld + sub * 64 + lane];
    if (s >= np) pr[s] = 0.0;
  }
  dma_wait<0>();

  int full = 0;
#pragma unroll 1
  for (int i0 = 0;; i0 += NS) {
    if (bq[0] >= nbt) break;
#pragma unroll
    for (int u = 0; u < NS; ++u) {
      const int i = i0 + u;
      const int t = bq[0];
      if (t < nbt) {
        if (full >= NS) dma_wait<kAhead>(); else if (i >= NS) dma_wait<0>();
        bq[NS] = ticket_take(tk[u]);
        const char* const slot = stage + u * kOneSlotBytes + off_x;
        double x[RB];
#pragma unroll
        for (int r = 0; r < RB; ++r) x[r] = *reinterpret_cast<const double*>(slot + r * 512);
        const bool more = bq[NS] < nbt;
        if (more) issue(bq[NS], i + NS);
        else asm volatile("s_waitcnt lgkmcnt(0)" ::: "memory");
        ticket_pull(tk[u], ctr);
        full = more ? full + 1 : 0;
        sweep_apply_one<K>(x, pr, reinterpret_cast<const double*>(mult + (i % NM) * 2048));
        char* const out = dst_base + (int64_t)t * batch_bytes;
#pragma unroll
        for (int r = 0; r < RB; ++r) {
          double* q = reinterpret_cast<double*>(out + (off_x + (uint32_t)r * rb32));
          if (NT) __builtin_nontemporal_store(x[r], q); else *q = x[r];
        }
      } else {
        bq[NS] = INT_MAX;
      }
#pragma unroll
      for (int k = 0; k < NS; ++k) bq[k] = bq[k + 1];
    }
  }
  dma_wait<0>();
}

#if LPX_FUSED
typedef double d4v __attribute__((ext_vector_type(4)));

__global__ __launch_bounds__(256) void k_pack_multipliers_mfma(const double* __restrict__ col_ring, int64_t mp,
                                                               const LpxCtl* __restrict__ ring, int kmax, int ntiles,
                                                               double* __restrict__ colM, unsigned* __restrict__ tickets,
                                                               int nsub, long long* __restrict__ clk, int pairs) {
  __shared__ int sh_np;
  const int np = ring_count(ring, 64, kmax, &sh_np);
  if (clk && blockIdx.x < 8 && threadIdx.x == 0) {
    const unsigned x = xcc_id() & 7u;
    clk[x * 4 + 0] = __builtin_amdgcn_s_memtime(); clk[x * 4 + 1] = wall_clock64();
  }
  if (blockIdx.x == 0)
    for (int u = threadIdx.x; u < nsub; u += 256) tickets[u * 32] = 0u;
  const int tile = blockIdx.x;
  if (tile >= ntiles) return;
#pragma unroll
  for (int q = 0; q < 4; ++q) {
    const int idx = q * 256 + threadIdx.x;
    const int g = idx >> 6, l = idx & 63, k = l >> 4, i = l & 15;
    const int s = 4 * g + k;
    const double c = s < np ? col_ring[(int64_t)s * mp + (int64_t)tile * 16 + i] : 0.0;
    colM[(int64_t)tile * 1024 + (pairs ? (g >> 1) * 128 + 2 * l + (g & 1) : idx)] = -c;
  }
}

#ifdef LPX_WITH_VARIANTS
#define LPX_VARIANT_PART 4
#include "variants/lpx_variants.inc"
#undef LPX_VARIANT_PART
#endif


constexpr int kMfma2LdsBytes = 2 * 16 * 4 * 64 * 8;
static_assert(2 * kMfma2LdsBytes <= 160 * 1024, "two workgroups per CU");
typedef unsigned v2u __attribute__((ext_vector_type(2)));
typedef unsigned v4u __attribute__((ext_vector_type(4)));
template <bool NT, bool OOP>
__global__ __launch_bounds__(256, 2) void k_sweep64_mfma2(double* A, const double* Asrc,
                                                          int64_t ld, int m_local,
                                                          const double* __restrict__ prow_ring,
                                                          const LpxCtl* __restrict__ ring, int kmax, int nstrips_full,
                                                          const double* colM,
                                                          unsigned* tickets, int kmin, long long* clk) {
  constexpr int NG = 16, CT = 4;
  constexpr int kRsrcWord3 = 0x00020000;
  constexpr int kAuxNt = NT ? 2 : 0;
  __shared__ __attribute__((aligned(16))) double sh_b[2 * NG * CT * 64];
  __shared__ int sh_np;
  sweep_front_stamp(clk);
  const int np = ring_count(ring, 64, kmax, &sh_np);
  if (np < kmin) return;
  const int lane = threadIdx.x & 63;
  const int wave = __builtin_amdgcn_readfirstlane((int)(threadIdx.x >> 6));
  const int ngroups = nstrips_full * 4;
  const int grp = (ngroups % 8 == 0)
                      ? (int)(((blockIdx.x >> 3) + (blockIdx.x & 7) * (unsigned)(ngroups / 8)) % (unsigned)ngroups)
                      : (int)(blockIdx.x % (unsigned)ngroups);
  const int ntiles = 2 * (m_local / 16);
  unsigned* const ctr = tickets + grp * 32;
  const int64_t row_bytes = ld * 8;
  char* const dst_base = reinterpret_cast<char*>(A + grp * 128);
  const char* const src_base = OOP ? reinterpret_cast<const char*>(Asrc + grp * 128) : dst_base;
  const uint32_t rb32 = (uint32_t)row_bytes;
  const uint32_t off_c = (uint32_t)(lane >> 4) * rb32 + (uint32_t)(lane & 15) * 8u;
  const uint32_t off_a = (uint32_t)lane * 8u;
  for (int q = wave; q < 2 * NG * CT; q += 4) {
    const int h = q / (NG * CT), g = (q / CT) % NG, ct = q % CT;
    const int s = 4 * g + (lane >> 4);
    sh_b[q * 64 + lane] = s < np ? prow_ring[(int64_t)s * ld + grp * 128 + h * 64 + ct * 16 + (lane & 15)] : 0.0;
  }
  __syncthreads();
  auto load_tile = [&](int t, d4v (&c)[CT], double (&a)[NG]) {
    const int tt = max(0, min(t, ntiles - 1));
    const __amdgpu_buffer_rsrc_t rc = __builtin_amdgcn_make_buffer_rsrc(
        const_cast<char*>(src_base) + (int64_t)(tt >> 1) * 16 * row_bytes + (tt & 1) * 512, 0, -1, kRsrcWord3);
#pragma unroll
    for (int r = 0; r < 4; ++r)
#pragma unroll
      for (int ct = 0; ct < CT; ++ct)
        c[ct][r] = __builtin_bit_cast(double, __builtin_amdgcn_raw_buffer_load_b64(rc, off_c + (uint32_t)ct * 128u,
                                                                                    (int)((uint32_t)(4 * r) * rb32), kAuxNt));
    const __amdgpu_buffer_rsrc_t ra = __builtin_amdgcn_make_buffer_rsrc(
        const_cast<double*>(colM) + (int64_t)(tt >> 1) * 1024, 0, -1, kRsrcWord3);
#pragma unroll
    for (int p = 0; p < NG / 2; ++p) {
      const v4u x = __builtin_amdgcn_raw_buffer_load_b128(ra, 2u * off_a + (uint32_t)(p & 3) * 1024u, (p >> 2) * 4096, 0);
      a[2 * p] = __builtin_bit_cast(double, v2u{x[0], x[1]});
      a[2 * p + 1] = __builtin_bit_cast(double, v2u{x[2], x[3]});
    }
  };
#define LPX_MFMA_FENCE __builtin_amdgcn_sched_barrier(0)
  auto work_tile = [&](int t, d4v (&c)[CT], const double (&a)[NG]) {
    const double* const bl = sh_b + (max(0, min(t, ntiles - 1)) & 1) * (NG * CT * 64) + lane;
#pragma unroll
    for (int g = 0; g < NG; ++g)
#pragma unroll
      for (int ct = 0; ct < CT; ++ct) {
        c[ct] = __builtin_amdgcn_mfma_f64_16x16x4f64(a[g], bl[(g * CT + ct) * 64], c[ct], 0, 0, 0);
      }
    __builtin_amdgcn_sched_group_barrier(0x100, 2, 0);
#pragma unroll
    for (int g = 0; g < NG; ++g) {
      if (g + 1 < NG) __builtin_amdgcn_sched_group_barrier(0x100, 2, 0);
      __builtin_amdgcn_sched_group_barrier(0x008, 4, 0);
    }
    const int tt = max(0, min(t, ntiles - 1));
    char* const out = dst_base + (int64_t)(tt >> 1) * 16 * row_bytes + (tt & 1) * 512;
    const __amdgpu_buffer_rsrc_t rd = __builtin_amdgcn_make_buffer_rsrc(out, 0, __builtin_amdgcn_readfirstlane((unsigned)t < (unsigned)ntiles ? -1 : 0), kRsrcWord3);
#pragma unroll
    for (int r = 0; r < 4; ++r)
#pragma unroll
      for (int ct = 0; ct < CT; ++ct)
        __builtin_amdgcn_raw_buffer_store_b64(__builtin_bit_cast(v2u, (double)c[ct][r]), rd, off_c + (uint32_t)ct * 128u,
                                              (int)((uint32_t)(4 * r) * rb32), kAuxNt);
  };
  constexpr int kStepOps = 16 + 8 + 16;
  static_assert(kStepOps + 1 <= 63, "vmcnt is six bits wide");
  auto take = [&](unsigned& tk) -> int {
    asm volatile("s_waitcnt vmcnt(%0)" :: "n"(kStepOps + 1) : "memory");
    return ticket_take(tk);
  };
  d4v c0[CT], c1[CT], c2[CT];
  double a0[NG], a1[NG], a2[NG];
  int t0, t1;
  unsigned k0, k1, k2;
  {
    ticket_pull(k0, ctr); ticket_pull(k1, ctr);
    asm volatile("s_waitcnt vmcnt(0)" ::: "memory");
    t0 = ticket_take(k0); t1 = ticket_take(k1);
  }
  if (t0 >= ntiles) return;
  load_tile(t0, c0, a0);
  load_tile(t1, c1, a1);
  ticket_pull(k2, ctr);
  __builtin_amdgcn_s_waitcnt(0x0F70);
#pragma unroll 1
  do {
    ticket_pull(k0, ctr);
    const int t2 = take(k2);
    load_tile(t2, c2, a2);
    LPX_MFMA_FENCE;
    work_tile(t0, c0, a0);
    LPX_MFMA_FENCE;
    ticket_pull(k1, ctr);
    const int t3 = take(k0);
    load_tile(t3, c0, a0);
    LPX_MFMA_FENCE;
    work_tile(t1, c1, a1);
    LPX_MFMA_FENCE;
    ticket_pull(k2, ctr);
    const int t4 = take(k1);
    load_tile(t4, c1, a1);
    LPX_MFMA_FENCE;
    work_tile(t2, c2, a2);
    LPX_MFMA_FENCE;
    t0 = t3; t1 = t4;
  } while (t0 < ntiles);
}

#undef LPX_MFMA_FENCE
__global__ __launch_bounds__(256) void k_pack_multipliers_mfma128(const double* __restrict__ col_ring, int64_t mp,
                                                                  const LpxCtl* __restrict__ ring, int kmax, int ntiles,
                                                                  double* __restrict__ colM, unsigned* __restrict__ tickets, int nctr,
                                                                  long long* __restrict__ clk) {
  __shared__ int sh_np;
  const int np = ring_count128(ring, kmax, &sh_np);
  if (blockIdx.x == 0)
    for (int u = threadIdx.x; u < nctr; u += 256) tickets[u * 32] = 0u;
  if (clk && blockIdx.x == 0 && threadIdx.x < 32) clk[threadIdx.x] = 0;
  const int tile = blockIdx.x;
  if (tile >= ntiles) return;
#pragma unroll
  for (int q = 0; q < 8; ++q) {
    const int idx = q * 256 + threadIdx.x;
    const int g = idx >> 6, l = idx & 63, k = l >> 4, i = l & 15;
    const int s = 4 * g + k;
    const double c = s < np ? col_ring[(int64_t)s * mp + (int64_t)tile * 16 + i] : 0.0;
    colM[(int64_t)tile * 2048 + (g >> 1) * 128 + 2 * l + (g & 1)] = -c;
  }
}
#define LPX_MFMA_FENCE __builtin_amdgcn_sched_barrier(0)
template <bool NT, bool OOP>
__global__ __launch_bounds__(256, 2) void k_sweep128_mfma(double* A, const double* Asrc,
                                                          int64_t ld, int m_local,
                                                          const double* __restrict__ prow_ring,
                                                          const LpxCtl* __restrict__ ring, int kmax, int nsub,
                                                          const double* colM,
                                                          unsigned* tickets, int nranges) {
  constexpr int NG = 32, CT = 4;
  constexpr int kRsrcWord3 = 0x00020000;
  constexpr int kAuxNt = NT ? 2 : 0;
  __shared__ __attribute__((aligned(16))) double sh_b[NG * CT * 64];
  __shared__ int sh_np, sh_chunk;
  const int np = ring_count128(ring, kmax, &sh_np);
  if (np < 1 && !OOP) return;
  const int lane = threadIdx.x & 63;
  const int wave = __builtin_amdgcn_readfirstlane((int)(threadIdx.x >> 6));
  const int rowblocks = m_local / 16;
  const int per_range = (rowblocks + nranges - 1) / nranges;
  const int nchunks = nsub * nranges;
  const int64_t row_bytes = ld * 8;
  const uint32_t rb32 = (uint32_t)row_bytes;
  const uint32_t off_c = (uint32_t)(lane >> 4) * rb32 + (uint32_t)(lane & 15) * 8u;
  const uint32_t off_a = (uint32_t)lane * 8u;
// ... 372 lines not shown
```

Before: 24570.

## Fuse multiplier packing into block chain kernel, skip separate pack launch

The chain kernel now writes each negated column multiplier directly into the MFMA-packed layout and zero-pads the unused slots. It also resets the sweep tickets and clock words. Because of this, the sweep launchers skip the separate k_pack_multipliers kernel when a pack layout is selected. The aim is to remove one kernel launch and one extra pass over the column ring per block. The cost is extra scattered stores inside the latency-critical chain kernel, plus an edge-case change to the sweep's early-exit condition for out-of-place launches.

Result: no change. 24480 (median of 2 runs) (-0.4%).

```diff
diff --git a/linear_programming_solver_amd/csrc/lpx_decisions.inc b/linear_programming_solver_amd/csrc/lpx_decisions.inc
--- a/linear_programming_solver_amd/csrc/lpx_decisions.inc
+++ b/linear_programming_solver_amd/csrc/lpx_decisions.inc
@@ -253,7 +253,17 @@
   unsigned long long* arrive2_peer[kMaxDevices];
   unsigned spin_max;
   int diag;
+  int pack_layout;
+  double* col_packed;
+  unsigned* tickets;
+  int pack_tickets;
+  long long* pack_clk;
 };
+enum PackLayout { kPackNone = 0, kPackMfma64 = 1, kPackMfma128 = 2 };
+__device__ __forceinline__ int64_t pack_row_offset(int layout, int i) { return (int64_t)(i >> 4) * (1024 * layout) + 2 * (i & 15); }
+__device__ __forceinline__ int pack_slot_offset(int s) { return (s >> 3) * 128 + 32 * (s & 3) + ((s >> 2) & 1); }
+template <int KB, bool MG>
+__device__ constexpr bool chain2_packs() { return LPX_FUSED && !MG && KB > 32; }
 
 template <int KB>
 __device__ __forceinline__ int chain_restart(const unsigned long long* sh_mask) {
@@ -888,6 +898,24 @@
 #else
 #define LPX_OWN_STORE(p_, x_) (*(p_) = (x_))
 #endif
+template <int KB, int NT, bool MG>
+__device__ __forceinline__ void chain2_pack_tail(const ChainArgs& P, int np) {
+  if constexpr (chain2_packs<KB, MG>()) {
+    const int layout = P.pack_layout;
+    if (!layout) return;
+#ifdef LPX_CHAIN2_ONE_XCD
+    const int gid = (blockIdx.x >> 3) * NT + threadIdx.x, T = (gridDim.x >> 3) * NT;
+#else
+    const int gid = blockIdx.x * NT + threadIdx.x, T = gridDim.x * NT;
+#endif
+    const int kpad = 64 * layout;
+    for (int i = gid; i < P.m; i += T) {
+      double* const dst = P.col_packed + pack_row_offset(layout, i);
+      for (int s = np; s < kpad; ++s) dst[pack_slot_offset(s)] = -0.0;
+    }
+  }
+}
+#define LPX_C2_RETURN(np_) do { chain2_pack_tail<KB, NT, MG>(P, (np_)); return; } while (0)
 template <int KB, int NT, bool MG>
 __device__ __forceinline__ void block_chain2_body(const ChainArgs& P) {
   static_assert(KB == 32 || KB == 64 || KB == 128, "ring half of 32, 64 or 128 slots");
@@ -935,11 +963,17 @@
   if (lst && lead) { lst[0] = wall_clock64(); lst[3] = P.hand_base / (unsigned)kBlockMax; }
 #endif
   if (lead) st_agent(reinterpret_cast<int32_t*>(P.bar_next), 0);
+  if constexpr (chain2_packs<KB, MG>()) {
+    if (P.pack_layout && bid == (unsigned)(G - 1)) {
+      for (int u = tid; u < P.pack_tickets; u += NT) P.tickets[u * 32] = 0u;
+      if (P.pack_clk && tid < 32) P.pack_clk[tid] = 0;
+    }
+  }
   int e = ctl->e_next;
   if (ctl->status != kRunning || e < 0 || nb < 1) {
     if (book && nb >= 1) P.up[0].do_update = 0;
     if (book) chain_publish(ctl, P.host_snap);
-    return;
+    LPX_C2_RETURN(0);
   }
   if (tid < 2 * KB) {
     sh_pe[tid] = 0.0; sh_cs[tid] = 0.0; sh_dv[tid] = 0.0; sh_p[tid] = 1.0; sh_bl[tid] = 0.0;
@@ -1121,6 +1155,8 @@
       LPX_C2_STAMP(9)
       st_agent(&P.col[(int64_t)s * mp + i], a);
       LPX_OWN_STORE(&P.own_col[(int64_t)s * mp + i], a);
+      if constexpr (chain2_packs<KB, MG>())
+        if (P.pack_layout) P.col_packed[pack_row_offset(P.pack_layout, i) + pack_slot_offset(s)] = -a;
       if (i == gid) { a_first = a; b_first = bi; }
       const double rt = ratio_of(a, bi);
       if (rt < best.ratio) {
@@ -1162,7 +1198,7 @@
       lds_barrier();
       if (sh_fail) {
         if (book) { ctl->status = 7 ; ctl->reserved = sh_fail + 1000 * s; chain_publish(ctl, P.host_snap); }
-        return;
+        LPX_C2_RETURN(s);
       }
     }
     if (P.dbg && lead) P.dbg[s * LPX_C2_STRIDE + 3] = wall_clock64();
@@ -1226,28 +1262,28 @@
         win_b = lane_f64(theirs_b, wl);
       }
       lds_barrier();
-      if (sh_fail) { if (book) { ctl->status = 7; ctl->reserved = sh_fail + 1000 * s; chain_publish(ctl, P.host_snap); } return; }
+      if (sh_fail) { if (book) { ctl->status = 7; ctl->reserved = sh_fail + 1000 * s; chain_publish(ctl, P.host_snap); } LPX_C2_RETURN(s); }
     }
     if (w.row == INT_MAX || !(w.ratio < kInf)) {
       if (book) {
         ctl->status = 1; ctl->do_update = 0; ctl->l = -1; ctl->ratio = w.ratio; P.up[s].do_update = 0;
         chain_publish(ctl, P.host_snap);
       }
-      return;
+      LPX_C2_RETURN(s);
     }
     if (max_pivots >= 0 && pivots >= max_pivots) {
       if (book) {
         ctl->status = 9 ; ctl->do_update = 0; P.up[s].do_update = 0;
         chain_publish(ctl, P.host_snap);
       }
-      return;
+      LPX_C2_RETURN(s);
     }
     LPX_C2_STAMP(12)
     const int l = w.row;
     const double p = win_p, raw_b = win_b;
     if (p == 0.0) {
       if (book) { ctl->status = 8; ctl->do_update = 0; P.up[s].do_update = 0; chain_publish(ctl, P.host_snap); }
-      return;
+      LPX_C2_RETURN(s);
     }
     int rb;
     {
@@ -1285,7 +1321,7 @@
           if (P.fences & 2) __builtin_amdgcn_fence(__ATOMIC_ACQUIRE, "");
         }
         lds_barrier();
-        if (sh_fail) { if (book) { ctl->status = 7; ctl->reserved = sh_fail + 1000 * s; chain_publish(ctl, P.host_snap); } return; }
+        if (sh_fail) { if (book) { ctl->status = 7; ctl->reserved = sh_fail + 1000 * s; chain_publish(ctl, P.host_snap); } LPX_C2_RETURN(s); }
       }
     }
     double x = 0.0, cj = 0.0;
@@ -1486,7 +1522,7 @@
         sh_hand[tid] = (unsigned)rec;
       }
       lds_barrier();
-      if (sh_fail) { if (book) { ctl->status = 7; ctl->reserved = sh_fail + 1000 * s; chain_publish(ctl, P.host_snap); } return; }
+      if (sh_fail) { if (book) { ctl->status = 7; ctl->reserved = sh_fail + 1000 * s; chain_publish(ctl, P.host_snap); } LPX_C2_RETURN(s + 1); }
       e_next = (int)sh_hand[0] - 2;
       have_rec = e_next >= 0;
     }
@@ -1499,7 +1535,7 @@
       target += (unsigned)G;
       if (!grid_barrier(P.bar, target, &sh_fail, P.fences, P.spin_max)) {
         if (book) { ctl->status = 7; chain_publish(ctl, P.host_snap); }
-        return;
+        LPX_C2_RETURN(s + 1);
       }
       RatioRow m2 = rr_none();
       if (tid < G) { m2.ratio = ld_agent(&P.partB[tid].ratio); m2.row = ld_agent(&P.partB[tid].row); }
@@ -1520,7 +1556,7 @@
     }
     if (e_next < 0 || s + 1 == nb) {
       if (book) chain_publish(ctl, P.host_snap);
-      return;
+      LPX_C2_RETURN(s + 1);
     }
     e = e_next;
     lds_barrier();
@@ -1535,6 +1571,7 @@
 __global__ __launch_bounds__(NT) void k_block_decide128(const ChainArgs P) {
   block_chain2_body<128, NT, false>(P);
 }
+#undef LPX_C2_RETURN
 #undef LPX_C2_STAMP
 #undef LPX_C2_STRIDE
 #undef LPX_CHAIN_STEP_A
diff --git a/linear_programming_solver_amd/csrc/lpx_dispatch.cpp b/linear_programming_solver_amd/csrc/lpx_dispatch.cpp
--- a/linear_programming_solver_amd/csrc/lpx_dispatch.cpp
+++ b/linear_programming_solver_amd/csrc/lpx_dispatch.cpp
@@ -46,9 +46,12 @@
 }
 int launch_block_chain(const Buffers& B, const BlockRing& R, int n, int m, int nb, int half, int old_half, int n_old,
                        int b_from_tableau, int seq, int dantzig, int wgs, int fences, bool trace, LpxCtl* host_snap,
-                       hipStream_t s, const MgPeers* mg, hipEvent_t stop) {
+                       hipStream_t s, const MgPeers* mg, hipEvent_t stop, int pack_layout) {
   return LPX_PICK(B, launch_block_chain)(B, R, n, m, nb, half, old_half, n_old, b_from_tableau, seq, dantzig, wgs, fences, trace,
-                                  host_snap, s, mg, stop);
+                                  host_snap, s, mg, stop, pack_layout);
+}
+int sweep_pack_layout(const Buffers& B, const BlockRing& R, int m_local, int K, int form) {
+  return LPX_PICK(B, sweep_pack_layout)(B, R, m_local, K, form);
 }
 void preload_block_kernels(const Buffers& B, const BlockRing& R, hipStream_t s) {
   plain::preload_block_kernels(B, R, s);
@@ -60,9 +63,10 @@
 const char* sweep_kernel_name(int code) { return plain::sweep_kernel_name(code); }
 int launch_block_sweep(const Buffers& B, const BlockRing& R, int n, int m_local, int row0, int K, int rows_per_wg,
                        bool nt, hipStream_t s, const double* A_src, const double* b_src, hipEvent_t after_sweep, int cus,
-                       int form, int* kernel_used, const FixSide* side, hipEvent_t stop, hipEvent_t before_sweep) {
+                       int form, int* kernel_used, const FixSide* side, hipEvent_t stop, hipEvent_t before_sweep,
+                       int packed_layout) {
   return LPX_PICK(B, launch_block_sweep)(B, R, n, m_local, row0, K, rows_per_wg, nt, s, A_src, b_src, after_sweep, cus,
-                                         form, kernel_used, side, stop, before_sweep);
+                                         form, kernel_used, side, stop, before_sweep, packed_layout);
 }
 void launch_fill_column(double* A, int64_t ld, int m, int col, double value, hipStream_t s) {
   plain::launch_fill_column(A, ld, m, col, value, s);
diff --git a/linear_programming_solver_amd/csrc/lpx_engine.cpp b/linear_programming_solver_amd/csrc/lpx_engine.cpp
--- a/linear_programming_solver_amd/csrc/lpx_engine.cpp
+++ b/linear_programming_solver_amd/csrc/lpx_engine.cpp
@@ -633,7 +633,8 @@
 }
 
 int launch_sweep_profiled(lpx_state* s, int K, hipStream_t stream, const Buffers& B, const lpxk::BlockRing& R,
-                                 const double* A_src, const double* b_src, const lpxk::FixSide* side, hipEvent_t stop) {
+                                 const double* A_src, const double* b_src, const lpxk::FixSide* side, hipEvent_t stop,
+                                 int packed_layout) {
   const bool sample = s->prof > 0 && (s->prof_seq++ % s->prof) == 0;
   if (sample) {
     if (s->ev_used + 2 > s->ev.size()) {
@@ -651,14 +652,14 @@
                                                 s->nontemporal, stream, A_src, b_src,
                                                 sample ? s->ev[s->ev_used + 1] : nullptr, cus,
                                                 (int)s->opt[LPX_OPT_SWEEP_FORM], &kernel_used, side, stop,
-                                                sample ? s->ev[s->ev_used] : nullptr);
+                                                sample ? s->ev[s->ev_used] : nullptr, packed_layout);
   s->info.sweep_kernel = kernel_used;
   if (sample) s->ev_used += 2;
   HIP_TRY(hipGetLastError());
   return 0;
 }
-static int launch_sweep_profiled(lpx_state* s, int K) {
-  return launch_sweep_profiled(s, K, s->stream, s->B, s->R, nullptr, nullptr, nullptr, nullptr);
+static int launch_sweep_profiled(lpx_state* s, int K, int packed_layout = 0) {
+  return launch_sweep_profiled(s, K, s->stream, s->B, s->R, nullptr, nullptr, nullptr, nullptr, packed_layout);
 }
 
 lpxk::BlockRing ring_half(const lpx_state* s, int h) {
@@ -800,22 +801,24 @@
     if (nb <= 0) return 1;
     const int h = k & 1;
     Buffers Brd = s->B;
+    const bool probing = max_pivots >= 0 && decided == max_pivots;
+    const int pack = probing ? 0 : lpxk::sweep_pack_layout(s->B, ring_half(s, h), s->m, nb, (int)s->opt[LPX_OPT_SWEEP_FORM]);
     if (serial) {
       if (k >= 1) HIP_TRY(hipStreamWaitEvent(s->ov_chain, s->ev_ov_sweep[h ^ 1], 0));
       Brd.A = Abuf[h];
       Brd.b = bbuf[h];
       s->info.chain_wgs = lpxk::launch_block_chain(Brd, s->R, s->n, s->m, nb, h, h ^ 1, 0, 1, s->chain_seq++, s->pricing == 1,
-                                                   chain_wgs, fences, trace, d_snap + h, s->ov_chain, nullptr, s->ev_ov_chain[h]);
+                                                   chain_wgs, fences, trace, d_snap + h, s->ov_chain, nullptr, s->ev_ov_chain[h], pack);
     } else {
       if (k >= 2) HIP_TRY(hipStreamWaitEvent(s->ov_chain, s->ev_ov_sweep[h], 0));
       Brd.A = Abuf[k == 0 ? 0 : (k - 1) & 1];
       Brd.b = bbuf[k == 0 ? 0 : (k - 1) & 1];
       s->info.chain_wgs = lpxk::launch_block_chain(Brd, s->R, s->n, s->m, nb, h, h ^ 1, k > 0 ? nb_prev : 0, k == 0,
                                                    s->chain_seq++, s->pricing == 1, chain_wgs, fences, trace, d_snap + h,
-                                                   s->ov_chain, nullptr, s->ev_ov_chain[h]);
+                                                   s->ov_chain, nullptr, s->ev_ov_chain[h], pack);
     }
     s->chain_nb_last = nb;
-    if (max_pivots >= 0 && decided == max_pivots) {
+    if (probing) {
       decided += nb;
       return 0;
     }
@@ -825,7 +828,7 @@
     Bdst.b = bbuf[h ^ 1];
     const lpxk::FixSide side{fix_mode > 0 ? s->ov_fix[fix_mode] : nullptr, s->ev_ov_chain[h], s->ev_ov_fix[h], s->ev_ov_pack[h]};
     if (int rc = launch_sweep_profiled(s, nb, s->ov_sweep, Bdst, ring_half(s, h), Abuf[h], bbuf[h], fix_mode > 0 ? &side : nullptr,
-                                       s->ev_ov_sweep[h])) return rc;
+                                       s->ev_ov_sweep[h], pack)) return rc;
     decided += nb;
     nb_prev = nb;
     nblk = k + 1;
@@ -883,9 +886,12 @@
   if (fused) HIP_TRY(hipHostGetDevicePointer((void**)&d_snap, s->h_snap, 0));
   auto issue_block = [&](int slot) -> int {
     const int nb = block_len(K, max_pivots, decided);
+    const bool probe_only = max_pivots >= 0 && decided == max_pivots;
+    int pack = 0;
     if (fused && nb > 0) {
+      if (!probe_only) pack = lpxk::sweep_pack_layout(s->B, s->R, s->m, nb, (int)s->opt[LPX_OPT_SWEEP_FORM]);
       s->info.chain_wgs = lpxk::launch_block_chain(s->B, s->R, s->n, s->m, nb, 0, 0, 0, 1, s->chain_seq++, s->pricing == 1,
-                                                   chain_wgs, fences, trace, d_snap + slot, s->stream);
+                                                   chain_wgs, fences, trace, d_snap + slot, s->stream, nullptr, nullptr, pack);
       s->chain_nb_last = nb;
     } else {
       for (int k = 0; k < nb; k++) {
@@ -894,10 +900,9 @@
         if (s->pricing == 1) lpxk::launch_entering_dantzig(s->B, s->n, false, s->stream);
       }
     }
-    const bool probe_only = max_pivots >= 0 && decided == max_pivots;
     decided += nb;
     if (nb > 0 && !probe_only) {
-      if (int rc = launch_sweep_profiled(s, nb)) return rc;
+      if (int rc = launch_sweep_profiled(s, nb, pack)) return rc;
     }
     if (!fused)
       HIP_TRY(hipMemcpyAsync(&h2[slot], s->B.ctl, sizeof(LpxCtl), hipMemcpyDeviceToHost, s->stream));
diff --git a/linear_programming_solver_amd/csrc/lpx_internal.h b/linear_programming_solver_amd/csrc/lpx_internal.h
--- a/linear_programming_solver_amd/csrc/lpx_internal.h
+++ b/linear_programming_solver_amd/csrc/lpx_internal.h
@@ -100,7 +100,8 @@
 int device_cus(const lpx_state* s);
 int launch_sweep_profiled(lpx_state* s, int K, hipStream_t stream, const Buffers& B, const lpxk::BlockRing& R,
                           const double* A_src, const double* b_src, const lpxk::FixSide* side = nullptr,
-                          hipEvent_t stop = nullptr);
+                          hipEvent_t stop = nullptr,
+                          int packed_layout = 0);
 int ensure_fix_side(lpx_state* s, int mode);
 lpxk::BlockRing ring_half(const lpx_state* s, int h);
 void launch_seed_entering(lpx_state* s, const lpxk::LoopStart& start = lpxk::LoopStart{});
diff --git a/linear_programming_solver_amd/csrc/lpx_kernels.hip b/linear_programming_solver_amd/csrc/lpx_kernels.hip
--- a/linear_programming_solver_amd/csrc/lpx_kernels.hip
+++ b/linear_programming_solver_amd/csrc/lpx_kernels.hip
@@ -813,9 +813,26 @@
                      R.prow + (int64_t)slot * B.ld, B.perm, B.ctl, R.up + slot, 0);
 }
 
+int sweep_pack_layout(const Buffers& B, const BlockRing& R, int m_local, int K, int form) {
+#if LPX_FUSED && !defined(LPX_CHAIN2_ONE_XCD)
+  if (!R.tickets || !R.col_packed || m_local < 16 || m_local % 16 != 0 || B.ld % 512 != 0 || B.ld < 512 ||
+      16 * B.ld * 8 + 1024 >= ((int64_t)1 << 32))
+    return kPackNone;
+#ifdef LPX_WITH_VARIANTS
+  if (B.chain_form != 1 || form != 0) return kPackNone;
+#else
+  if (form == 3) return kPackNone;
+#endif
+  return K > 64 ? kPackMfma128 : K > 32 ? kPackMfma64 : kPackNone;
+#else
+  (void)B; (void)R; (void)m_local; (void)K; (void)form;
+  return kPackNone;
+#endif
+}
+
 int launch_block_chain(const Buffers& B, const BlockRing& R, int n, int m, int nb, int half, int old_half, int n_old,
                         int b_from_tableau, int seq, int dantzig, int wgs, int fences, bool trace, LpxCtl* host_snap,
-                        hipStream_t s, const MgPeers* mg, hipEvent_t stop) {
+                        hipStream_t s, const MgPeers* mg, hipEvent_t stop, int pack_layout) {
   const int64_t work = std::max<int64_t>(m, B.ld);
   int G = wgs > 0 ? wgs : (int)std::min<int64_t>(64, std::max<int64_t>(1, (work + 511) / 512));
   G = std::max(1, std::min(G, kChainMaxWgs));
@@ -872,6 +889,14 @@
     } else LPX_LAUNCH_STOP((k_block_chain_t<true, 32>), dim3(G), dim3(256), s, stop, P);
   } else if (form2) {
     P.m_global = m; P.n_dev = 1;
+    if (pack_layout != kPackNone && R.col_packed && R.tickets) {
+      P.pack_layout = pack_layout;
+      P.col_packed = R.col_packed + (int64_t)half * (R.mp / 4 + 1) * (4 * kColPackedRowBytes / (int64_t)sizeof(double));
+      P.tickets = R.tickets + (int64_t)half * sweep_ticket_slots(B.ld) * 32;
+      const int nranges = std::max(1, std::min(kSweep128Ranges, m / 16));
+      P.pack_tickets = pack_layout == kPackMfma128 ? 1 + (int)(B.ld / 64) * nranges : (int)(B.ld / 512) * 8;
+      P.pack_clk = pack_layout == kPackMfma128 ? R.clk : nullptr;
+    }
 #ifdef LPX_CHAIN2_ONE_XCD
     G = std::min(G, 32);
     if (wide128) hipLaunchKernelGGL((k_block_decide128<kChain2Threads>), dim3(8 * G), dim3(kChain2Threads), 0, s, P);
@@ -1091,14 +1116,16 @@
 #if LPX_FUSED
 static void launch_sweep64_mfma(const Buffers& B, const BlockRing& R, int m_local, int kmax, bool nt, const double* A_src,
                                 hipStream_t s, int slots = 256, bool two_waves = false, int kmin = 33, const FixSide* side = nullptr,
-                                hipEvent_t t0 = nullptr, hipEvent_t t1 = nullptr) {
+                                hipEvent_t t0 = nullptr, hipEvent_t t1 = nullptr, bool packed = false) {
   const int nstrips_full = (int)(B.ld / 512);
   const int ngroups = nstrips_full * 2;
   const int ntiles = m_local / 16;
   const int G = std::max(1, std::min(ntiles, slots / std::max(1, ngroups)));
-  LPX_LAUNCH_STOP(k_pack_multipliers_mfma, dim3(ntiles), dim3(256), pack_stream(side, s), pack_stop(side), R.col, R.mp, R.up, kmax, ntiles, R.col_packed,
-                     R.tickets, nstrips_full * 8, two_waves ? (long long*)nullptr : R.clk, two_waves ? 1 : 0);
-  pack_done(side, s);
+  if (!packed) {
+    LPX_LAUNCH_STOP(k_pack_multipliers_mfma, dim3(ntiles), dim3(256), pack_stream(side, s), pack_stop(side), R.col, R.mp, R.up, kmax, ntiles, R.col_packed,
+                       R.tickets, nstrips_full * 8, two_waves ? (long long*)nullptr : R.clk, two_waves ? 1 : 0);
+    pack_done(side, s);
+  }
   if (two_waves) {
     const int ng2 = nstrips_full * 4;
     const int G2 = std::max(1, std::min(ntiles, 2 * slots / std::max(1, ng2)));
@@ -1127,13 +1154,15 @@
 
 #if LPX_FUSED
 static void launch_sweep128_mfma(const Buffers& B, const BlockRing& R, int m_local, int kmax, bool nt, const double* A_src,
-                                 hipStream_t s, int cus, const FixSide* side, hipEvent_t t0, hipEvent_t t1) {
+                                 hipStream_t s, int cus, const FixSide* side, hipEvent_t t0, hipEvent_t t1, bool packed) {
   const int nsub = (int)(B.ld / 64);
   const int ntiles = m_local / 16;
   const int nranges = std::max(1, std::min(kSweep128Ranges, ntiles));
-  LPX_LAUNCH_STOP(k_pack_multipliers_mfma128, dim3(ntiles), dim3(256), pack_stream(side, s), pack_stop(side), R.col, R.mp, R.up, kmax,
-                  ntiles, R.col_packed, R.tickets, 1 + nsub * nranges, R.clk);
-  pack_done(side, s);
+  if (!packed) {
+    LPX_LAUNCH_STOP(k_pack_multipliers_mfma128, dim3(ntiles), dim3(256), pack_stream(side, s), pack_stop(side), R.col, R.mp, R.up, kmax,
+                    ntiles, R.col_packed, R.tickets, 1 + nsub * nranges, R.clk);
+    pack_done(side, s);
+  }
   const dim3 grid(std::max(1, std::min(2 * cus, nsub * nranges))), block(256);
 #define LPX_LAUNCH_MFMA128(NT_, OOP_)                                                                                    \
   LPX_LAUNCH_TIMED((k_sweep128_mfma<NT_, OOP_>), grid, block, s, t0, t1, B.A, A_src, B.ld, m_local, R.prow, R.up, kmax, nsub, \
@@ -1187,7 +1216,8 @@
 
 int launch_block_sweep(const Buffers& B, const BlockRing& R, int n, int m_local, int row0, int K, int rows_per_wg,
                        bool nt, hipStream_t s, const double* A_src, const double* b_src, hipEvent_t after_sweep,
-                       int cus, int form, int* kernel_used, const FixSide* side, hipEvent_t stop, hipEvent_t before_sweep) {
+                       int cus, int form, int* kernel_used, const FixSide* side, hipEvent_t stop, hipEvent_t before_sweep,
+                       int packed_layout) {
   int used = kSweepNone;
   if (kernel_used) *kernel_used = used;
   if (K < 1) {
@@ -1227,7 +1257,8 @@
 #if LPX_FUSED
       timed_own = before_sweep && after_sweep;
       if (!timed_own) bracket();
-      launch_sweep128_mfma(B, R, m_local, K, nt, A_src, s, cus, side, timed_own ? before_sweep : nullptr, timed_own ? after_sweep : nullptr);
+      launch_sweep128_mfma(B, R, m_local, K, nt, A_src, s, cus, side, timed_own ? before_sweep : nullptr, timed_own ? after_sweep : nullptr,
+                           packed_layout == kPackMfma128);
 #endif
       rows_per_wg = 16;
       used = kSweepMfma128;
@@ -1266,7 +1297,7 @@
     if (mfma) {
 #if LPX_FUSED
       launch_sweep64_mfma(B, R, m_local, K, nt, A_src, s, cus, mfma2, whole ? 1 : 33, side, timed_own ? before_sweep : nullptr,
-                          timed_own ? after_sweep : nullptr);
+                          timed_own ? after_sweep : nullptr, packed_layout == kPackMfma64 && whole);
 #endif
       rows64 = 16;
     } else if (one) {
diff --git a/linear_programming_solver_amd/csrc/lpx_launchers.inc b/linear_programming_solver_amd/csrc/lpx_launchers.inc
--- a/linear_programming_solver_amd/csrc/lpx_launchers.inc
+++ b/linear_programming_solver_amd/csrc/lpx_launchers.inc
@@ -18,7 +18,9 @@
                          int slot, hipStream_t s);
 int launch_block_chain(const Buffers& B, const BlockRing& R, int n, int m, int nb, int half, int old_half, int n_old,
                         int b_from_tableau, int seq, int dantzig, int wgs, int fences, bool trace, LpxCtl* host_snap,
-                        hipStream_t s, const MgPeers* mg = nullptr, hipEvent_t stop = nullptr);
+                        hipStream_t s, const MgPeers* mg = nullptr, hipEvent_t stop = nullptr,
+                        int pack_layout = 0);
+int sweep_pack_layout(const Buffers& B, const BlockRing& R, int m_local, int K, int form);
 void preload_block_kernels(const Buffers& B, const BlockRing& R, hipStream_t s);
 unsigned* sweep_fail_word(const BlockRing& R, int64_t ld);
 int64_t sweep_ticket_slots(int64_t ld);
@@ -27,7 +29,8 @@
 int launch_block_sweep(const Buffers& B, const BlockRing& R, int n, int m_local, int row0, int K, int rows_per_wg,
                        bool nt, hipStream_t s, const double* A_src = nullptr, const double* b_src = nullptr,
                        hipEvent_t after_sweep = nullptr, int cus = 0, int form = 0, int* kernel_used = nullptr,
-                       const FixSide* side = nullptr, hipEvent_t stop = nullptr, hipEvent_t before_sweep = nullptr);
+                       const FixSide* side = nullptr, hipEvent_t stop = nullptr, hipEvent_t before_sweep = nullptr,
+                       int packed_layout = 0);
 void launch_fill_column(double* A, int64_t ld, int m, int col, double value, hipStream_t s);
 void launch_drop_column(double* A, int64_t ld, int m, int n_old, int col, hipStream_t s);
 void launch_restore_objective(const Buffers& B, int n, const RestoreEntry* d_entries, int n_entries, hipStream_t s);
diff --git a/linear_programming_solver_amd/csrc/lpx_sweeps.inc b/linear_programming_solver_amd/csrc/lpx_sweeps.inc
--- a/linear_programming_solver_amd/csrc/lpx_sweeps.inc
+++ b/linear_programming_solver_amd/csrc/lpx_sweeps.inc
@@ -813,7 +813,7 @@
   __shared__ int sh_np;
   sweep_front_stamp(clk);
   const int np = ring_count(ring, 64, kmax, &sh_np);
-  if (np < kmin) return;
+  if (np < kmin && !(OOP && kmin <= 1)) return;
   const int lane = threadIdx.x & 63;
   const int wave = __builtin_amdgcn_readfirstlane((int)(threadIdx.x >> 6));
   const int ngroups = nstrips_full * 4;
```
